# GuyTevet/motion-diffusion-model

Measured on NVIDIA H100. Metric: motions/sec, higher is better.
Workload: dtype fp16 operands / fp32 accumulate (in/out projections hi-lo split)

## Files before the change

include/b200mdm.h:

```cpp
#ifndef B200MDM_H_
#define B200MDM_H_

#include <stdint.h>

#ifdef __cplusplus
extern "C" {
#endif

#define B200MDM_OK 0
#define B200MDM_EINVAL (-1)
#define B200MDM_ECUDA (-2)
#define B200MDM_ESTATE (-3)
#define B200MDM_ENOTIMPL (-4)

#define B200MDM_ARCH_TRANS_ENC 0
#define B200MDM_ARCH_TRANS_DEC 1

#define B200MDM_COND_NONE 0
#define B200MDM_COND_TEXT 1
#define B200MDM_COND_ACTION 2

#define B200MDM_MODE_X0 0
#define B200MDM_MODE_DDPM 1
#define B200MDM_MODE_DDIM 2
#define B200MDM_MODE_DDIM_REVERSE 6

#define B200MDM_FLAG_CONST_NOISE 1
#define B200MDM_FLAG_CLIP_DENOISED 2
#define B200MDM_FLAG_PHILOX_NOISE 4

#define B200MDM_SCHED_STRIDE 8

typedef struct b200mdm_engine b200mdm_engine;

typedef struct b200mdm_config {
  int32_t arch;
  int32_t latent_dim;
  int32_t ff_size;
  int32_t num_layers;
  int32_t num_heads;
  int32_t njoints;
  int32_t nfeats;
  int32_t cond_mode;
  int32_t cond_dim;
  int32_t num_actions;
  int32_t mask_frames;
  int32_t pos_embed_max_len;
  int32_t temb_rows;
  int32_t context_len;
  int32_t target_encoder;
  int32_t target_enc_layers;
  int32_t target_joints;
  int32_t emb_trans_dec;
  int32_t dec_memory;
  int32_t reserved[1];
} b200mdm_config;

#define B200MDM_DEC_MEMORY_TOKENS 0
#define B200MDM_DEC_MEMORY_CLIP 1

#define B200MDM_TARGET_NONE 0
#define B200MDM_TARGET_SINGLE 1
#define B200MDM_TARGET_MULTI 2
#define B200MDM_TARGET_SPLIT 3

const char* b200mdm_last_error(void);
int b200mdm_version(void);

int b200mdm_create(const b200mdm_config* cfg, b200mdm_engine** out);
int b200mdm_destroy(b200mdm_engine* e);

int b200mdm_load_weight(b200mdm_engine* e, const char* name, const float* data, const int64_t* shape, int32_t ndim);

int b200mdm_finalize_weights(b200mdm_engine* e, void* stream);

int b200mdm_set_schedule(b200mdm_engine* e, int32_t n_steps, const float* rows_host, const int32_t* timestep_map_host);

#define B200MDM_SCHED_NEXT_STRIDE 2
int b200mdm_set_schedule_next(b200mdm_engine* e, int32_t n_steps, const float* rows_host);

#define B200MDM_SCHED_DPM_STRIDE 4
int b200mdm_set_schedule_dpm(b200mdm_engine* e, int32_t n_steps, const float* rows_host);

#define B200MDM_SCHED_VB_STRIDE 12
int b200mdm_set_schedule_vb(b200mdm_engine* e, int32_t n_steps, const float* rows_host);

int b200mdm_set_cond(b200mdm_engine* e, int32_t batch, int32_t nframes, const float* cond_embed_dev,
                     const int64_t* lengths_host, const float* scale_dev, int32_t force_uncond,
                     const int64_t* action_host, void* stream);

int b200mdm_set_cond_dec(b200mdm_engine* e, int32_t batch, int32_t nframes, const float* enc_text_dev,
                         const uint8_t* text_mask_host, int32_t n_tokens, const int64_t* lengths_host,
                         const float* scale_dev, int32_t force_uncond, void* stream);
int b200mdm_set_prefix(b200mdm_engine* e, const float* prefix_dev, void* stream);

int b200mdm_set_target(b200mdm_engine* e, const float* target_dev, const uint8_t* valid_host, void* stream);

int b200mdm_set_inpaint(b200mdm_engine* e, const uint8_t* mask_dev, const float* motion_dev);
int b200mdm_set_inpaint_weight(b200mdm_engine* e, const float* weight_dev, const float* motion_dev);

int b200mdm_set_handshake(b200mdm_engine* e, int32_t h, const int64_t* lengths_host, const uint8_t* motion_start_host,
                          void* stream);

int b200mdm_set_joint_guidance(b200mdm_engine* e, const float* mean_dev, const float* std_dev, const float* target_dev,
                               const float* weight_dev, float step, int32_t iters, void* stream);

int b200mdm_set_foot_guidance(b200mdm_engine* e, float contact_weight, float floor_weight, float floor_height,
                              const float* contact_dev, const int64_t* lengths_host, void* stream);

typedef struct b200mdm_grid {
  const float* values;
  int64_t batch_stride;
  int32_t gz, gx;
  float x0, z0, cell;
} b200mdm_grid;

int b200mdm_set_scene_guidance(b200mdm_engine* e, float obstacle_weight, float obstacle_margin, const b200mdm_grid* sdf,
                               const b200mdm_grid* terrain, void* stream);

#define B200MDM_MAX_INTERACTION_PAIRS 1024
int b200mdm_set_interaction_guidance(b200mdm_engine* e, int32_t characters, float weight, float margin,
                                     const float* placement_dev, const int32_t* pairs_host, int32_t n_pairs,
                                     const float* reach_host, const float* pair_weight_dev, int64_t pair_weight_stride,
                                     void* stream);

#define B200MDM_MAX_PROMPTS 8
int b200mdm_set_cond_multi(b200mdm_engine* e, int32_t batch, int32_t nframes, int32_t K, const float* prompt_embed_dev,
                           const int64_t* lengths_host, const int64_t* prompt_action_host, void* stream);
int b200mdm_set_cond_multi_dec(b200mdm_engine* e, int32_t batch, int32_t nframes, int32_t K, const float* prompt_clip_dev,
                               const int64_t* lengths_host, void* stream);
int b200mdm_set_cond_multi_tokens(b200mdm_engine* e, int32_t batch, int32_t nframes, int32_t K, const float* tokens_dev,
                                  const uint8_t* mask_host, int32_t n_tokens, const int64_t* lengths_host, void* stream);
int b200mdm_set_prompt_weight(b200mdm_engine* e, int32_t K, const float* weight_dev, int64_t stride_b, int64_t stride_k,
                              int64_t stride_f, int64_t stride_t, void* stream);

int b200mdm_denoise(b200mdm_engine* e, const float* x_dev, const int32_t* timesteps_host, float* out_dev, void* stream);

int b200mdm_sample_step(b200mdm_engine* e, int32_t mode, int32_t index, const float* x_t_dev, const float* noise_dev,
                        int32_t flags, float* x_out_dev, float* pred_xstart_dev, void* stream);

int b200mdm_sample_loop(b200mdm_engine* e, int32_t mode, int32_t skip_timesteps, const float* x_T_dev, float* x_0_dev,
                        const float* noise_tape_dev, int64_t noise_step_stride, int32_t flags, int32_t use_graph,
                        void* stream);

int b200mdm_sample_loop_range(b200mdm_engine* e, int32_t mode, int32_t first_index, int32_t n_run, const float* x_in_dev,
                              float* x_out_dev, const float* noise_tape_dev, int64_t noise_step_stride, int32_t flags,
                              int32_t use_graph, void* stream);

int b200mdm_sample_step_at(b200mdm_engine* e, int32_t mode, const int32_t* index_host, const float* x_t_dev,
                           const float* noise_dev, int32_t flags, float* x_out_dev, float* pred_xstart_dev, void* stream);

int b200mdm_slots_begin(b200mdm_engine* e, int32_t slots, int32_t nframes, int32_t guided, int32_t mode, int32_t flags,
                        void* stream);

int b200mdm_slot_admit(b200mdm_engine* e, int32_t slot, const float* cond_embed_dev, int64_t action, float scale,
                       int64_t length, uint64_t seed, int64_t sample_index, void* stream);

int b200mdm_slots_run(b200mdm_engine* e, int32_t n_steps, int32_t use_graph, void* stream);

int b200mdm_slot_read(b200mdm_engine* e, int32_t slot, float* out_dev, void* stream);

int b200mdm_chain_slots_begin(b200mdm_engine* e, int32_t slots, int32_t nframes, int32_t guided, int32_t mode,
                              int32_t flags, int32_t n_tokens, void* stream);

int b200mdm_chain_slot_admit(b200mdm_engine* e, int32_t slot, const float* tokens_dev, const uint8_t* mask_dev,
                             const float* prefix_dev, float scale, int64_t length, int32_t include_prefix, uint64_t seed,
                             int64_t sample_index, void* stream);

int b200mdm_chain_slot_handoff(b200mdm_engine* e, int32_t slot, float* out_dev, const float* tokens_dev,
                               const uint8_t* mask_dev, void* stream);

int b200mdm_ddim_reverse_loop_range(b200mdm_engine* e, int32_t first_index, int32_t n_run, const float* x_in_dev,
                                    float* x_out_dev, int32_t flags, int32_t use_graph, void* stream);

int b200mdm_plms_loop_range(b200mdm_engine* e, int32_t order, int32_t first_index, int32_t n_run, const float* x_in_dev,
                            float* x_out_dev, int32_t flags, int32_t use_graph, void* stream);

int b200mdm_plms_step(b200mdm_engine* e, int32_t index, int32_t order, const float* x_t_dev, const float* const* old_eps_dev,
                      int32_t n_old, int32_t flags, float* x_out_dev, float* pred_xstart_dev, float* eps_out_dev,
                      void* stream);

int b200mdm_dpm_loop_range(b200mdm_engine* e, int32_t order, int32_t first_index, int32_t n_run, const float* x_in_dev,
                           float* x_out_dev, int32_t flags, int32_t use_graph, void* stream);
int b200mdm_dpm_pred_xstart(b200mdm_engine* e, float* out_dev, void* stream);

int b200mdm_chain_setup(b200mdm_engine* e, int32_t n_chunks, int32_t pred_len, int32_t context_len, int32_t include_prefix,
                        int32_t crop, const float* enc_chunks_dev, const uint8_t* text_mask_chunks_host, void* stream);
int b200mdm_chain_loop_range(b200mdm_engine* e, int32_t mode, int32_t order, int32_t first_step, int32_t n_run,
                             const float* x_T_dev, int64_t x_T_chunk_stride, const float* noise_tape_dev,
                             int64_t noise_step_stride, float* out_dev, int32_t flags, int32_t use_graph, void* stream);
int b200mdm_chain_set_goal(b200mdm_engine* e, const float* mean_dev, const float* std_dev, const float* goal_dev,
                           int32_t n_goals, const uint8_t* valid_host, void* stream);
int b200mdm_chunk_frame(double* carry_dev, const float* frames_dev, int32_t batch, int32_t n_feats, int32_t n_frames,
                        const float* mean_dev, const float* std_dev, const float* goal_dev, int32_t n_ext, float* target_dev,
                        void* stream);

int b200mdm_vb_loop_range(b200mdm_engine* e, int32_t first_index, int32_t n_run, const float* x_start_dev,
                          const float* noise_tape_dev, int64_t noise_step_stride, int32_t flags, float* terms_dev,
                          float* bpd_dev, int32_t use_graph, void* stream);

int b200mdm_set_noise_stream(b200mdm_engine* e, uint64_t seed, int64_t sample_index_base);
int b200mdm_philox_normal(float* out_dev, int32_t batch, int64_t n_per_sample, uint64_t seed, int64_t sample_index_base,
                          int32_t step_id, void* stream);

int b200mdm_q_sample(b200mdm_engine* e, float sqrt_ac, float sqrt_1mac, const float* x_start_dev,
                     const float* noise_dev, float* out_dev, int64_t n, void* stream);

int64_t b200mdm_launch_count(b200mdm_engine* e, int32_t reset);

int b200mdm_recover_from_ric(const float* data_dev, int64_t stride_b, int64_t stride_f, int64_t stride_t,
                             const float* mean_dev, const float* std_dev, float* out_dev, int64_t ostride_b,
                             int64_t ostride_t, int64_t ostride_c, int32_t batch, int32_t nframes, int32_t njoints,
                             void* stream);

int b200mdm_test_gemm_f16(const void* a16_dev, const void* w16_dev, const float* bias_dev, void* out16_dev, int32_t M,
                          int32_t N, int32_t K, int32_t act, int32_t block_n, void* stream);
int b200mdm_test_gemm_epi(const void* a16_dev, const void* w16_dev, const float* bias_dev, void* out16_dev, int32_t M,
                          int32_t N, int32_t K, int32_t epi, void* stream);
int b200mdm_test_embed(const float* x_dev, const float* w_in_dev, const float* b_in_dev, const float* pe_dev, void* hres16_dev,
                       int32_t B, int32_t JF, int32_t T, int32_t d, int32_t s_off, int32_t halves, void* stream);
int b200mdm_test_out_step(const void* hres16_dev, const float* scale_dev, const float* w_out_dev, const float* b_out_dev,
                          const float* x_t_dev, const float* noise_dev, const float* sched_row_dev, int32_t mode, int32_t flags,
                          const uint8_t* inpaint_mask_dev, const float* inpaint_motion_dev, float* x_out_dev,
                          float* pred_xstart_dev, int32_t B, int32_t JF, int32_t T, int32_t d, int32_t s_off, int32_t halves,
                          void* stream);
int b200mdm_test_out_dpm(const void* hres16_dev, const float* scale_dev, const float* w_out_dev, const float* b_out_dev,
                         const float* x_t_dev, const float* dpm_row_dev, int32_t index, int32_t step, int32_t order,
                         int32_t flags, const uint8_t* inpaint_mask_dev, const float* inpaint_motion_dev,
                         float* x0_hist_dev, float* x_out_dev, int32_t B, int32_t JF, int32_t T, int32_t d, int32_t s_off,
                         int32_t halves, void* stream);
int b200mdm_test_out_vb(const void* hres16_dev, const float* scale_dev, const float* w_out_dev, const float* b_out_dev,
                        const float* x_t_dev, const float* x_start_dev, const float* noise_dev, const float* vb_row_dev,
                        int32_t index, int32_t n_steps, int32_t flags, const uint8_t* inpaint_mask_dev,
                        const float* inpaint_motion_dev, float* pred_xstart_dev, float* elem_dev, float* terms_dev, int32_t B,
                        int32_t JF, int32_t T, int32_t d, int32_t s_off, int32_t halves, void* stream);
int b200mdm_test_out_weight(const void* hres16_dev, const float* scale_dev, const float* w_out_dev, const float* b_out_dev,
                            const float* x_t_dev, int32_t mode, int32_t flags, const float* weight_dev,
                            const float* motion_dev, float* pred_xstart_dev, int32_t B, int32_t JF, int32_t T, int32_t d,
                            int32_t s_off, int32_t halves, void* stream);
int b200mdm_test_blend_handshake(const void* hres16_dev, const float* scale_dev, void* g16_dev, int32_t B, int32_t T,
                                 int32_t d, int32_t s_off, int32_t halves, int32_t h, const int64_t* lengths_host,
                                 const uint8_t* motion_start_host, void* stream);
int b200mdm_test_joint_guidance(const float* x0_dev, const float* mean_dev, const float* std_dev, const float* target_dev,
                                const float* weight_dev, int32_t B, int32_t T, int32_t D, float step, int32_t iters,
                                float* x0_out_dev, float* loss_out_dev, void* stream);
int b200mdm_test_foot_guidance(const float* x0_dev, const float* mean_dev, const float* std_dev, const float* target_dev,
                               const float* weight_dev, const float* contact_dev, const int64_t* lengths_host, int32_t B,
                               int32_t T, int32_t D, float step, int32_t iters, float contact_weight, float floor_weight,
                               float floor_height, float* x0_out_dev, float* loss_out_dev, void* stream);
int b200mdm_test_scene_guidance(const float* x0_dev, const float* mean_dev, const float* std_dev, const float* target_dev,
                                const float* weight_dev, const float* contact_dev, const int64_t* lengths_host, int32_t B,
                                int32_t T, int32_t D, float step, int32_t iters, float contact_weight, float floor_weight,
                                float floor_height, float obstacle_weight, float obstacle_margin, const b200mdm_grid* sdf,
                                const b200mdm_grid* terrain, float* x0_out_dev, float* loss_out_dev, void* stream);
int b200mdm_test_interaction_guidance(const float* x0_dev, const float* mean_dev, const float* std_dev, const float* target_dev,
                                      const float* weight_dev, const float* contact_dev, const int64_t* lengths_host,
                                      int32_t B, int32_t T, int32_t D, float step, int32_t iters, float contact_weight,
                                      float floor_weight, float floor_height, float obstacle_weight, float obstacle_margin,
                                      const b200mdm_grid* sdf, const b200mdm_grid* terrain, int32_t characters, float weight,
                                      float margin, const float* placement_dev, const int32_t* pairs_host, int32_t n_pairs,
                                      const float* reach_host, const float* pair_weight_dev, int64_t pair_weight_stride,
                                      float* x0_out_dev, float* loss_out_dev, void* stream);
int b200mdm_test_attention(const void* qkv16_dev, void* out16_dev, const int32_t* kvlen_dev, int32_t n_samples,
                           int32_t S, int32_t d, int32_t impl, void* stream);
int b200mdm_test_cross_attention(const void* q16_dev, const void* kv16_dev, const unsigned char* mask_dev, void* out16_dev,
                                 int32_t n_samples, int32_t S, int32_t n_tokens, int32_t ld_kv, void* stream);
int b200mdm_test_qkv_attention(const void* h16_dev, int32_t ld, const void* wqkv16_dev, const float* bqkv_dev,
                               void* out16_dev, const int32_t* kvlen_dev, int32_t n_samples, int32_t S, void* stream);
int b200mdm_test_gemm_resid_ln(const void* a16_dev, const void* w16_dev, const float* bias_dev, const float* gamma_dev,
                               const float* beta_dev, void* hres16_dev, int32_t M, int32_t K, void* stream);
int b200mdm_test_target(b200mdm_engine* e, const float* target_dev, const uint8_t* valid_host, int32_t batch,
                        float* out_dev, void* stream);
int b200mdm_test_cross_rows(b200mdm_engine* e, int32_t timestep, float* out_dev, void* stream);
int b200mdm_test_row_bias_ln(void* hres16_dev, const float* c_dev, const float* gamma_dev, const float* beta_dev,
                             int32_t M, int32_t S, void* stream);

#define B200MDM_TAP_EMBED 0
#define B200MDM_TAP_TOK0 1
#define B200MDM_TAP_CONDPROJ 2
#define B200MDM_TAP_TEMB 3
#define B200MDM_TAP_MEM16 4
#define B200MDM_TAP_CROSS_C 5
#define B200MDM_TAP_KVC16 6
#define B200MDM_TAP_L_IN 7
#define B200MDM_TAP_L_QKV 8
#define B200MDM_TAP_L_ATT 9
#define B200MDM_TAP_L_LN1 10
#define B200MDM_TAP_L_QC 11
#define B200MDM_TAP_L_XATT 12
#define B200MDM_TAP_L_LN2 13
#define B200MDM_TAP_L_FFN 14
#define B200MDM_TAP_L_LN3 15
#define B200MDM_TAP_BLEND 16
#define B200MDM_TAP_COUNT 17
int b200mdm_test_forward_taps(b200mdm_engine* e, const float* x_dev, const int32_t* timesteps_host, float* out_dev,
                              int32_t layer, void* const* tap_dev, int32_t n_taps, void* stream);

#ifdef __cplusplus
}
#endif
#endif
```

motion-diffusion-model_b200/_lib.py:

```python
import ctypes
import os

HERE = os.path.dirname(os.path.abspath(__file__))
LIB_PATH = os.environ.get("B200MDM_LIB") or os.path.join(HERE, "lib", "libb200mdm.so")

OK, EINVAL, ECUDA, ESTATE, ENOTIMPL = 0, -1, -2, -3, -4
ARCH = {"trans_enc": 0, "trans_dec": 1}
COND_NONE, COND_TEXT, COND_ACTION = 0, 1, 2
TARGET = {"single": 1, "multi": 2, "split": 3}
MODE_X0, MODE_DDPM, MODE_DDIM = 0, 1, 2
MODE_DDIM_REVERSE = 6
MODE_PLMS_AB, MODE_DPM, MODE_VB = 3, 7, 8
FLAG_CONST_NOISE, FLAG_CLIP_DENOISED, FLAG_PHILOX_NOISE = 1, 2, 4
SCHED_STRIDE = 8
SCHED_NEXT_STRIDE = 2
SCHED_DPM_STRIDE = 4
SCHED_VB_STRIDE = 12

SYMBOLS = [
    "b200mdm_last_error", "b200mdm_version", "b200mdm_create", "b200mdm_destroy", "b200mdm_load_weight",
    "b200mdm_finalize_weights", "b200mdm_set_schedule", "b200mdm_set_cond", "b200mdm_set_cond_dec", "b200mdm_set_prefix",
    "b200mdm_set_inpaint",
    "b200mdm_denoise", "b200mdm_sample_step", "b200mdm_sample_loop", "b200mdm_q_sample", "b200mdm_launch_count",
    "b200mdm_sample_loop_range", "b200mdm_set_noise_stream", "b200mdm_philox_normal",
    "b200mdm_recover_from_ric", "b200mdm_test_gemm_f16", "b200mdm_test_attention", "b200mdm_test_cross_attention", "b200mdm_test_qkv_attention",
    "b200mdm_test_gemm_resid_ln", "b200mdm_test_gemm_epi", "b200mdm_test_embed", "b200mdm_test_out_step",
    "b200mdm_set_target", "b200mdm_test_target", "b200mdm_plms_loop_range", "b200mdm_plms_step",
    "b200mdm_set_schedule_next", "b200mdm_ddim_reverse_loop_range", "b200mdm_test_cross_rows",
    "b200mdm_test_row_bias_ln", "b200mdm_test_forward_taps",
    "b200mdm_set_schedule_dpm", "b200mdm_dpm_loop_range", "b200mdm_dpm_pred_xstart", "b200mdm_test_out_dpm",
    "b200mdm_set_schedule_vb", "b200mdm_vb_loop_range", "b200mdm_test_out_vb",
    "b200mdm_set_handshake", "b200mdm_test_blend_handshake", "b200mdm_set_inpaint_weight", "b200mdm_test_out_weight",
    "b200mdm_chain_setup", "b200mdm_chain_loop_range", "b200mdm_set_joint_guidance", "b200mdm_test_joint_guidance",
    "b200mdm_set_cond_multi", "b200mdm_set_cond_multi_dec", "b200mdm_set_prompt_weight",
    "b200mdm_set_cond_multi_tokens", "b200mdm_set_foot_guidance", "b200mdm_test_foot_guidance",
    "b200mdm_set_scene_guidance", "b200mdm_test_scene_guidance", "b200mdm_chain_set_goal", "b200mdm_chunk_frame",
    "b200mdm_set_interaction_guidance", "b200mdm_test_interaction_guidance",
    "b200mdm_sample_step_at", "b200mdm_slots_begin", "b200mdm_slot_admit", "b200mdm_slots_run", "b200mdm_slot_read",
    "b200mdm_chain_slots_begin", "b200mdm_chain_slot_admit", "b200mdm_chain_slot_handoff",
]
MAX_PROMPTS = 8
MAX_CHARACTERS = 8
MAX_INTERACTION_PAIRS = 1024
MAX_MEMORY_TOKENS = 512
TAPS = ["EMBED", "TOK0", "CONDPROJ", "TEMB", "MEM16", "CROSS_C", "KVC16", "L_IN", "L_QKV", "L_ATT", "L_LN1", "L_QC",
        "L_XATT", "L_LN2", "L_FFN", "L_LN3", "BLEND"]
DEC_MEMORY_TOKENS, DEC_MEMORY_CLIP = 0, 1


class Config(ctypes.Structure):
    _fields_ = [(n, ctypes.c_int32) for n in (
        "arch", "latent_dim", "ff_size", "num_layers", "num_heads", "njoints", "nfeats", "cond_mode", "cond_dim",
        "num_actions", "mask_frames", "pos_embed_max_len", "temb_rows", "context_len", "target_encoder",
        "target_enc_layers", "target_joints", "emb_trans_dec", "dec_memory")] + [("reserved", ctypes.c_int32 * 1)]


class Grid(ctypes.Structure):
    _fields_ = [("values", ctypes.c_void_p), ("batch_stride", ctypes.c_int64), ("gz", ctypes.c_int32),
                ("gx", ctypes.c_int32), ("x0", ctypes.c_float), ("z0", ctypes.c_float), ("cell", ctypes.c_float)]


class B200MDMError(RuntimeError):
    def __init__(self, code, msg):
        super().__init__("libb200mdm error %d: %s" % (code, msg))
        self.code = code


_lib = None


def load():
    global _lib
    if _lib is not None:
        return _lib
    if not os.path.exists(LIB_PATH):
        raise ImportError(
            "libb200mdm.so is not built (%s). Run `python -c 'import __graft_entry__ as g; g.build()'`; "
            "there is no CPU / PyTorch fallback for the sampling path." % LIB_PATH)
    import torch
    lib = ctypes.CDLL(LIB_PATH, mode=ctypes.RTLD_GLOBAL)
    vp, i32, i64, f32 = ctypes.c_void_p, ctypes.c_int32, ctypes.c_int64, ctypes.c_float
    lib.b200mdm_last_error.restype = ctypes.c_char_p
    lib.b200mdm_last_error.argtypes = []
    lib.b200mdm_version.restype = i32
    lib.b200mdm_create.argtypes = [ctypes.POINTER(Config), ctypes.POINTER(vp)]
    lib.b200mdm_destroy.argtypes = [vp]
    lib.b200mdm_load_weight.argtypes = [vp, ctypes.c_char_p, vp, ctypes.POINTER(i64), i32]
    lib.b200mdm_finalize_weights.argtypes = [vp, vp]
    lib.b200mdm_set_schedule.argtypes = [vp, i32, vp, vp]
    lib.b200mdm_set_cond.argtypes = [vp, i32, i32, vp, vp, vp, i32, vp, vp]
    lib.b200mdm_set_cond_dec.argtypes = [vp, i32, i32, vp, vp, i32, vp, vp, i32, vp]
    lib.b200mdm_set_prefix.argtypes = [vp, vp, vp]
    lib.b200mdm_set_inpaint.argtypes = [vp, vp, vp]
    lib.b200mdm_recover_from_ric.argtypes = [vp, i64, i64, i64, vp, vp, vp, i64, i64, i64, i32, i32, i32, vp]
    lib.b200mdm_denoise.argtypes = [vp, vp, vp, vp, vp]
    lib.b200mdm_sample_step.argtypes = [vp, i32, i32, vp, vp, i32, vp, vp, vp]
    lib.b200mdm_sample_step_at.argtypes = [vp, i32, vp, vp, vp, i32, vp, vp, vp]
    lib.b200mdm_slots_begin.argtypes = [vp, i32, i32, i32, i32, i32, vp]
    lib.b200mdm_slot_admit.argtypes = [vp, i32, vp, i64, f32, i64, ctypes.c_uint64, i64, vp]
    lib.b200mdm_slots_run.argtypes = [vp, i32, i32, vp]
    lib.b200mdm_slot_read.argtypes = [vp, i32, vp, vp]
    lib.b200mdm_sample_loop.argtypes = [vp, i32, i32, vp, vp, vp, i64, i32, i32, vp]
    lib.b200mdm_sample_loop_range.argtypes = [vp, i32, i32, i32, vp, vp, vp, i64, i32, i32, vp]
    lib.b200mdm_set_noise_stream.argtypes = [vp, ctypes.c_uint64, i64]
    lib.b200mdm_philox_normal.argtypes = [vp, i32, i64, ctypes.c_uint64, i64, i32, vp]
    lib.b200mdm_q_sample.argtypes = [vp, f32, f32, vp, vp, vp, i64, vp]
    lib.b200mdm_launch_count.argtypes = [vp, i32]
    lib.b200mdm_launch_count.restype = i64
    lib.b200mdm_test_gemm_f16.argtypes = [vp, vp, vp, vp, i32, i32, i32, i32, i32, vp]
    lib.b200mdm_test_attention.argtypes = [vp, vp, vp, i32, i32, i32, i32, vp]
    if hasattr(lib, "b200mdm_test_cross_attention"):
        lib.b200mdm_test_cross_attention.argtypes = [vp, vp, vp, vp, i32, i32, i32, i32, vp]
    lib.b200mdm_test_qkv_attention.argtypes = [vp, i32, vp, vp, vp, vp, i32, i32, vp]
    lib.b200mdm_test_gemm_resid_ln.argtypes = [vp, vp, vp, vp, vp, vp, i32, i32, vp]
    for name, args in (("b200mdm_test_gemm_epi", [vp, vp, vp, vp, i32, i32, i32, i32, vp]),
                       ("b200mdm_test_embed", [vp, vp, vp, vp, vp, i32, i32, i32, i32, i32, i32, vp]),
                       ("b200mdm_test_out_step", [vp, vp, vp, vp, vp, vp, vp, i32, i32, vp, vp, vp, vp,
                                                  i32, i32, i32, i32, i32, i32, vp]),
                       ("b200mdm_set_target", [vp, vp, vp, vp]),
                       ("b200mdm_test_target", [vp, vp, vp, i32, vp, vp]),
                       ("b200mdm_plms_loop_range", [vp, i32, i32, i32, vp, vp, i32, i32, vp]),
                       ("b200mdm_plms_step", [vp, i32, i32, vp, ctypes.POINTER(vp), i32, i32, vp, vp, vp, vp]),
                       ("b200mdm_set_schedule_next", [vp, i32, vp]),
                       ("b200mdm_ddim_reverse_loop_range", [vp, i32, i32, vp, vp, i32, i32, vp]),
                       ("b200mdm_test_cross_rows", [vp, i32, vp, vp]),
                       ("b200mdm_test_row_bias_ln", [vp, vp, vp, vp, i32, i32, vp]),
                       ("b200mdm_test_forward_taps", [vp, vp, vp, vp, i32, ctypes.POINTER(vp), i32, vp]),
                       ("b200mdm_set_schedule_dpm", [vp, i32, vp]),
                       ("b200mdm_dpm_loop_range", [vp, i32, i32, i32, vp, vp, i32, i32, vp]),
                       ("b200mdm_dpm_pred_xstart", [vp, vp, vp]),
                       ("b200mdm_test_out_dpm", [vp, vp, vp, vp, vp, vp, i32, i32, i32, i32, vp, vp, vp, vp,
                                                 i32, i32, i32, i32, i32, i32, vp]),
                       ("b200mdm_set_schedule_vb", [vp, i32, vp]),
                       ("b200mdm_vb_loop_range", [vp, i32, i32, vp, vp, i64, i32, vp, vp, i32, vp]),
                       ("b200mdm_test_out_vb", [vp, vp, vp, vp, vp, vp, vp, vp, i32, i32, i32, vp, vp, vp, vp, vp,
                                                i32, i32, i32, i32, i32, i32, vp]),
                       ("b200mdm_set_handshake", [vp, i32, vp, vp, vp]),
                       ("b200mdm_test_blend_handshake", [vp, vp, vp, i32, i32, i32, i32, i32, i32, vp, vp, vp]),
                       ("b200mdm_set_inpaint_weight", [vp, vp, vp]),
                       ("b200mdm_test_out_weight", [vp, vp, vp, vp, vp, i32, i32, vp, vp, vp, i32, i32, i32, i32, i32, i32,
                                                    vp]),
                       ("b200mdm_chain_setup", [vp, i32, i32, i32, i32, i32, vp, vp, vp]),
                       ("b200mdm_chain_loop_range", [vp, i32, i32, i32, i32, vp, i64, vp, i64, vp, i32, i32, vp]),
                       ("b200mdm_set_joint_guidance", [vp, vp, vp, vp, vp, f32, i32, vp]),
                       ("b200mdm_test_joint_guidance", [vp, vp, vp, vp, vp, i32, i32, i32, f32, i32, vp, vp, vp]),
                       ("b200mdm_set_foot_guidance", [vp, f32, f32, f32, vp, vp, vp]),
                       ("b200mdm_test_foot_guidance", [vp, vp, vp, vp, vp, vp, vp, i32, i32, i32, f32, i32, f32, f32, f32,
                                                       vp, vp, vp]),
                       ("b200mdm_set_scene_guidance", [vp, f32, f32, ctypes.POINTER(Grid), ctypes.POINTER(Grid), vp]),
                       ("b200mdm_test_scene_guidance", [vp, vp, vp, vp, vp, vp, vp, i32, i32, i32, f32, i32, f32, f32, f32,
                                                        f32, f32, ctypes.POINTER(Grid), ctypes.POINTER(Grid), vp, vp, vp]),
                       ("b200mdm_set_interaction_guidance", [vp, i32, f32, f32, vp, vp, i32, vp, vp, ctypes.c_int64, vp]),
                       ("b200mdm_test_interaction_guidance", [vp, vp, vp, vp, vp, vp, vp, i32, i32, i32, f32, i32, f32, f32,
                                                              f32, f32, f32, ctypes.POINTER(Grid), ctypes.POINTER(Grid), i32,
                                                              f32, f32, vp, vp, i32, vp, vp, ctypes.c_int64, vp, vp, vp]),
                       ("b200mdm_set_cond_multi", [vp, i32, i32, i32, vp, vp, vp, vp]),
                       ("b200mdm_set_cond_multi_dec", [vp, i32, i32, i32, vp, vp, vp]),
                       ("b200mdm_set_cond_multi_tokens", [vp, i32, i32, i32, vp, vp, i32, vp, vp]),
                       ("b200mdm_set_prompt_weight", [vp, i32, vp, i64, i64, i64, i64, vp]),
                       ("b200mdm_chain_set_goal", [vp, vp, vp, vp, i32, vp, vp]),
                       ("b200mdm_chunk_frame", [vp, vp, i32, i32, i32, vp, vp, vp, i32, vp, vp]),
                       ("b200mdm_chain_slots_begin", [vp, i32, i32, i32, i32, i32, i32, vp]),
                       ("b200mdm_chain_slot_admit", [vp, i32, vp, vp, vp, f32, i64, i32, ctypes.c_uint64, i64, vp]),
                       ("b200mdm_chain_slot_handoff", [vp, i32, vp, vp, vp, vp])):
        if hasattr(lib, name):
            getattr(lib, name).argtypes = args
    for name in SYMBOLS:
        if not hasattr(lib, name) and os.environ.get("B200MDM_LIB"):
            continue
        fn = getattr(lib, name)
        if fn.restype is ctypes.c_int and name not in ("b200mdm_version",):
            fn.restype = i32
    _lib = lib
    return lib


def check(code):
    if code != OK:
        raise B200MDMError(code, load().b200mdm_last_error().decode("utf-8", "replace"))
```

motion-diffusion-model_b200/csrc/engine.cu:

```cuda
#include <cuda.h>
#include <cuda_fp16.h>
#include <cuda_runtime.h>

#include <algorithm>
#include <cmath>
#include <cstdarg>
#include <cstdio>
#include <cstring>
#include <initializer_list>
#include <map>
#include <string>
#include <vector>

#include "../../include/b200mdm.h"
#include "attention_tc.cuh"
#include "epilogues.cuh"
#include "gemm.cuh"
#include "gemm_ln.cuh"
#include "gemm_pingpong.cuh"
#include "chunk_frame.cuh"
#include "joint_guidance.cuh"
#include "compose.cuh"
#include "postprocess.cuh"
#include "kernels.cuh"

using namespace b200;

static thread_local char g_err[512] = "";
static int fail(int code, const char* fmt, ...) {
  va_list ap;
  va_start(ap, fmt);
  vsnprintf(g_err, sizeof(g_err), fmt, ap);
  va_end(ap);
  return code;
}
#define CUDA_TRY(expr)                                                                               \
  do {                                                                                               \
    cudaError_t _e = (expr);                                                                         \
    if (_e != cudaSuccess)                                                                           \
      return fail(B200MDM_ECUDA, "%s failed: %s (%s:%d)", #expr, cudaGetErrorString(_e), __FILE__, __LINE__); \
  } while (0)
#define TRY(expr)            \
  do {                       \
    int _r = (expr);         \
    if (_r != B200MDM_OK) return _r; \
  } while (0)

typedef CUresult (*EncodeTiledFn)(CUtensorMap*, CUtensorMapDataType, cuuint32_t, void*, const cuuint64_t*,
                                  const cuuint64_t*, const cuuint32_t*, const cuuint32_t*, CUtensorMapInterleave,
                                  CUtensorMapSwizzle, CUtensorMapL2promotion, CUtensorMapFloatOOBfill);
static EncodeTiledFn g_encode = nullptr;
static int resolve_driver() {
  if (g_encode) return B200MDM_OK;
  void* fn = nullptr;
  cudaDriverEntryPointQueryResult qres;
  CUDA_TRY(cudaGetDriverEntryPoint("cuTensorMapEncodeTiled", &fn, cudaEnableDefault, &qres));
  if (!fn || qres != cudaDriverEntryPointSuccess) return fail(B200MDM_ECUDA, "cuTensorMapEncodeTiled not available");
  g_encode = reinterpret_cast<EncodeTiledFn>(fn);
  return B200MDM_OK;
}
static int encode_map(CUtensorMap* m, CUtensorMapDataType dtype, uint32_t rank, const void* ptr, const cuuint64_t* gdim,
                      const cuuint64_t* gstride_bytes, const cuuint32_t* box, CUtensorMapSwizzle swizzle, const char* what) {
  TRY(resolve_driver());
  if ((reinterpret_cast<uintptr_t>(ptr) & 15) || gstride_bytes[0] % 16) return fail(B200MDM_EINVAL, "TMA operand misaligned");
  const cuuint32_t estr[3] = {1, 1, 1};
  CUresult r = g_encode(m, dtype, rank, const_cast<void*>(ptr), gdim, gstride_bytes, box, estr, CU_TENSOR_MAP_INTERLEAVE_NONE,
                        swizzle, CU_TENSOR_MAP_L2_PROMOTION_L2_256B, CU_TENSOR_MAP_FLOAT_OOB_FILL_NONE);
  if (r != CUDA_SUCCESS) return fail(B200MDM_ECUDA, "cuTensorMapEncodeTiled%s failed (%d)", what, static_cast<int>(r));
  return B200MDM_OK;
}
static int make_map_t(CUtensorMap* m, const void* ptr, int elem_bytes, uint64_t rows, uint64_t cols, uint64_t ld,
                      uint32_t box_rows) {
  const cuuint64_t gdim[2] = {cols, rows}, gstr[1] = {ld * elem_bytes};
  const cuuint32_t box[2] = {static_cast<cuuint32_t>(128 / elem_bytes), box_rows};
  return encode_map(m, elem_bytes == 2 ? CU_TENSOR_MAP_DATA_TYPE_FLOAT16 : CU_TENSOR_MAP_DATA_TYPE_FLOAT32, 2, ptr, gdim, gstr,
                    box, CU_TENSOR_MAP_SWIZZLE_128B, "");
}
static int make_map(CUtensorMap* m, const void* ptr, uint64_t rows, uint64_t cols, uint64_t ld, uint32_t box_rows) {
  return make_map_t(m, ptr, 2, rows, cols, ld, box_rows);
}
static int make_map_3d(CUtensorMap* m, const void* ptr, uint64_t n, uint64_t rows, uint64_t cols, uint64_t ld,
                       uint32_t box_rows) {
  const cuuint64_t gdim[3] = {cols, rows, n}, gstr[2] = {ld * 2, rows * ld * 2};
  const cuuint32_t box[3] = {64, box_rows, 1};
  return encode_map(m, CU_TENSOR_MAP_DATA_TYPE_FLOAT16, 3, ptr, gdim, gstr, box, CU_TENSOR_MAP_SWIZZLE_128B, "(3d)");
}

static int make_hres_map(CUtensorMap* m, const void* hres, uint64_t rows) {
  return make_map(m, hres, rows, 2 * GLN_D, 2 * GLN_D, GLN_RES_BOX_ROWS);
}

static int make_map_res(CUtensorMap* m, const void* ptr, uint64_t rows, uint64_t d) {
  const cuuint64_t gdim[2] = {2 * d, rows}, gstr[1] = {d * 4};
  const cuuint32_t box[2] = {32, 32};
  return encode_map(m, CU_TENSOR_MAP_DATA_TYPE_FLOAT16, 2, ptr, gdim, gstr, box, CU_TENSOR_MAP_SWIZZLE_64B, "(residual)");
}

enum SchedTable { TAB_STEP, TAB_NEXT, TAB_DPM, TAB_VB, N_TABLES };
static constexpr int TAB_STRIDE[N_TABLES] = {SCHED_STRIDE, SCHED_NEXT_STRIDE, SCHED_DPM_STRIDE, SCHED_VB_STRIDE};
static const char* const TAB_SETTER[N_TABLES] = {"b200mdm_set_schedule", "b200mdm_set_schedule_next",
                                                 "b200mdm_set_schedule_dpm", "b200mdm_set_schedule_vb"};
static_assert(SCHED_STRIDE == B200MDM_SCHED_STRIDE && SCHED_NEXT_STRIDE == B200MDM_SCHED_NEXT_STRIDE &&
                  SCHED_DPM_STRIDE == B200MDM_SCHED_DPM_STRIDE && SCHED_VB_STRIDE == B200MDM_SCHED_VB_STRIDE,
              "the tables' row layouts are part of the ABI");

struct Tensor32 {
  float* dev = nullptr;
  std::vector<int64_t> shape;
  size_t numel = 0;
};

struct LayerW {
  __half *wqkv = nullptr, *wo = nullptr, *w1 = nullptr, *w2 = nullptr;
  const float *bqkv, *bo, *b1, *b2, *g1, *be1, *g2, *be2;
  CUtensorMap m_wqkv, m_w1;
  CUtensorMap m_wo_256, m_w2_256;
  __half *wq_c = nullptr, *wo_c = nullptr;
  const float *bq_c = nullptr, *bo_c = nullptr, *g3 = nullptr, *be3 = nullptr;
  CUtensorMap m_wq_c, m_wo_c_256;
  const float *wv_c32 = nullptr, *bv_c32 = nullptr, *wo_c32 = nullptr;
};

struct GraphKey {
  int mode = -1, B = 0, T = 0, flags = 0;
  int order = 0;
  const void *pred = nullptr, *imask = nullptr, *iweight = nullptr, *imotion = nullptr;
  const void* target_g = nullptr;
  const void* hs = nullptr;
  int guide = -1;
  int chars = 0;
  int groups = 0;
  bool slots = false;
  bool operator==(const GraphKey& o) const {
    return mode == o.mode && B == o.B && T == o.T && flags == o.flags && order == o.order && pred == o.pred &&
           imask == o.imask && iweight == o.iweight && imotion == o.imotion && target_g == o.target_g && hs == o.hs &&
           guide == o.guide && chars == o.chars && groups == o.groups && slots == o.slots;
  }
};

struct Workspace {
  int B = 0, T = 0, S = 0, halves = 1, Bp = 0, M = 0, MB = 0;
  int groups = 0;
  float* mp_x0 = nullptr;
  __half *xin16 = nullptr, *hres = nullptr, *qkv16 = nullptr, *att16 = nullptr, *ffn16 = nullptr, *g16 = nullptr;
  float *tok0 = nullptr, *condproj = nullptr, *proj = nullptr, *scale = nullptr, *x_work = nullptr, *eps_buf = nullptr;
  int *kvlen = nullptr, *tvec = nullptr, *action = nullptr;
  CUtensorMap m_xin, m_h16, m_att, m_ffn, m_g16;
  CUtensorMap m_qkv_st, m_ffn_st;
  CUtensorMap m_qkv_kv;
  CUtensorMap m_res_c, m_res_u;
  CUtensorMap m_hres;
  float* pe_bias = nullptr;
  bool cond_set = false;
  int Mt = 0;
  float *encperm = nullptr, *memtok = nullptr, *memproj = nullptr;
  __half *mem16 = nullptr, *qc16 = nullptr, *kvc16 = nullptr;
  unsigned char* memmask = nullptr;
  CUtensorMap m_mem, m_qc_st, m_kvc_st;
  bool prefix_set = false;
  float *cross_mb = nullptr, *cross_u = nullptr, *cross_b = nullptr, *cross_c = nullptr;
  float *tgt_valid = nullptr, *tgt_g = nullptr;
  bool target_set = false;
  int* hs_desc = nullptr;
  bool hs_set = false;
  float* jg_x0 = nullptr;
  float *plms_ring = nullptr, *plms_mid = nullptr, *plms_pred = nullptr;
  int plms_done = -1, plms_order = 0;
  float* dpm_hist = nullptr;
  int dpm_done = -1, dpm_order = 0;
  float *vb_xs = nullptr, *vb_part = nullptr, *vb_terms = nullptr;
  int vb_cap = 0;
  bool vb_live = false;
  SlotState* slots = nullptr;
  cudaGraphExec_t graph_exec = nullptr;
  GraphKey graph_key;
  int graph_kernels = 0;
  unsigned long long last_use = 0;
};

struct b200mdm_engine : Workspace {
  b200mdm_config cfg;
  int d, ff, L, H, JF, Kp_in, N_out_pad;
  int num_sms = 132;
  std::map<std::string, Tensor32> store;
  bool finalized = false;
  __half *w_in3 = nullptr, *w_out3 = nullptr;
  CUtensorMap m_win, m_wout;
  std::vector<LayerW> layers;
  const float *b_in = nullptr, *b_out = nullptr, *pe = nullptr, *w_txt = nullptr, *b_txt = nullptr, *act_emb = nullptr;
  float *temb_hidden = nullptr, *temb_table = nullptr;
  __half* wkv_all = nullptr;
  float* bkv_all = nullptr;
  CUtensorMap m_wkv_all;
  float *tw0 = nullptr, *tb0 = nullptr, *twk = nullptr, *tbk = nullptr, *twsum = nullptr;
  int tG = 0, tdj = 0, tin = 0, tlayers = 0;
  std::vector<float> h_valid;
  float* tab[N_TABLES] = {};
  bool tab_fresh[N_TABLES] = {};
  int* tmap = nullptr;
  int n_steps = 0, sched_cap = 0;
  std::vector<Workspace> pool;
  unsigned long long use_clock = 0;
  std::vector<int> h_kv, h_action;
  std::vector<unsigned char> h_mask;
  std::vector<int> h_hs;
  bool dec = false;
  bool dec_clip = false;
  float* cross_t = nullptr;
  int ctx = 0, s_off = 1;
  int kw = 1;
  const unsigned char* inpaint_mask = nullptr;
  const float* inpaint_weight = nullptr;
  const float* inpaint_motion = nullptr;
  GuideDesc* jg_desc = nullptr;
  GuideDesc h_guide{};
  unsigned guide_terms = 0;
  int* fg_len = nullptr;
  int fg_len_cap = 0;
  std::vector<int> h_fg_len;
  InterPair* ig_pairs = nullptr;
  int ig_pairs_cap = 0;
  std::vector<InterPair> h_ig_pairs;
  PromptWeight* pw_desc = nullptr;
  PromptWeight h_pw{};
  bool pw_set = false;
  unsigned long long noise_seed = 0;
  long long noise_sample_base = 0;
  StepState* state = nullptr;
  cudaStream_t work = nullptr;
  cudaEvent_t ev_in = nullptr, ev_out = nullptr;
  long long launches = 0;
  bool mem_uncond = false;
  float *chain_mem = nullptr, *chain_prefix = nullptr;
  unsigned char* chain_mask = nullptr;
  size_t chain_mem_cap = 0, chain_mask_cap = 0, chain_prefix_cap = 0;
  std::vector<unsigned char> h_chain_mask;
  int chain_n = 0, chain_off = 0, chain_crop = 0, chain_next = -1;
  bool chain_mems = false;
  const float* prefix_src = nullptr;
  bool slot_mode = false;
  int slot_sampler = 0, slot_flags = 0;
  std::vector<unsigned char> slot_busy;
  std::vector<int> slot_left;
  std::vector<int> h_slot_idx;
  struct ChainSlot {
    unsigned long long seed = 0;
    long long g = 0;
    float scale = 0.f;
    int kv = 0, length = 0, off = 0, chunk = 0, n_chunks = 0;
  };
  std::vector<ChainSlot> chain_slot;
  const float *goal_mean = nullptr, *goal_std = nullptr, *goal_src = nullptr;
  double* goal_carry = nullptr;
  float* goal_tgt = nullptr;
  size_t goal_carry_cap = 0, goal_tgt_cap = 0;
  int goal_n = 0;
  bool goal_set = false;
};

template <class T>
static int dalloc(T** p, size_t n, bool zero = false) {
  const cudaError_t err = cudaMalloc(reinterpret_cast<void**>(p), n * sizeof(T));
  if (err != cudaSuccess) {
    cudaGetLastError();
    return fail(B200MDM_ECUDA, "cudaMalloc of %zu bytes failed: %s", n * sizeof(T), cudaGetErrorString(err));
  }
  if (zero) CUDA_TRY(cudaMemset(*p, 0, n * sizeof(T)));
  return B200MDM_OK;
}
template <class T>
static void dfree(T*& p) {
  if (p) cudaFree(p);
  p = nullptr;
}

template <int BN, class Epi>
static int set_gemm_attr() {
  CUDA_TRY(cudaFuncSetAttribute(gemm_f16_wgmma<BN, Epi>, cudaFuncAttributeMaxDynamicSharedMemorySize, GemmSmem<BN, Epi>::TOTAL));
  return B200MDM_OK;
}
template <class Epi>
static int set_pingpong_attr() {
  CUDA_TRY(cudaFuncSetAttribute(gemm_f16_pingpong<Epi>, cudaFuncAttributeMaxDynamicSharedMemorySize, PP_SMEM_BYTES));
  return B200MDM_OK;
}
template <int KEYS>
static int set_attention_attr() {
  CUDA_TRY(cudaFuncSetAttribute(attention_tc_kernel<KEYS, false>, cudaFuncAttributeMaxDynamicSharedMemorySize,
                                AttnTcSmem::total(KEYS)));
  CUDA_TRY(cudaFuncSetAttribute(attention_tc_kernel<KEYS, true>, cudaFuncAttributeMaxDynamicSharedMemorySize,
                                AttnTcSmem::total(KEYS)));
  return B200MDM_OK;
}

enum GuideTerm : unsigned { GT_JOINT = 1, GT_FOOT = 2, GT_SCENE = 4, GT_INTER = 8 };
struct GuideVariant {
  void (*step)(const GuideDesc*, const float*, EpiOutParams);
  void (*test)(GuideDesc, const float*, float*, float*, int, int, int);
  size_t (*smem)(int, int);
  bool clusters;
};
static const GuideVariant GUIDE_VARIANTS[] = {
    {joint_guidance_step_kernel<false, false>, joint_guidance_test_kernel<false, false>, jg_smem_bytes, false},
    {joint_guidance_step_kernel<true, false>, joint_guidance_test_kernel<true, false>, fg_smem_bytes, false},
    {joint_guidance_step_kernel<true, true>, joint_guidance_test_kernel<true, true>, fg_smem_bytes, false},
    {joint_guidance_step_kernel<true, true, true>, joint_guidance_test_kernel<true, true, true>, ig_smem_bytes, true},
};
static int guide_variant(unsigned terms) { return terms ? 31 - __builtin_clz(terms) : -1; }
struct RicDims {
  int J, R;
};
static RicDims ric_dims(int D) {
  const int J = D == 263 ? 22 : 21;
  return {J, 4 + 3 * (J - 1)};
}

static int init_kernel_attrs() {
  static unsigned long long done_mask = 0;
  int dev = 0;
  CUDA_TRY(cudaGetDevice(&dev));
  if (dev < 64 && ((done_mask >> dev) & 1ull)) return B200MDM_OK;
  TRY((set_pingpong_attr<EpiBiasF16<false>>()));
  TRY((set_pingpong_attr<EpiBiasF16<true>>()));
  TRY((set_pingpong_attr<EpiBiasF16Wide<true>>()));
  TRY((set_pingpong_attr<EpiBiasF16Global>()));
  CUDA_TRY(cudaFuncSetAttribute(gemm_resid_ln_cluster, cudaFuncAttributeMaxDynamicSharedMemorySize, GemmLnSmem::TOTAL));
  TRY((set_gemm_attr<128, EpiEmbed>()));
  TRY((set_gemm_attr<96, EpiOut<OutStep>>()));
  TRY((set_gemm_attr<96, EpiOut<OutStepSlots>>()));
  TRY((set_gemm_attr<96, EpiOut<OutPlms>>()));
  TRY((set_gemm_attr<96, EpiOut<OutReverse>>()));
  TRY((set_gemm_attr<96, EpiOut<OutDpm>>()));
  TRY((set_gemm_attr<96, EpiOut<OutVb>>()));
  TRY((set_attention_attr<64>()));
  TRY((set_attention_attr<208>()));
  TRY((set_attention_attr<256>()));
  CUDA_TRY(cudaFuncSetAttribute(cross_attention_long_kernel, cudaFuncAttributeMaxDynamicSharedMemorySize, XAL_SMEM));
  for (const GuideVariant& v : GUIDE_VARIANTS) {
    const int smem = static_cast<int>(v.smem(JG_MAX_FRAMES, JG_MAX_FEATS));
    CUDA_TRY(cudaFuncSetAttribute(v.step, cudaFuncAttributeMaxDynamicSharedMemorySize, smem));
    CUDA_TRY(cudaFuncSetAttribute(v.test, cudaFuncAttributeMaxDynamicSharedMemorySize, smem));
  }
  if (dev < 64) done_mask |= 1ull << dev;
  return B200MDM_OK;
}

static bool g_pdl_now = false;
static bool pdl_enabled() {
  static int v = -1;
  if (v < 0) {
    const char* e = getenv("B200MDM_PDL");
    v = (e && e[0] == '0') ? 0 : 1;
  }
  return v == 1;
}
struct PdlScope {
  PdlScope() { g_pdl_now = pdl_enabled(); }
  ~PdlScope() { g_pdl_now = false; }
};
template <class... KArgs, class... Args>
static cudaError_t launch_kc(void (*kern)(KArgs...), dim3 grid, dim3 block, size_t smem, cudaStream_t s, int cluster,
                             Args&&... args) {
  cudaLaunchConfig_t cfg;
  memset(&cfg, 0, sizeof(cfg));
  cfg.gridDim = grid;
  cfg.blockDim = block;
  cfg.dynamicSmemBytes = smem;
  cfg.stream = s;
  cudaLaunchAttribute at[2];
  int n = 0;
  if (cluster > 0) {
    at[n].id = cudaLaunchAttributeClusterDimension;
    at[n].val.clusterDim.x = static_cast<unsigned>(cluster);
    at[n].val.clusterDim.y = 1;
    at[n].val.clusterDim.z = 1;
    ++n;
  }
  if (g_pdl_now) {
    at[n].id = cudaLaunchAttributeProgrammaticStreamSerialization;
    at[n].val.programmaticStreamSerializationAllowed = 1;
    ++n;
  }
  cfg.attrs = at;
  cfg.numAttrs = n;
  return cudaLaunchKernelEx(&cfg, kern, static_cast<KArgs>(std::forward<Args>(args))...);
}
template <class... KArgs, class... Args>
static cudaError_t launch_k(void (*kern)(KArgs...), dim3 grid, dim3 block, size_t smem, cudaStream_t s, Args&&... args) {
  return launch_kc(kern, grid, block, smem, s, 0, std::forward<Args>(args)...);
}

template <class Epi, class = void> struct epi_unstaged : std::false_type {};
template <class Epi> struct epi_unstaged<Epi, std::enable_if_t<Epi::UNSTAGED>> : std::true_type {};

static_assert(GemmSmem<128, EpiEmbed>::STAGES == 2, "shared-memory budget: 2 operand stages for the embedding GEMM");
static_assert(GemmSmem<96, EpiOut<OutStep>>::STAGES == 5, "shared-memory budget: 5 operand stages for the output GEMM");
template <int BN, class Epi>
static int launch_gemm(const CUtensorMap& a, const CUtensorMap& b, int M, int N, int K, const typename Epi::Params& p,
                       cudaStream_t s, int num_sms) {
  const int tiles = ((M + GEMM_BLOCK_M - 1) / GEMM_BLOCK_M) * ((N + BN - 1) / BN);
  const int grid = tiles < num_sms ? tiles : num_sms;
  CUDA_TRY(launch_k(gemm_f16_wgmma<BN, Epi>, dim3(grid), dim3(GEMM_THREADS), GemmSmem<BN, Epi>::TOTAL, s, a, b, M, N, K, p));
  return B200MDM_OK;
}
template <class Epi>
static int launch_gemm_pp(const CUtensorMap& a, const CUtensorMap& b, const CUtensorMap& c, int M, int N, int K,
                          const typename Epi::Params& p, cudaStream_t s, int num_sms) {
  if (!epi_unstaged<Epi>::value && N * 4 > GEMM_BIAS_BYTES)
    return fail(B200MDM_ENOTIMPL, "GEMM epilogue vectors are staged for N <= %d", GEMM_BIAS_BYTES / 4);
  const int tiles = ((M + GEMM_BLOCK_M - 1) / GEMM_BLOCK_M) * ((N + PP_BLOCK_N - 1) / PP_BLOCK_N);
  const int grid = tiles < num_sms ? tiles : num_sms;
  CUDA_TRY(launch_k(gemm_f16_pingpong<Epi>, dim3(grid), dim3(GEMM_THREADS), PP_SMEM_BYTES, s, a, b, c, M, N, K, p));
  return B200MDM_OK;
}
template <bool GELU>
static int launch_gemm_bias(const CUtensorMap& a, const CUtensorMap& b, const CUtensorMap& c, int M, int N, int K,
                            const float* bias, cudaStream_t s, int num_sms) {
  typename EpiBiasF16<GELU>::Params p{bias};
  return launch_gemm_pp<EpiBiasF16<GELU>>(a, b, c, M, N, K, p, s, num_sms);
}

static int launch_gemm_resid_ln(const CUtensorMap& a, const CUtensorMap& w256, const CUtensorMap& hres, int M, int K,
                                const float* bias, const float* gamma, const float* beta, cudaStream_t s, int num_sms) {
  const int tiles = (M + GEMM_BLOCK_M - 1) / GEMM_BLOCK_M;
  const int max_clusters = num_sms / 2;
  const int clusters = tiles < max_clusters ? tiles : max_clusters;
  GemmLnParams lp{bias, gamma, beta, 1e-5f};
  CUDA_TRY(launch_k(gemm_resid_ln_cluster, dim3(2 * clusters), dim3(GLN_THREADS), GemmLnSmem::TOTAL, s, a, w256, hres, M, K, lp));
  return B200MDM_OK;
}

static int make_attention_kv_map(CUtensorMap* m, const void* qkv, int n_samples, int S, int ld) {
  return make_map_3d(m, qkv, n_samples, S, ld, ld, atc_keys(S));
}
template <int KEYS>
static cudaError_t launch_attention_keys(const CUtensorMap& map_kv, const __half* qkv, __half* out, const int* kvlen,
                                         dim3 grid, int S, int d, float scale_log2, cudaStream_t s, bool wide) {
  return launch_k(wide ? attention_tc_kernel<KEYS, true> : attention_tc_kernel<KEYS, false>, grid, dim3(ATC_THREADS),
                  AttnTcSmem::total(KEYS), s, map_kv, qkv, out, kvlen, S, d, scale_log2);
}
static int launch_attention_tc(const CUtensorMap& map_kv, const __half* qkv, __half* out, const int* kvlen, int n_samples,
                               int S, int d, int H, cudaStream_t s, bool wide = false) {
  if (d != H * ATC_DH) return fail(B200MDM_ENOTIMPL, "attention: head_dim must be 128");
  if (S > ATC_MAX_KEYS) return fail(B200MDM_ENOTIMPL, "attention: at most %d tokens per sample", ATC_MAX_KEYS);
  const float scale_log2 = 1.4426950408889634f / sqrtf(static_cast<float>(ATC_DH));
  const int tiles = (S + ATC_QROWS - 1) / ATC_QROWS;
  const dim3 grid(H, n_samples, (tiles + ATC_TILES_PER_CTA - 1) / ATC_TILES_PER_CTA);
  const int keys = atc_keys(S);
  if (keys == 64) CUDA_TRY(launch_attention_keys<64>(map_kv, qkv, out, kvlen, grid, S, d, scale_log2, s, wide));
  else if (keys == 208) CUDA_TRY(launch_attention_keys<208>(map_kv, qkv, out, kvlen, grid, S, d, scale_log2, s, wide));
  else CUDA_TRY(launch_attention_keys<256>(map_kv, qkv, out, kvlen, grid, S, d, scale_log2, s, wide));
  return B200MDM_OK;
}
static int launch_cross_attention(const __half* q16, const __half* kv, const unsigned char* mask, __half* out, int n_samples,
                                  int S, int Mt, int d, int H, int ld_kv, cudaStream_t s) {
  const float sl2 = 1.4426950408889634f / sqrtf(128.0f);
  const dim3 cg(H, n_samples), cb(128);
  if (Mt <= 16)
    CUDA_TRY(launch_k(cross_attention_kernel<2>, cg, cb, 0, s, q16, kv, mask, out, S, Mt, d, ld_kv, sl2));
  else if (Mt <= 32)
    CUDA_TRY(launch_k(cross_attention_kernel<4>, cg, cb, 0, s, q16, kv, mask, out, S, Mt, d, ld_kv, sl2));
  else if (Mt <= 64)
    CUDA_TRY(launch_k(cross_attention_kernel<8>, cg, cb, 0, s, q16, kv, mask, out, S, Mt, d, ld_kv, sl2));
  else
    CUDA_TRY(launch_k(cross_attention_long_kernel, dim3(H, n_samples, (S + XAL_ROWS - 1) / XAL_ROWS), cb, XAL_SMEM, s, q16, kv,
                      mask, out, S, Mt, d, ld_kv, sl2));
  return B200MDM_OK;
}
static int launch_row_bias_ln(__half* hres, const float* c, const float* gamma, const float* beta, int M, int S, cudaStream_t s) {
  CUDA_TRY(launch_k(row_bias_ln_kernel, dim3((M + RBLN_ROWS_PER_CTA - 1) / RBLN_ROWS_PER_CTA), dim3(32 * RBLN_ROWS_PER_CTA), 0, s,
                    hres, c, gamma, beta, M, S, 1e-5f));
  return B200MDM_OK;
}
static int philox_blocks(int B, long long n) {
  const long long quads = (n + 3) / 4 * B;
  return static_cast<int>(quads / 256 + 1 < 1184 ? quads / 256 + 1 : 1184);
}
static int launch_philox(float* out, int B, long long n, unsigned long long seed, long long sample_base, uint32_t step_id,
                         const StepState* state, cudaStream_t s) {
  CUDA_TRY(launch_k(philox_normal_kernel, dim3(philox_blocks(B, n)), dim3(256), 0, s, out, B, n, seed, sample_base, step_id,
                    state));
  return B200MDM_OK;
}
static int launch_pack_input(const float* x, __half* xin16, int B, int JF, int cols, int S, int Kp, int row_off, cudaStream_t s) {
  CUDA_TRY(launch_k(pack_input_kernel, dim3((cols + 31) / 32, (JF + 31) / 32, B), dim3(32, 8), 0, s, x, xin16, B, JF, cols, S,
                    Kp, 3 * Kp, row_off));
  return B200MDM_OK;
}
static int launch_embed_gemm(const CUtensorMap& m_xin, const CUtensorMap& m_win, const CUtensorMap& m_res_c,
                             const CUtensorMap& m_res_u, const float* pe_bias, int MB, int S, int d, int Kp, int halves,
                             cudaStream_t s, int num_sms) {
  EpiEmbed::Params p;
  p.res_c = m_res_c; p.res_u = m_res_u;
  p.pe_bias = pe_bias;
  p.S = S; p.d = d; p.halves = halves;
  return launch_gemm<128, EpiEmbed>(m_xin, m_win, MB, d, 3 * Kp, p, s, num_sms);
}
static int launch_vb_xt(float* x_t, const float* x_start, const float* noise, const float* sched_vb, const StepState* state,
                        size_t n, cudaStream_t s) {
  const int blocks = static_cast<int>(n / 256 + 1 < 1184 ? n / 256 + 1 : 1184);
  CUDA_TRY(launch_k(vb_xt_kernel, dim3(blocks), dim3(256), 0, s, x_t, x_start, noise, sched_vb, state, n));
  return B200MDM_OK;
}
static int launch_vb_reduce(float* terms, int ld_terms, const float* part, int B, int T, int JF, const StepState* state,
                            cudaStream_t s) {
  CUDA_TRY(launch_k(vb_reduce_kernel, dim3(B, VB_TERMS), dim3(VB_REDUCE_THREADS), 0, s, terms, ld_terms, part, B,
                    T * ((JF + 31) / 32), static_cast<float>(JF) * static_cast<float>(T), state));
  return B200MDM_OK;
}
static int launch_blend_split(const __half* hres, __half* g16, const float* scale, int B, int S, int T, int s_off, int d,
                              int halves, const int* hs, cudaStream_t s) {
  CUDA_TRY(launch_k(blend_split_kernel, dim3((B * T + 7) / 8), dim3(256), 0, s, hres, g16, scale, B, S, T, s_off, d, halves, hs));
  return B200MDM_OK;
}

static int handshake_desc(int h, int B, int T, const int64_t* lengths, const uint8_t* motion_start, std::vector<int>* desc) {
  desc->clear();
  if (h < 0) return fail(B200MDM_EINVAL, "handshake size %d < 0", h);
  if (B <= 0 || T <= 0) return fail(B200MDM_EINVAL, "bad batch / nframes");
  if (motion_start && !motion_start[0]) return fail(B200MDM_EINVAL, "window 0 must begin a motion (motion_start[0])");
  if (h == 0) return B200MDM_OK;
  std::vector<int> d(1 + 2 * static_cast<size_t>(B), 0);
  d[HS_H] = h;
  bool any = false;
  for (int b = 0; b < B; ++b) {
    const long long n = lengths ? lengths[b] : T;
    if (n < 0 || n > T) return fail(B200MDM_EINVAL, "window %d: length %lld outside [0, %d]", b, n, T);
    d[HS_LEN(b)] = static_cast<int>(n);
    d[HS_CHAIN(b)] = (b > 0 && !(motion_start && motion_start[b])) ? 1 : 0;
    any = any || d[HS_CHAIN(b)];
  }
  for (int b = 0; b < B; ++b) {
    const bool prev = d[HS_CHAIN(b)] != 0, next = b + 1 < B && d[HS_CHAIN(b + 1)] != 0;
    const int n = d[HS_LEN(b)];
    if ((prev || next) && n < h) return fail(B200MDM_EINVAL, "chained window %d has %d frames < handshake size %d", b, n, h);
    if (prev && next && n < 2 * h)
      return fail(B200MDM_EINVAL, "window %d has %d frames < 2 x handshake size %d: its two handshakes would overlap", b, n, h);
  }
  if (any) desc->swap(d);
  return B200MDM_OK;
}
#ifdef B200_TRACE
static int debug_skip_mask() {
  static int v = -1;
  if (v < 0) {
    const char* e = getenv("B200MDM_DEBUG_SKIP");
    v = e ? atoi(e) : 0;
  }
  return v;
}
#define B200_SKIP(bit) (debug_skip_mask() & (bit))
#else
#define B200_SKIP(bit) (0)
#endif
extern "C" const char* b200mdm_last_error(void) { return g_err; }
extern "C" int b200mdm_version(void) { return 1; }

extern "C" int b200mdm_create(const b200mdm_config* cfg, b200mdm_engine** out) {
  if (!cfg || !out) return fail(B200MDM_EINVAL, "null argument");
  if (cfg->arch != B200MDM_ARCH_TRANS_ENC && cfg->arch != B200MDM_ARCH_TRANS_DEC)
    return fail(B200MDM_ENOTIMPL, "arch %d: trans_enc and trans_dec are implemented", cfg->arch);
  if (cfg->arch == B200MDM_ARCH_TRANS_DEC && (cfg->cond_mode != B200MDM_COND_TEXT || cfg->context_len < 0))
    return fail(B200MDM_ENOTIMPL, "trans_dec needs text-token conditioning (BERT) and context_len >= 0");
  if (cfg->emb_trans_dec < 0 || cfg->emb_trans_dec > 1 || cfg->dec_memory < B200MDM_DEC_MEMORY_TOKENS ||
      cfg->dec_memory > B200MDM_DEC_MEMORY_CLIP)
    return fail(B200MDM_EINVAL, "emb_trans_dec must be 0 or 1 and dec_memory 0 (tokens) or 1 (CLIP) (got %d / %d)",
                cfg->emb_trans_dec, cfg->dec_memory);
  if (cfg->arch == B200MDM_ARCH_TRANS_ENC && (cfg->emb_trans_dec || cfg->dec_memory))
    return fail(B200MDM_EINVAL, "emb_trans_dec and dec_memory are trans_dec fields");
  if (cfg->arch == B200MDM_ARCH_TRANS_DEC && (cfg->dec_memory == B200MDM_DEC_MEMORY_CLIP) != (cfg->emb_trans_dec == 1))
    return fail(B200MDM_ENOTIMPL, "trans_dec implements the BERT token memory without the timestep token (DiP) and the CLIP "
                "memory with it (emb_trans_dec); got dec_memory %d, emb_trans_dec %d", cfg->dec_memory, cfg->emb_trans_dec);
  if (cfg->dec_memory == B200MDM_DEC_MEMORY_CLIP && cfg->context_len != 0)
    return fail(B200MDM_ENOTIMPL, "trans_dec with a CLIP memory has no prefix completion (context_len %d)", cfg->context_len);
  if (cfg->latent_dim != 512 || cfg->num_heads != 4 || cfg->ff_size % 64 || cfg->ff_size <= 0)
    return fail(B200MDM_ENOTIMPL, "kernels are specialised for latent_dim 512 / 4 heads (got %d / %d)", cfg->latent_dim,
                cfg->num_heads);
  if (cfg->num_layers <= 0 || cfg->njoints <= 0 || cfg->nfeats <= 0 || cfg->pos_embed_max_len <= 0 || cfg->temb_rows <= 0)
    return fail(B200MDM_EINVAL, "bad config");
  if (cfg->target_encoder < B200MDM_TARGET_NONE || cfg->target_encoder > B200MDM_TARGET_SPLIT)
    return fail(B200MDM_EINVAL, "target_encoder %d: 0 none, 1 single, 2 multi, 3 split", cfg->target_encoder);
  if (cfg->target_encoder != B200MDM_TARGET_NONE) {
    if (cfg->target_joints <= 0 || cfg->target_joints > 64 || cfg->target_enc_layers < 0 || cfg->target_enc_layers > 16)
      return fail(B200MDM_EINVAL, "target encoder: 1..64 joints and 0..16 layers (got %d / %d)", cfg->target_joints,
                  cfg->target_enc_layers);
    if (cfg->target_encoder == B200MDM_TARGET_SPLIT && cfg->latent_dim % cfg->target_joints)
      return fail(B200MDM_EINVAL, "split target encoder: latent_dim %% target_joints != 0 (model/mdm.py:427)");
  }
  int dev = 0;
  CUDA_TRY(cudaGetDevice(&dev));
  cudaDeviceProp prop;
  CUDA_TRY(cudaGetDeviceProperties(&prop, dev));
  if (prop.major != 9 || prop.minor != 0) return fail(B200MDM_ECUDA, "sm_90a device required (found sm_%d%d)", prop.major, prop.minor);
  TRY(init_kernel_attrs());
  TRY(resolve_driver());
  b200mdm_engine* e = new b200mdm_engine();
  e->cfg = *cfg;
  e->d = cfg->latent_dim;
  e->ff = cfg->ff_size;
  e->L = cfg->num_layers;
  e->H = cfg->num_heads;
  e->JF = cfg->njoints * cfg->nfeats;
  e->Kp_in = (e->JF + 7) & ~7;
  e->N_out_pad = ((e->JF + 95) / 96) * 96;
  e->num_sms = prop.multiProcessorCount;
  e->layers.resize(e->L);
  e->dec = cfg->arch == B200MDM_ARCH_TRANS_DEC;
  e->dec_clip = e->dec && cfg->dec_memory == B200MDM_DEC_MEMORY_CLIP;
  e->ctx = e->dec ? cfg->context_len : 0;
  e->s_off = (e->dec && !e->dec_clip) ? e->ctx : 1;
  e->kw = (e->dec && !e->dec_clip) ? 2 : 1;
  CUDA_TRY(cudaStreamCreateWithFlags(&e->work, cudaStreamNonBlocking));
  CUDA_TRY(cudaEventCreateWithFlags(&e->ev_in, cudaEventDisableTiming));
  CUDA_TRY(cudaEventCreateWithFlags(&e->ev_out, cudaEventDisableTiming));
  TRY(dalloc(&e->state, 1, true));
  *out = e;
  return B200MDM_OK;
}

static void drop_graph(Workspace* w) {
  if (w->graph_exec) cudaGraphExecDestroy(w->graph_exec);
  w->graph_exec = nullptr;
  w->graph_key = GraphKey();
}
static void free_workspace(Workspace* w) {
  drop_graph(w);
  dfree(w->xin16); dfree(w->hres); dfree(w->qkv16); dfree(w->att16); dfree(w->ffn16); dfree(w->g16);
  dfree(w->tok0); dfree(w->condproj); dfree(w->proj); dfree(w->scale); dfree(w->x_work); dfree(w->pe_bias); dfree(w->eps_buf);
  dfree(w->kvlen); dfree(w->tvec); dfree(w->action); dfree(w->slots);
  dfree(w->encperm); dfree(w->memtok); dfree(w->memproj); dfree(w->mem16); dfree(w->qc16); dfree(w->kvc16); dfree(w->memmask);
  dfree(w->cross_mb); dfree(w->cross_u); dfree(w->cross_b); dfree(w->cross_c);
  dfree(w->tgt_valid); dfree(w->tgt_g); dfree(w->hs_desc); dfree(w->jg_x0); dfree(w->mp_x0);
  dfree(w->plms_ring); dfree(w->plms_mid); dfree(w->plms_pred);
  dfree(w->dpm_hist);
  dfree(w->vb_xs); dfree(w->vb_part); dfree(w->vb_terms);
  *w = Workspace();
}
static void free_all_workspaces(b200mdm_engine* e) {
  free_workspace(static_cast<Workspace*>(e));
  for (auto& w : e->pool) free_workspace(&w);
  e->pool.clear();
}
static void drop_all_graphs(b200mdm_engine* e) {
  drop_graph(static_cast<Workspace*>(e));
  for (auto& w : e->pool) drop_graph(&w);
}

static void free_repacks(b200mdm_engine* e) {
  for (auto& l : e->layers) { dfree(l.wqkv); dfree(l.wo); dfree(l.w1); dfree(l.w2); dfree(l.wq_c); dfree(l.wo_c); }
  dfree(e->w_in3); dfree(e->w_out3); dfree(e->temb_hidden); dfree(e->temb_table); dfree(e->wkv_all); dfree(e->bkv_all);
  dfree(e->cross_t);
}

extern "C" int b200mdm_destroy(b200mdm_engine* e) {
  if (!e) return B200MDM_OK;
  cudaDeviceSynchronize();
  free_all_workspaces(e);
  for (auto& kv : e->store) cudaFree(kv.second.dev);
  free_repacks(e);
  for (float*& t : e->tab) dfree(t);
  dfree(e->tmap);
  dfree(e->chain_mem); dfree(e->chain_mask); dfree(e->chain_prefix);
  dfree(e->goal_carry); dfree(e->goal_tgt);
  dfree(e->tw0); dfree(e->tb0); dfree(e->twk); dfree(e->tbk); dfree(e->twsum);
  dfree(e->state);
  dfree(e->jg_desc);
  dfree(e->ig_pairs);
  dfree(e->fg_len);
  dfree(e->pw_desc);
  if (e->work) cudaStreamDestroy(e->work);
  if (e->ev_in) cudaEventDestroy(e->ev_in);
  if (e->ev_out) cudaEventDestroy(e->ev_out);
  delete e;
  return B200MDM_OK;
}

static bool known_weight_name(const b200mdm_engine* e, const std::string& n) {
  static const char* fixed[] = {"input_process.poseEmbedding.weight", "input_process.poseEmbedding.bias",
                                "embed_timestep.time_embed.0.weight", "embed_timestep.time_embed.0.bias",
                                "embed_timestep.time_embed.2.weight", "embed_timestep.time_embed.2.bias",
                                "embed_text.weight", "embed_text.bias", "embed_action.action_embedding",
                                "output_process.poseFinal.weight", "output_process.poseFinal.bias",
                                "sequence_pos_encoder.pe", "embed_timestep.sequence_pos_encoder.pe"};
  for (const char* f : fixed)
    if (n == f) return true;
  static const char* per_layer[] = {"self_attn.in_proj_weight", "self_attn.in_proj_bias", "self_attn.out_proj.weight",
                                    "self_attn.out_proj.bias", "linear1.weight", "linear1.bias", "linear2.weight",
                                    "linear2.bias", "norm1.weight", "norm1.bias", "norm2.weight", "norm2.bias",
                                    "multihead_attn.in_proj_weight", "multihead_attn.in_proj_bias",
                                    "multihead_attn.out_proj.weight", "multihead_attn.out_proj.bias", "norm3.weight", "norm3.bias"};
  const std::string pre = e->dec ? "seqTransDecoder.layers." : "seqTransEncoder.layers.";
  if (n.compare(0, pre.size(), pre) == 0) {
    size_t dot = n.find('.', pre.size());
    if (dot == std::string::npos) return false;
    int l = atoi(n.substr(pre.size(), dot - pre.size()).c_str());
    if (l < 0 || l >= e->L) return false;
    std::string rest = n.substr(dot + 1);
    for (const char* f : per_layer)
      if (rest == f) return true;
  }
  if (e->cfg.target_encoder != B200MDM_TARGET_NONE) {
    const int tl = e->cfg.target_enc_layers, nj = e->cfg.target_joints;
    auto lin = [](const std::string& r, int max_layer) {
      for (int k = 0; k <= max_layer; ++k)
        if (r == std::to_string(2 * k) + ".weight" || r == std::to_string(2 * k) + ".bias") return true;
      return false;
    };
    auto joint = [nj](const std::string& r, std::string* tail) {
      size_t dot = r.find('.');
      if (dot == std::string::npos || dot == 0 || r.find_first_not_of("0123456789") != dot) return false;
      if (atoi(r.substr(0, dot).c_str()) >= nj) return false;
      *tail = r.substr(dot + 1);
      return true;
    };
    const std::string pre = "embed_target_cond.";
    if (n.compare(0, pre.size(), pre) != 0) return false;
    const std::string r = n.substr(pre.size());
    std::string tail;
    switch (e->cfg.target_encoder) {
      case B200MDM_TARGET_SINGLE:
        return r.compare(0, 4, "mlp.") == 0 && lin(r.substr(4), tl);
      case B200MDM_TARGET_SPLIT:
        return r.compare(0, 10, "mini_mlps.") == 0 && joint(r.substr(10), &tail) && lin(tail, tl);
      case B200MDM_TARGET_MULTI:
        if (r == "target_all_loc_emb.weights") return true;
        return r.compare(0, 15, "target_loc_emb.") == 0 && joint(r.substr(15), &tail) && lin(tail, 1);
    }
  }
  return false;
}

// ... 836 lines not shown
  CUDA_TRY(cudaOccupancyMaxActiveClusters(&n, kern, &cfg));
  if (n < 1) return fail(B200MDM_ENOTIMPL, "a cluster of %d guidance CTAs (%zu B of shared memory each) cannot be resident",
                         characters, smem);
  return B200MDM_OK;
}

static int upload_guide(b200mdm_engine* e, unsigned term, void* stream) {
  CUDA_TRY(cudaMemcpyAsync(e->jg_desc, &e->h_guide, sizeof(GuideDesc), cudaMemcpyHostToDevice,
                           static_cast<cudaStream_t>(stream)));
  e->guide_terms |= term;
  return B200MDM_OK;
}

extern "C" int b200mdm_set_joint_guidance(b200mdm_engine* e, const float* mean_dev, const float* std_dev,
                                          const float* target_dev, const float* weight_dev, float step, int32_t iters,
                                          void* stream) {
  if (!e) return fail(B200MDM_EINVAL, "null argument");
  JointGuide j;
  TRY(fill_joint(mean_dev, std_dev, target_dev, weight_dev, step, iters, &j));
  if (e->cfg.nfeats != 1 || (e->JF != 263 && e->JF != 251))
    return fail(B200MDM_EINVAL, "joint-position control needs the ric features of HumanML3D (263) or KIT (251) with nfeats 1 "
                "(got %d x %d)", e->cfg.njoints, e->cfg.nfeats);
  TRY(refuse(e, FAM_JOINT, F_PREFIX));
  if (!e->cond_set) return fail(B200MDM_ESTATE, "call b200mdm_set_cond / b200mdm_set_cond_dec first (they size the workspace)");
  TRY(refuse(e, FAM_JOINT));
  if (e->T > JG_MAX_FRAMES) return fail(B200MDM_ENOTIMPL, "joint-position control: at most %d frames", JG_MAX_FRAMES);
  if (!e->jg_desc) TRY(dalloc(&e->jg_desc, 1));
  if (!e->jg_x0) TRY(dalloc(&e->jg_x0, static_cast<size_t>(e->B) * e->JF * e->T));
  e->guide_terms = 0;
  e->h_guide = GuideDesc{};
  e->h_guide.j = j;
  return upload_guide(e, GT_JOINT, stream);
}

extern "C" int b200mdm_set_foot_guidance(b200mdm_engine* e, float contact_weight, float floor_weight, float floor_height,
                                         const float* contact_dev, const int64_t* lengths_host, void* stream) {
  if (!e) return fail(B200MDM_EINVAL, "null engine");
  FootGuide f;
  std::vector<int> len;
  TRY(fill_foot(contact_weight, floor_weight, floor_height, contact_dev, lengths_host, e->B, e->T, &f, &len));
  if (!(e->guide_terms & GT_JOINT)) return fail(B200MDM_ESTATE, "call b200mdm_set_joint_guidance first (foot guidance extends it)");
  e->guide_terms &= GT_FOOT - 1;
  if (lengths_host) {
    if (e->fg_len_cap < e->B) {
      dfree(e->fg_len);
      e->fg_len_cap = 0;
      TRY(dalloc(&e->fg_len, static_cast<size_t>(e->B)));
      e->fg_len_cap = e->B;
    }
    e->h_fg_len = std::move(len);
    CUDA_TRY(cudaMemcpyAsync(e->fg_len, e->h_fg_len.data(), e->B * sizeof(int), cudaMemcpyHostToDevice,
                             static_cast<cudaStream_t>(stream)));
    f.lengths = e->fg_len;
  }
  e->h_guide.f = f;
  e->h_guide.s = SceneGuide{};
  e->h_guide.i = InterGuide{};
  return upload_guide(e, contact_weight == 0.f && floor_weight == 0.f ? 0u : GT_FOOT, stream);
}

extern "C" int b200mdm_set_scene_guidance(b200mdm_engine* e, float obstacle_weight, float obstacle_margin,
                                          const b200mdm_grid* sdf, const b200mdm_grid* terrain, void* stream) {
  if (!e) return fail(B200MDM_EINVAL, "null engine");
  const bool joint = e->guide_terms & GT_JOINT;
  SceneGuide sg{};
  TRY(fill_scene(obstacle_weight, obstacle_margin, sdf, terrain, e->B, joint ? &e->h_guide.f : nullptr,
                 " (b200mdm_set_foot_guidance)", &sg));
  if (!joint) return fail(B200MDM_ESTATE, "call b200mdm_set_joint_guidance first (scene guidance extends it)");
  e->guide_terms &= GT_SCENE - 1;
  e->h_guide.s = sg;
  e->h_guide.i = InterGuide{};
  return upload_guide(e, obstacle_weight == 0.f && !terrain ? 0u : GT_SCENE, stream);
}

extern "C" int b200mdm_set_interaction_guidance(b200mdm_engine* e, int32_t characters, float weight, float margin,
                                                const float* placement_dev, const int32_t* pairs_host, int32_t n_pairs,
                                                const float* reach_host, const float* pair_weight_dev,
                                                int64_t pair_weight_stride, void* stream) {
  if (!e) return fail(B200MDM_EINVAL, "null engine");
  if (!(e->guide_terms & GT_JOINT))
    return fail(B200MDM_ESTATE, "call b200mdm_set_joint_guidance first (interaction guidance extends it)");
  InterGuide ig;
  std::vector<InterPair> rows;
  TRY(fill_inter(characters, weight, margin, placement_dev, pairs_host, n_pairs, reach_host, pair_weight_dev,
                 pair_weight_stride, e->B, e->T, e->JF, &ig, &rows));
  TRY(init_kernel_attrs());
  TRY(check_inter_cluster(GUIDE_VARIANTS[guide_variant(GT_INTER)].step, characters, e->B, e->T, e->JF));
  e->guide_terms &= GT_INTER - 1;
  if (n_pairs > 0) {
    if (e->ig_pairs_cap < n_pairs) {
      dfree(e->ig_pairs);
      e->ig_pairs_cap = 0;
      TRY(dalloc(&e->ig_pairs, static_cast<size_t>(n_pairs)));
      e->ig_pairs_cap = n_pairs;
    }
    e->h_ig_pairs = std::move(rows);
    CUDA_TRY(cudaMemcpyAsync(e->ig_pairs, e->h_ig_pairs.data(), n_pairs * sizeof(InterPair), cudaMemcpyHostToDevice,
                             static_cast<cudaStream_t>(stream)));
  }
  ig.pairs = e->ig_pairs;
  e->h_guide.i = ig;
  return upload_guide(e, GT_INTER, stream);
}

extern "C" int b200mdm_set_prompt_weight(b200mdm_engine* e, int32_t K, const float* weight_dev, int64_t stride_b,
                                         int64_t stride_k, int64_t stride_f, int64_t stride_t, void* stream) {
  if (!e || !weight_dev) return fail(B200MDM_EINVAL, "null argument");
  if (stride_b < 0 || stride_k < 0 || stride_f < 0 || stride_t < 0) return fail(B200MDM_EINVAL, "negative weight stride");
  if (!e->cond_set || e->groups == 0)
    return fail(B200MDM_ESTATE, "call b200mdm_set_cond_multi / b200mdm_set_cond_multi_dec first (they clear the weights)");
  if (K != e->groups - 1) return fail(B200MDM_EINVAL, "%d prompt weights for %d prompts", K, e->groups - 1);
  if (!e->pw_desc) TRY(dalloc(&e->pw_desc, 1));
  e->h_pw = PromptWeight{weight_dev, stride_b, stride_k, stride_f, stride_t, K};
  CUDA_TRY(cudaMemcpyAsync(e->pw_desc, &e->h_pw, sizeof(PromptWeight), cudaMemcpyHostToDevice, static_cast<cudaStream_t>(stream)));
  e->pw_set = true;
  return B200MDM_OK;
}

struct StepArgs {
  int mode = B200MDM_MODE_X0;
  const float* x_in = nullptr;
  const float* noise = nullptr;
  int const_noise = 0;
  int clip = 0;
  float* x_out = nullptr;
  float* pred = nullptr;
  bool explicit_t = false;
  bool philox = false;
  int back = 0;
  const float* x_step = nullptr;
  int order = 0;
  bool model_only = false;
  bool slots = false;
};

static void set_step_params(EpiOutParams* pp, const StepArgs& a, int B, int T, int JF) {
  EpiOutParams& p = *pp;
  p.x_t = a.x_in;
  p.noise = a.noise;
  p.x_out = a.x_out;
  p.pred_xstart = a.pred;
  p.x_step = a.x_step;
  p.noise_batch_stride = a.const_noise ? 0 : static_cast<long long>(JF) * T;
  p.B = B; p.T = T; p.J = JF; p.mode = a.mode;
  p.vb_chunks = (JF + 31) / 32;
  p.clip_denoised = a.clip;
  p.order = a.order;
  p.back = a.back;
}
static int launch_out_gemm(const CUtensorMap& m_g16, const CUtensorMap& m_wout, int B, int T, int JF, int d,
                           const StepArgs& a, EpiOutParams p, cudaStream_t s, int sms) {
  set_step_params(&p, a, B, T, JF);
  const int M = B * T, N = ((JF + 95) / 96) * 96, K = 3 * d;
  if (a.slots) return launch_gemm<96, EpiOut<OutStepSlots>>(m_g16, m_wout, M, N, K, p, s, sms);
  if (a.mode <= MODE_DDIM) return launch_gemm<96, EpiOut<OutStep>>(m_g16, m_wout, M, N, K, p, s, sms);
  if (a.mode == MODE_DDIM_REVERSE) return launch_gemm<96, EpiOut<OutReverse>>(m_g16, m_wout, M, N, K, p, s, sms);
  if (a.mode == MODE_DPM) return launch_gemm<96, EpiOut<OutDpm>>(m_g16, m_wout, M, N, K, p, s, sms);
  if (a.mode == MODE_VB) return launch_gemm<96, EpiOut<OutVb>>(m_g16, m_wout, M, N, K, p, s, sms);
  return launch_gemm<96, EpiOut<OutPlms>>(m_g16, m_wout, M, N, K, p, s, sms);
}

struct ForwardTaps {
  int layer = 0;
  void* const* dst = nullptr;
  int n = 0;
  const int32_t* t_host = nullptr;
};

static void tap_source(const b200mdm_engine* e, int id, const void** src, size_t* bytes) {
  const size_t M = e->M, d = e->d, h = sizeof(__half), f = sizeof(float), kw = e->kw, mem = static_cast<size_t>(e->Bp) * e->Mt;
  const bool dip = e->dec && !e->dec_clip;
  *src = nullptr;
  *bytes = 0;
  switch (id) {
    case B200MDM_TAP_EMBED: case B200MDM_TAP_TOK0: case B200MDM_TAP_L_IN: case B200MDM_TAP_L_LN1: case B200MDM_TAP_L_LN3:
      *src = e->hres; *bytes = M * 2 * d * h; break;
    case B200MDM_TAP_L_LN2:
      if (e->dec) { *src = e->hres; *bytes = M * 2 * d * h; }
      break;
    case B200MDM_TAP_CONDPROJ:
      if (!dip) { *src = e->condproj; *bytes = static_cast<size_t>(e->Bp) * d * f; }
      break;
    case B200MDM_TAP_TEMB: *src = e->temb_table; *bytes = static_cast<size_t>(e->B) * d * f; break;
    case B200MDM_TAP_MEM16: if (dip) { *src = e->mem16; *bytes = mem * 2 * d * h; } break;
    case B200MDM_TAP_KVC16: if (dip) { *src = e->kvc16; *bytes = mem * 2 * d * e->L * h; } break;
    case B200MDM_TAP_CROSS_C:
      if (e->dec_clip) { *src = e->cross_c; *bytes = static_cast<size_t>(e->L) * e->Bp * d * f; }
      break;
    case B200MDM_TAP_L_QKV: *src = e->qkv16; *bytes = M * 3 * d * h; break;
    case B200MDM_TAP_L_ATT: *src = e->att16; *bytes = M * kw * d * h; break;
    case B200MDM_TAP_L_QC: if (dip) { *src = e->qc16; *bytes = M * d * h; } break;
    case B200MDM_TAP_L_XATT: if (dip) { *src = e->att16; *bytes = M * kw * d * h; } break;
    case B200MDM_TAP_L_FFN: *src = e->ffn16; *bytes = M * kw * e->ff * h; break;
    case B200MDM_TAP_BLEND:
      *src = e->g16; *bytes = static_cast<size_t>(e->groups ? e->Bp : e->B) * e->T * 3 * d * h; break;
  }
}

static int take_taps(const b200mdm_engine* e, const ForwardTaps& tp, int first, int last, int l, cudaStream_t s) {
  if (l >= 0 && l != tp.layer) return B200MDM_OK;
  for (int id = first; id <= last && id < tp.n; ++id) {
    if (!tp.dst[id]) continue;
    const void* src;
    size_t bytes;
    tap_source(e, id, &src, &bytes);
    if (bytes == 0) continue;
    if (id == B200MDM_TAP_TEMB) {
      const size_t row = static_cast<size_t>(e->d) * sizeof(float);
      for (int b = 0; b < e->B; ++b)
        CUDA_TRY(cudaMemcpyAsync(static_cast<char*>(tp.dst[id]) + b * row, e->temb_table + static_cast<size_t>(tp.t_host[b]) * e->d,
                                 row, cudaMemcpyDeviceToDevice, s));
      continue;
    }
    CUDA_TRY(cudaMemcpyAsync(tp.dst[id], src, bytes, cudaMemcpyDeviceToDevice, s));
  }
  return B200MDM_OK;
}

static int launch_cross_rows(const b200mdm_engine* e, float* out, const int* tvec, int back, cudaStream_t s) {
  CUDA_TRY(launch_k(cross_rows_kernel, dim3(e->Bp, e->L), dim3(128), 0, s, out, e->cross_b, e->cross_t, tvec, e->tmap, e->state,
                    e->B, e->Bp, e->d, e->cfg.temb_rows, back));
  return B200MDM_OK;
}

static int enqueue_forward(b200mdm_engine* e, const StepArgs& a, cudaStream_t s, int* n_kernels,
                           const ForwardTaps* taps = nullptr) {
  const int d = e->d, ff = e->ff, B = e->B, T = e->T, S = e->S, JF = e->JF, Kp = e->Kp_in;
  int nk = 0;
  PdlScope pdl_scope;
  if (a.philox && a.slots) {
    const long long n = static_cast<long long>(JF) * T;
    CUDA_TRY(launch_k(philox_slots_kernel, dim3(philox_blocks(B, n)), dim3(256), 0, s, e->eps_buf, B, n,
                      static_cast<const SlotState*>(e->slots)));
    ++nk;
  } else if (a.philox) {
    TRY(launch_philox(e->eps_buf, B, static_cast<long long>(JF) * T, 0ull, 0ll, 0u, e->state, s));
    ++nk;
  }
  if (a.mode == MODE_VB) {
    TRY(launch_vb_xt(e->x_work, e->vb_xs, a.noise, e->tab[TAB_VB], e->state, static_cast<size_t>(B) * JF * T, s));
    ++nk;
  }
  TRY(launch_pack_input(a.x_in, e->xin16, B, JF, T, S, Kp, e->s_off, s));
  TRY(launch_embed_gemm(e->m_xin, e->m_win, e->m_res_c, e->m_res_u, e->pe_bias, e->MB, S, d, Kp, e->halves > 1 || e->groups > 1 ? 2 : 1,
                        s, e->num_sms));
  nk += 2;
  for (int g = 1; g < e->groups - 1; g += 2) {
    const int pair = g + 1 < e->groups - 1 ? 2 : 1;
    CUtensorMap m_a, m_b;
    TRY(make_map_res(&m_a, e->hres + static_cast<size_t>(g) * e->MB * d * 2, e->MB, d));
    TRY(make_map_res(&m_b, e->hres + static_cast<size_t>(g + pair - 1) * e->MB * d * 2, e->MB, d));
    TRY(launch_embed_gemm(e->m_xin, e->m_win, m_a, m_b, e->pe_bias, e->MB, S, d, Kp, pair, s, e->num_sms));
    ++nk;
  }
  if (taps) TRY(take_taps(e, *taps, B200MDM_TAP_EMBED, B200MDM_TAP_EMBED, -1, s));
  const float* target_g = e->target_set ? e->tgt_g : nullptr;
  if (!e->dec || e->dec_clip) {
    CUDA_TRY(launch_k(tok0_rows_kernel, dim3(e->Bp), dim3(128), 0, s, e->hres, e->dec_clip ? nullptr : e->condproj,
                      e->temb_table, e->pe, a.explicit_t ? e->tvec : nullptr, e->tmap, e->state, target_g, B, S, d,
                      e->cfg.temb_rows, a.back));
    if (e->dec_clip) {
      TRY(launch_cross_rows(e, e->cross_c, a.explicit_t ? e->tvec : nullptr, a.back, s));
      ++nk;
    }
  } else {
    CUDA_TRY(launch_k(mem_build_kernel, dim3(e->Mt, e->Bp), dim3(128), 0, s, e->mem16, e->memproj, e->temb_table,
                      a.explicit_t ? e->tvec : nullptr, e->tmap, e->state, target_g, B, e->Mt, d, e->cfg.temb_rows, a.back));
    EpiBiasF16Global::Params p{e->bkv_all};
    TRY((launch_gemm_pp<EpiBiasF16Global>(e->m_mem, e->m_wkv_all, e->m_kvc_st, e->Bp * e->Mt, e->L * 2 * d, d, p, s, e->num_sms)));
    ++nk;
  }
  ++nk;
  if (taps) TRY(take_taps(e, *taps, B200MDM_TAP_TOK0, B200MDM_TAP_KVC16, -1, s));
  const int kw = e->kw;
  const bool wide = kw == 2;
  for (int l = 0; l < e->L; ++l) {
    const LayerW& w = e->layers[l];
    if (taps) TRY(take_taps(e, *taps, B200MDM_TAP_L_IN, B200MDM_TAP_L_IN, l, s));
    if (B200_SKIP(1)) {
      ++nk;
    } else {
      {
        TRY((launch_gemm_bias<false>(e->m_h16, w.m_wqkv, e->m_qkv_st, e->M, 3 * d, d, w.bqkv, s, e->num_sms)));
      }
      if (taps) TRY(take_taps(e, *taps, B200MDM_TAP_L_QKV, B200MDM_TAP_L_QKV, l, s));
      TRY(launch_attention_tc(e->m_qkv_kv, e->qkv16, e->att16, e->kvlen, e->Bp, S, d, e->H, s, wide));
      if (taps) TRY(take_taps(e, *taps, B200MDM_TAP_L_ATT, B200MDM_TAP_L_ATT, l, s));
    }
    if (!B200_SKIP(2)) TRY(launch_gemm_resid_ln(e->m_att, w.m_wo_256, e->m_hres, e->M, kw * d, w.bo, w.g1, w.be1, s, e->num_sms));
    if (taps) TRY(take_taps(e, *taps, B200MDM_TAP_L_LN1, B200MDM_TAP_L_LN1, l, s));
    if (e->dec_clip) {
      TRY(launch_row_bias_ln(e->hres, e->cross_c + static_cast<size_t>(l) * e->Bp * d, w.g2, w.be2, e->M, S, s));
      ++nk;
    } else if (e->dec) {
      TRY((launch_gemm_bias<false>(e->m_h16, w.m_wq_c, e->m_qc_st, e->M, d, d, w.bq_c, s, e->num_sms)));
      if (taps) TRY(take_taps(e, *taps, B200MDM_TAP_L_QC, B200MDM_TAP_L_QC, l, s));
      TRY(launch_cross_attention(e->qc16, e->kvc16 + static_cast<size_t>(l) * 2 * d, e->memmask, e->att16, e->Bp, S, e->Mt, d,
                                 e->H, e->L * 2 * d, s));
      if (taps) TRY(take_taps(e, *taps, B200MDM_TAP_L_XATT, B200MDM_TAP_L_XATT, l, s));
      TRY(launch_gemm_resid_ln(e->m_att, w.m_wo_c_256, e->m_hres, e->M, d, w.bo_c, w.g2, w.be2, s, e->num_sms));
      nk += 3;
    }
    if (taps) TRY(take_taps(e, *taps, B200MDM_TAP_L_LN2, B200MDM_TAP_L_LN2, l, s));
    if (wide) {
      EpiBiasF16Wide<true>::Params p{w.b1, ff};
      TRY((launch_gemm_pp<EpiBiasF16Wide<true>>(e->m_h16, w.m_w1, e->m_ffn_st, e->M, ff, kw * d, p, s, e->num_sms)));
    } else if (!B200_SKIP(4)) {
      TRY((launch_gemm_bias<true>(e->m_h16, w.m_w1, e->m_ffn_st, e->M, ff, d, w.b1, s, e->num_sms)));
    }
    if (taps) TRY(take_taps(e, *taps, B200MDM_TAP_L_FFN, B200MDM_TAP_L_FFN, l, s));
    if (!B200_SKIP(8)) TRY(launch_gemm_resid_ln(e->m_ffn, w.m_w2_256, e->m_hres, e->M, kw * ff, w.b2, e->dec ? w.g3 : w.g2,
                             e->dec ? w.be3 : w.be2, s, e->num_sms));
    if (taps) TRY(take_taps(e, *taps, B200MDM_TAP_L_LN3, B200MDM_TAP_L_LN3, l, s));
    nk += 5;
  }
  const int G = e->groups, GB = G ? G * B : B;
  TRY(launch_blend_split(e->hres, e->g16, e->scale, GB, S, T, e->s_off, d, G ? 1 : e->halves, e->hs_set ? e->hs_desc : nullptr, s));
  ++nk;
  if (taps) TRY(take_taps(e, *taps, B200MDM_TAP_BLEND, B200MDM_TAP_BLEND, -1, s));
  {
    EpiOutParams p{};
    p.bias = e->b_out;
    p.inpaint_mask = a.model_only ? nullptr : e->inpaint_mask;
    p.inpaint_weight = a.model_only ? nullptr : e->inpaint_weight;
    p.inpaint_motion = a.model_only ? nullptr : e->inpaint_motion;
    set_tables(&p, e->tab);
    p.eps_ring = e->plms_ring;
    p.x0_hist = e->dpm_hist;
    p.x_start = e->vb_xs;
    p.vb_part = e->vb_part;
    p.state = e->state;
    p.slots = e->slots;
    if (G) {
      StepArgs ax = a;
      ax.mode = MODE_X0;
      ax.x_out = e->mp_x0;
      ax.pred = nullptr;
      ax.clip = 0;
      EpiOutParams px = p;
      px.inpaint_mask = nullptr;
      px.inpaint_weight = nullptr;
      px.inpaint_motion = nullptr;
      TRY(launch_out_gemm(e->m_g16, e->m_wout, GB, T, JF, d, ax, px, s, e->num_sms));
      set_step_params(&p, a, B, T, JF);
      const dim3 grid(static_cast<unsigned>((static_cast<size_t>(JF) * T + MP_THREADS - 1) / MP_THREADS), B);
      const PromptWeight* pw = e->pw_desc;
      const float* x0g = e->mp_x0;
      if (a.mode <= MODE_DDIM) CUDA_TRY(launch_k(compose_step_kernel<OutStep>, grid, dim3(MP_THREADS), 0, s, pw, x0g, p));
      else if (a.mode == MODE_DDIM_REVERSE) CUDA_TRY(launch_k(compose_step_kernel<OutReverse>, grid, dim3(MP_THREADS), 0, s, pw, x0g, p));
      else if (a.mode == MODE_DPM) CUDA_TRY(launch_k(compose_step_kernel<OutDpm>, grid, dim3(MP_THREADS), 0, s, pw, x0g, p));
      else
        CUDA_TRY(launch_k(compose_step_kernel<OutPlms>, grid, dim3(MP_THREADS), 0, s, pw, x0g, p));
      nk += 2;
    } else if (e->guide_terms && !a.model_only) {
      StepArgs ax = a;
      ax.mode = MODE_X0;
      ax.x_out = e->jg_x0;
      ax.pred = nullptr;
      ax.clip = 0;
      EpiOutParams px = p;
      px.inpaint_mask = nullptr;
      px.inpaint_weight = nullptr;
      px.inpaint_motion = nullptr;
      TRY(launch_out_gemm(e->m_g16, e->m_wout, B, T, JF, d, ax, px, s, e->num_sms));
      set_step_params(&p, a, B, T, JF);
      const GuideVariant& v = GUIDE_VARIANTS[guide_variant(e->guide_terms)];
      CUDA_TRY(launch_kc(v.step, dim3(B), dim3(JG_THREADS), v.smem(T, ric_dims(JF).R), s, v.clusters ? e->h_guide.i.chars : 0,
                         static_cast<const GuideDesc*>(e->jg_desc), static_cast<const float*>(e->jg_x0), p));
      nk += 2;
    } else {
      TRY(launch_out_gemm(e->m_g16, e->m_wout, B, T, JF, d, a, p, s, e->num_sms));
      ++nk;
    }
  }
  if (a.mode == MODE_VB) {
    TRY(launch_vb_reduce(e->vb_terms, e->vb_cap, e->vb_part, B, T, JF, e->state, s));
    ++nk;
  }
  *n_kernels = nk;
  return B200MDM_OK;
}

static int check_ready(b200mdm_engine* e, bool need_sched) {
  if (!e) return fail(B200MDM_EINVAL, "null engine");
  if (!e->finalized) return fail(B200MDM_ESTATE, "weights not finalised");
  if (!e->cond_set) return fail(B200MDM_ESTATE, "b200mdm_set_cond has not been called");
  if (e->dec && e->ctx > 0 && !e->prefix_set) return fail(B200MDM_ESTATE, "b200mdm_set_prefix has not been called (y['prefix'])");
  if (need_sched && e->n_steps <= 0) return fail(B200MDM_ESTATE, "b200mdm_set_schedule has not been called");
  if (e->groups && !e->pw_set) return fail(B200MDM_ESTATE, "b200mdm_set_prompt_weight has not been called");
  return B200MDM_OK;
}

static int check_flags(const char* family, int32_t flags, int32_t allowed) {
  if (!(flags & ~allowed)) return B200MDM_OK;
  return fail(B200MDM_EINVAL, "%s takes no flag but B200MDM_FLAG_CLIP_DENOISED%s", family,
              (allowed & B200MDM_FLAG_PHILOX_NOISE) ? " and B200MDM_FLAG_PHILOX_NOISE" : "");
}

static int check_timesteps(const b200mdm_engine* e, const int32_t* timesteps_host) {
  for (int b = 0; b < e->B; ++b)
    if (timesteps_host[b] < 0 || timesteps_host[b] >= e->cfg.temb_rows)
      return fail(B200MDM_EINVAL, "timestep %d outside the pre-embedded range [0, %d)", timesteps_host[b], e->cfg.temb_rows);
  return B200MDM_OK;
}

static int denoise_forward(b200mdm_engine* e, const float* x_dev, const int32_t* timesteps_host, float* out_dev,
                           cudaStream_t s, const ForwardTaps* taps, int* n_kernels) {
  CUDA_TRY(cudaMemcpyAsync(e->tvec, timesteps_host, e->B * sizeof(int), cudaMemcpyHostToDevice, s));
  CUDA_TRY(cudaStreamSynchronize(s));
  StepArgs a;
  a.mode = B200MDM_MODE_X0;
  a.x_in = x_dev;
  a.x_out = out_dev;
  a.explicit_t = true;
  a.model_only = true;
  return enqueue_forward(e, a, s, n_kernels, taps);
}

extern "C" int b200mdm_denoise(b200mdm_engine* e, const float* x_dev, const int32_t* timesteps_host, float* out_dev,
                               void* stream) {
  TRY(check_ready(e, false));
  if (!x_dev || !timesteps_host || !out_dev) return fail(B200MDM_EINVAL, "null tensor");
  TRY(check_timesteps(e, timesteps_host));
  int nk = 0;
  TRY(denoise_forward(e, x_dev, timesteps_host, out_dev, static_cast<cudaStream_t>(stream), nullptr, &nk));
  e->launches += nk;
  return B200MDM_OK;
}

extern "C" int b200mdm_test_forward_taps(b200mdm_engine* e, const float* x_dev, const int32_t* timesteps_host, float* out_dev,
                                         int32_t layer, void* const* tap_dev, int32_t n_taps, void* stream) {
  if (!e || !x_dev || !timesteps_host || !out_dev) return fail(B200MDM_EINVAL, "null argument");
  if (n_taps < 0 || n_taps > B200MDM_TAP_COUNT || (n_taps > 0 && !tap_dev))
    return fail(B200MDM_EINVAL, "n_taps %d: 0..%d tap buffers (tap_dev may be NULL only with n_taps 0)", n_taps, B200MDM_TAP_COUNT);
  TRY(check_ready(e, false));
  if (layer < 0 || layer >= e->L) return fail(B200MDM_EINVAL, "layer %d outside [0, %d)", layer, e->L);
  TRY(check_timesteps(e, timesteps_host));
  for (int id = 0; id < n_taps; ++id) {
    const void* src;
    size_t bytes;
    tap_source(e, id, &src, &bytes);
    if (tap_dev[id] && bytes == 0) return fail(B200MDM_EINVAL, "tap point %d does not exist in this model", id);
  }
  ForwardTaps tp;
  tp.layer = layer;
  tp.dst = tap_dev;
  tp.n = n_taps;
  tp.t_host = timesteps_host;
  int nk = 0;
  return denoise_forward(e, x_dev, timesteps_host, out_dev, static_cast<cudaStream_t>(stream), &tp, &nk);
}

extern "C" int b200mdm_sample_step(b200mdm_engine* e, int32_t mode, int32_t index, const float* x_t_dev,
                                   const float* noise_dev, int32_t flags, float* x_out_dev,
                                   float* pred_xstart_dev, void* stream) {
  TRY(check_ready(e, true));
  const bool reverse = mode == B200MDM_MODE_DDIM_REVERSE;
  if (mode != B200MDM_MODE_DDPM && mode != B200MDM_MODE_DDIM && !reverse) return fail(B200MDM_EINVAL, "bad mode");
  if (index < 0 || index >= e->n_steps) return fail(B200MDM_EINVAL, "schedule index out of range");
  if (!x_t_dev || (!noise_dev && !reverse) || !x_out_dev) return fail(B200MDM_EINVAL, "null tensor");
  if (reverse) {
    TRY(check_flags("DDIM inversion", flags, B200MDM_FLAG_CLIP_DENOISED));
    TRY(need_table(e, TAB_NEXT));
    TRY(refuse(e, FAM_REVERSE));
  }
  cudaStream_t s = static_cast<cudaStream_t>(stream);
  step_set_kernel<<<1, 1, 0, s>>>(e->state, 0, index, nullptr, 0, e->noise_seed, e->noise_sample_base, e->n_steps);
  CUDA_TRY(cudaGetLastError());
  StepArgs a;
  a.mode = mode;
  a.x_in = x_t_dev;
  a.noise = noise_dev;
  a.const_noise = flags & B200MDM_FLAG_CONST_NOISE;
  a.clip = (flags & B200MDM_FLAG_CLIP_DENOISED) ? 1 : 0;
  a.x_out = x_out_dev;
  a.pred = pred_xstart_dev;
  int nk = 0;
  TRY(enqueue_forward(e, a, s, &nk));
  e->launches += nk + 1;
  return B200MDM_OK;
}

static cudaError_t launch_advance(b200mdm_engine* e, const StepArgs& a, cudaStream_t s) {
  PdlScope pdl_scope;
  if (a.slots)
    return launch_k(slot_advance_kernel, dim3((e->B + 127) / 128), dim3(128), 0, s, e->slots, e->tvec,
                    static_cast<const int*>(e->tmap), e->B);
  return launch_k(step_advance_kernel, dim3(1), dim3(1), 0, s, e->state, a.mode == MODE_DDIM_REVERSE ? 1 : -1);
}

static int ensure_step_graph(b200mdm_engine* e, const GraphKey& key, const StepArgs& a) {
  if (e->graph_exec && key == e->graph_key) return B200MDM_OK;
  drop_graph(e);
  cudaGraph_t graph = nullptr;
  CUDA_TRY(cudaStreamBeginCapture(e->work, cudaStreamCaptureModeThreadLocal));
  int nk = 0;
  int r = enqueue_forward(e, a, e->work, &nk);
  if (r == B200MDM_OK && launch_advance(e, a, e->work) != cudaSuccess)
    r = fail(B200MDM_ECUDA, "step_advance launch failed during capture");
  cudaError_t ce = cudaStreamEndCapture(e->work, &graph);
  if (r != B200MDM_OK) {
    if (graph) cudaGraphDestroy(graph);
    return r;
  }
  if (ce != cudaSuccess) return fail(B200MDM_ECUDA, "graph capture failed: %s", cudaGetErrorString(ce));
  ce = cudaGraphInstantiate(&e->graph_exec, graph, 0);
  cudaGraphDestroy(graph);
  if (ce != cudaSuccess) {
    e->graph_exec = nullptr;
    return fail(B200MDM_ECUDA, "graph instantiate failed: %s", cudaGetErrorString(ce));
  }
  e->graph_key = key;
  e->graph_kernels = nk + 1;
  return B200MDM_OK;
}

static int enqueue_step(b200mdm_engine* e, const StepArgs& a, cudaStream_t s, bool use_graph) {
  if (use_graph) {
    CUDA_TRY(cudaGraphLaunch(e->graph_exec, s));
    e->launches += e->graph_kernels;
    return B200MDM_OK;
  }
  int nk = 0;
  TRY(enqueue_forward(e, a, s, &nk));
  CUDA_TRY(launch_advance(e, a, s));
  e->launches += nk + 1;
  return B200MDM_OK;
}

static int enqueue_plms_euler(b200mdm_engine* e, const StepArgs& base, const float* x_t, float* x_out, cudaStream_t s) {
  StepArgs a = base;
  a.mode = MODE_PLMS_EULER1;
  a.x_in = x_t;
  a.x_out = e->plms_mid;
  a.pred = e->plms_pred;
  int nk1 = 0, nk2 = 0;
  TRY(enqueue_forward(e, a, s, &nk1));
  a.mode = MODE_PLMS_EULER2;
  a.x_in = e->plms_mid;
  a.x_step = x_t;
  a.x_out = x_out;
  a.back = 1;
  TRY(enqueue_forward(e, a, s, &nk2));
  CUDA_TRY(launch_advance(e, a, s));
  e->launches += nk1 + nk2 + 1;
  return B200MDM_OK;
}

static int loop_enter(b200mdm_engine* e, const StepArgs& a, int32_t flags, int32_t use_graph, cudaStream_t user,
                      cudaStream_t* s) {
  *s = use_graph ? e->work : user;
  if (!use_graph) attach_l2_window(e, user);
  if (use_graph) {
    GraphKey key;
    key.mode = a.mode; key.B = e->B; key.T = e->T; key.flags = flags; key.order = a.order;
    key.imask = e->inpaint_mask; key.iweight = e->inpaint_weight; key.imotion = e->inpaint_motion;
    key.target_g = e->target_set ? e->tgt_g : nullptr;
    key.hs = e->hs_set ? e->hs_desc : nullptr;
    key.guide = guide_variant(e->guide_terms);
    key.chars = key.guide >= 0 && GUIDE_VARIANTS[key.guide].clusters ? e->h_guide.i.chars : 0;
    key.groups = e->groups;
    key.slots = a.slots;
    TRY(ensure_step_graph(e, key, a));
    CUDA_TRY(cudaEventRecord(e->ev_in, user));
    CUDA_TRY(cudaStreamWaitEvent(e->work, e->ev_in, 0));
  }
  e->plms_done = -1;
  e->dpm_done = -1;
  e->chain_next = -1;
  return B200MDM_OK;
}

static int loop_leave(b200mdm_engine* e, int32_t use_graph, cudaStream_t user) {
  if (use_graph) {
    CUDA_TRY(cudaEventRecord(e->ev_out, e->work));
    CUDA_TRY(cudaStreamWaitEvent(user, e->ev_out, 0));
  }
  return B200MDM_OK;
}

static int run_loop(b200mdm_engine* e, const StepArgs& a, int32_t flags, int32_t first_index, int32_t n_run,
                    const float* x_in_dev, float* x_out_dev, const float* noise_tape_dev, int64_t noise_step_stride,
                    int32_t use_graph, void* stream, int done = 0, bool plms_euler = false) {
  cudaStream_t user = static_cast<cudaStream_t>(stream);
  const size_t x_bytes = static_cast<size_t>(e->B) * e->JF * e->T * sizeof(float);
  cudaStream_t s;
  TRY(loop_enter(e, a, flags, use_graph, user, &s));
  if (x_in_dev) CUDA_TRY(cudaMemcpyAsync(e->x_work, x_in_dev, x_bytes, cudaMemcpyDeviceToDevice, s));
  step_set_kernel<<<1, 1, 0, s>>>(e->state, done, first_index, noise_tape_dev, noise_step_stride, e->noise_seed,
                                  e->noise_sample_base, e->n_steps);
  CUDA_TRY(cudaGetLastError());
  e->launches += 1;
  int k = 0;
  if (plms_euler) {
    TRY(enqueue_plms_euler(e, a, e->x_work, e->x_work, s));
    k = 1;
  }
  for (; k < n_run; ++k) TRY(enqueue_step(e, a, s, use_graph));
  if (a.mode == MODE_PLMS_AB) {
    e->plms_done = done + n_run;
    e->plms_order = a.order;
  } else if (a.mode == MODE_DPM) {
    e->dpm_done = done + n_run;
    e->dpm_order = a.order;
  }
  if (x_out_dev) CUDA_TRY(cudaMemcpyAsync(x_out_dev, e->x_work, x_bytes, cudaMemcpyDeviceToDevice, s));
  return loop_leave(e, use_graph, user);
}

static int check_range_down(const b200mdm_engine* e, int32_t first_index, int32_t n_run) {
  if (n_run <= 0 || first_index >= e->n_steps || first_index - n_run + 1 < 0) return fail(B200MDM_EINVAL, "bad step range");
  return B200MDM_OK;
}

static StepArgs loop_args(b200mdm_engine* e, int mode, int order, int32_t flags, bool philox) {
  StepArgs a;
  a.mode = mode;
// ... 736 lines not shown
struct StreamScratch {
  cudaStream_t s;
  std::vector<void*> ptrs;
  explicit StreamScratch(cudaStream_t st) : s(st) {}
  ~StreamScratch() {
    for (void* p : ptrs) cudaFreeAsync(p, s);
  }
  template <class T>
  int alloc(T** p, size_t n, bool zero = false) {
    CUDA_TRY(cudaMallocAsync(reinterpret_cast<void**>(p), n * sizeof(T), s));
    ptrs.push_back(*p);
    if (zero) CUDA_TRY(cudaMemsetAsync(*p, 0, n * sizeof(T), s));
    return B200MDM_OK;
  }
};

extern "C" int b200mdm_test_gemm_epi(const void* a16_dev, const void* w16_dev, const float* bias_dev, void* out16_dev,
                                     int32_t M, int32_t N, int32_t K, int32_t epi, void* stream) {
  if (!a16_dev || !w16_dev || !bias_dev || !out16_dev || M <= 0 || N <= 0 || K <= 0 || K % 8)
    return fail(B200MDM_EINVAL, "bad argument (K %% 8 == 0 required)");
  int sms = 132;
  TRY(test_prologue(&sms));
  cudaStream_t s = static_cast<cudaStream_t>(stream);
  CUtensorMap ma, mb, mc;
  TRY(make_map(&ma, a16_dev, M, K, K, GEMM_BLOCK_M));
  TRY(make_map(&mb, w16_dev, N, K, K, 128));
  if (epi == 0) {
    if (N % 64) return fail(B200MDM_EINVAL, "EpiBiasF16Wide needs N %% 64 == 0");
    TRY(make_map_t(&mc, out16_dev, 2, M, 2 * static_cast<uint64_t>(N), 2 * static_cast<uint64_t>(N), 32));
    EpiBiasF16Wide<true>::Params p{bias_dev, N};
    return launch_gemm_pp<EpiBiasF16Wide<true>>(ma, mb, mc, M, N, K, p, s, sms);
  }
  if (epi == 1) {
    if (N % 32) return fail(B200MDM_EINVAL, "EpiBiasF16Global needs N %% 32 == 0");
    TRY(make_map_t(&mc, out16_dev, 2, M, N, N, 32));
    EpiBiasF16Global::Params p{bias_dev};
    return launch_gemm_pp<EpiBiasF16Global>(ma, mb, mc, M, N, K, p, s, sms);
  }
  return fail(B200MDM_EINVAL, "epi must be 0 (EpiBiasF16Wide<GELU>) or 1 (EpiBiasF16Global)");
}

extern "C" int b200mdm_test_embed(const float* x_dev, const float* w_in_dev, const float* b_in_dev, const float* pe_dev,
                                  void* hres16_dev, int32_t B, int32_t JF, int32_t T, int32_t d, int32_t s_off,
                                  int32_t halves, void* stream) {
  if (!x_dev || !w_in_dev || !b_in_dev || !pe_dev || !hres16_dev || B <= 0 || JF <= 0 || T <= 0 || s_off < 0 ||
      d <= 0 || d % 64 || d * 4 > GEMM_BIAS_BYTES || (halves != 1 && halves != 2))
    return fail(B200MDM_EINVAL, "bad argument (d %% 64 == 0, d <= %d, halves 1 or 2)", GEMM_BIAS_BYTES / 4);
  int sms = 132;
  TRY(test_prologue(&sms));
  cudaStream_t s = static_cast<cudaStream_t>(stream);
  const int S = T + s_off, Kp = (JF + 7) & ~7, MB = B * S;
  StreamScratch scr(s);
  __half *xin16 = nullptr, *w_in3 = nullptr;
  float* pe_bias = nullptr;
  TRY(scr.alloc(&xin16, static_cast<size_t>(MB) * 3 * Kp, true));
  TRY(scr.alloc(&w_in3, static_cast<size_t>(d) * 3 * Kp, true));
  TRY(scr.alloc(&pe_bias, static_cast<size_t>(S) * d));
  TRY(launch_pack_input(x_dev, xin16, B, JF, T, S, Kp, s_off, s));
  split_weight_kernel<<<d, 128, 0, s>>>(w_in_dev, w_in3, d, JF, Kp);
  CUDA_TRY(cudaGetLastError());
  pe_bias_kernel<<<S, 128, 0, s>>>(pe_bias, pe_dev, b_in_dev, S, d);
  CUDA_TRY(cudaGetLastError());
  CUtensorMap m_xin, m_win, m_res_c, m_res_u;
  TRY(make_map(&m_xin, xin16, MB, 3 * Kp, 3 * Kp, GEMM_BLOCK_M));
  TRY(make_map(&m_win, w_in3, d, 3 * Kp, 3 * Kp, 128));
  TRY(make_map_res(&m_res_c, hres16_dev, MB, d));
  TRY(make_map_res(&m_res_u, static_cast<__half*>(hres16_dev) + (halves == 2 ? static_cast<size_t>(MB) * d * 2 : 0), MB, d));
  return launch_embed_gemm(m_xin, m_win, m_res_c, m_res_u, pe_bias, MB, S, d, Kp, halves, s, sms);
}

struct OutHook {
  const void* hres16;
  const float *scale, *w_out, *b_out;
  int B, JF, T, d, s_off, halves;
  const uint8_t* inpaint_mask;
  const float *inpaint_weight, *inpaint_motion;
  StepArgs a;
  SchedTable table = TAB_STEP;
  const float* row = nullptr;
  int index = 0, done = 0, n_steps = 0;
  float *x0_hist = nullptr, *vb_elem = nullptr, *terms = nullptr;
  const float* x_start = nullptr;
};
static int run_out_hook(OutHook h, cudaStream_t s) {
  const int B = h.B, JF = h.JF, T = h.T, d = h.d;
  if (!h.hres16 || !h.w_out || !h.b_out || !h.a.x_in || B <= 0 || JF <= 0 || T <= 0 || h.s_off < 0 || d <= 0 || d % 64 ||
      (h.halves != 1 && h.halves != 2) || (h.halves == 2 && !h.scale) ||
      (h.inpaint_mask == nullptr && h.inpaint_weight == nullptr) != (h.inpaint_motion == nullptr))
    return fail(B200MDM_EINVAL, "bad argument");
  int sms = 132;
  TRY(test_prologue(&sms));
  StreamScratch scr(s);
  const int N_out_pad = ((JF + 95) / 96) * 96;
  const size_t n = static_cast<size_t>(B) * JF * T;
  __half *g16 = nullptr, *w_out3 = nullptr;
  TRY(scr.alloc(&g16, static_cast<size_t>(B) * T * 3 * d));
  TRY(scr.alloc(&w_out3, static_cast<size_t>(N_out_pad) * 3 * d, true));
  split_weight_kernel<<<JF, 128, 0, s>>>(h.w_out, w_out3, JF, d, d);
  CUDA_TRY(cudaGetLastError());
  TRY(launch_blend_split(static_cast<const __half*>(h.hres16), g16, h.scale, B, T + h.s_off, T, h.s_off, d, h.halves, nullptr, s));
  CUtensorMap m_g16, m_wout;
  TRY(make_map(&m_g16, g16, static_cast<uint64_t>(B) * T, 3 * d, 3 * d, GEMM_BLOCK_M));
  TRY(make_map(&m_wout, w_out3, N_out_pad, 3 * d, 3 * d, 96));
  EpiOutParams p{};
  p.bias = h.b_out;
  p.inpaint_mask = h.inpaint_mask;
  p.inpaint_weight = h.inpaint_weight;
  p.inpaint_motion = h.inpaint_motion;
  float* tab[N_TABLES];
  for (int t = 0; t < N_TABLES; ++t) TRY(scr.alloc(&tab[t], static_cast<size_t>(h.index + 1) * TAB_STRIDE[t], true));
  if (h.row)
    CUDA_TRY(cudaMemcpyAsync(tab[h.table] + static_cast<size_t>(h.index) * TAB_STRIDE[h.table], h.row,
                             TAB_STRIDE[h.table] * sizeof(float), cudaMemcpyDeviceToDevice, s));
  set_tables(&p, tab);
  StepState* st = nullptr;
  TRY(scr.alloc(&st, 1));
  step_set_kernel<<<1, 1, 0, s>>>(st, h.done, h.index, nullptr, 0, 0, 0, h.n_steps);
  CUDA_TRY(cudaGetLastError());
  p.state = st;
  float* zeros = nullptr;
  TRY(scr.alloc(&zeros, n, true));
  TRY(scr.alloc(&p.eps_ring, PLMS_RING * n, true));
  p.x0_hist = h.x0_hist;
  if (!p.x0_hist) TRY(scr.alloc(&p.x0_hist, DPM_SLOTS * n, true));
  TRY(scr.alloc(&p.vb_part, static_cast<size_t>(VB_TERMS) * B * T * ((JF + 31) / 32), true));
  p.vb_elem = h.vb_elem;
  p.x_start = h.x_start ? h.x_start : zeros;
  if (!h.a.noise) h.a.noise = zeros;
  if (!h.a.x_out) TRY(scr.alloc(&h.a.x_out, n));
  TRY(launch_out_gemm(m_g16, m_wout, B, T, JF, d, h.a, p, s, sms));
  return h.terms ? launch_vb_reduce(h.terms, h.n_steps, p.vb_part, B, T, JF, st, s) : B200MDM_OK;
}

extern "C" int b200mdm_test_out_step(const void* hres16_dev, const float* scale_dev, const float* w_out_dev,
                                     const float* b_out_dev, const float* x_t_dev, const float* noise_dev,
                                     const float* sched_row_dev, int32_t mode, int32_t flags, const uint8_t* inpaint_mask_dev,
                                     const float* inpaint_motion_dev, float* x_out_dev, float* pred_xstart_dev, int32_t B,
                                     int32_t JF, int32_t T, int32_t d, int32_t s_off, int32_t halves, void* stream) {
  if (!x_out_dev || !pred_xstart_dev || mode < B200MDM_MODE_X0 || mode > B200MDM_MODE_DDIM ||
      (mode != B200MDM_MODE_X0 && (!noise_dev || !sched_row_dev)))
    return fail(B200MDM_EINVAL, "bad argument");
  OutHook h{hres16_dev, scale_dev, w_out_dev, b_out_dev, B, JF, T, d, s_off, halves, inpaint_mask_dev, nullptr, inpaint_motion_dev};
  h.a.mode = mode;
  h.a.x_in = x_t_dev;
  h.a.noise = noise_dev;
  h.a.const_noise = flags & B200MDM_FLAG_CONST_NOISE;
  h.a.clip = (flags & B200MDM_FLAG_CLIP_DENOISED) ? 1 : 0;
  h.a.x_out = x_out_dev;
  h.a.pred = pred_xstart_dev;
  h.row = sched_row_dev;
  return run_out_hook(h, static_cast<cudaStream_t>(stream));
}

extern "C" int b200mdm_test_out_dpm(const void* hres16_dev, const float* scale_dev, const float* w_out_dev,
                                    const float* b_out_dev, const float* x_t_dev, const float* dpm_row_dev, int32_t index,
                                    int32_t step, int32_t order, int32_t flags, const uint8_t* inpaint_mask_dev,
                                    const float* inpaint_motion_dev, float* x0_hist_dev, float* x_out_dev, int32_t B,
                                    int32_t JF, int32_t T, int32_t d, int32_t s_off, int32_t halves, void* stream) {
  if (!dpm_row_dev || !x0_hist_dev || !x_out_dev || index < 0 || step < 0 || (order != 1 && order != 2) ||
      (flags & ~B200MDM_FLAG_CLIP_DENOISED))
    return fail(B200MDM_EINVAL, "bad argument");
  OutHook h{hres16_dev, scale_dev, w_out_dev, b_out_dev, B, JF, T, d, s_off, halves, inpaint_mask_dev, nullptr, inpaint_motion_dev};
  h.a.mode = MODE_DPM;
  h.a.order = order;
  h.a.x_in = x_t_dev;
  h.a.clip = (flags & B200MDM_FLAG_CLIP_DENOISED) ? 1 : 0;
  h.a.x_out = x_out_dev;
  h.table = TAB_DPM;
  h.row = dpm_row_dev;
  h.index = index;
  h.done = step;
  h.n_steps = index + 1;
  h.x0_hist = x0_hist_dev;
  return run_out_hook(h, static_cast<cudaStream_t>(stream));
}

extern "C" int b200mdm_test_out_vb(const void* hres16_dev, const float* scale_dev, const float* w_out_dev,
                                   const float* b_out_dev, const float* x_t_dev, const float* x_start_dev, const float* noise_dev,
                                   const float* vb_row_dev, int32_t index, int32_t n_steps, int32_t flags,
                                   const uint8_t* inpaint_mask_dev, const float* inpaint_motion_dev, float* pred_xstart_dev,
                                   float* elem_dev, float* terms_dev, int32_t B, int32_t JF, int32_t T, int32_t d, int32_t s_off,
                                   int32_t halves, void* stream) {
  if (!x_start_dev || !noise_dev || !vb_row_dev || !terms_dev || index < 0 || index >= n_steps ||
      (flags & ~B200MDM_FLAG_CLIP_DENOISED))
    return fail(B200MDM_EINVAL, "bad argument");
  OutHook h{hres16_dev, scale_dev, w_out_dev, b_out_dev, B, JF, T, d, s_off, halves, inpaint_mask_dev, nullptr, inpaint_motion_dev};
  h.a.mode = MODE_VB;
  h.a.x_in = x_t_dev;
  h.a.noise = noise_dev;
  h.a.clip = (flags & B200MDM_FLAG_CLIP_DENOISED) ? 1 : 0;
  h.a.pred = pred_xstart_dev;
  h.table = TAB_VB;
  h.row = vb_row_dev;
  h.index = index;
  h.n_steps = n_steps;
  h.x_start = x_start_dev;
  h.vb_elem = elem_dev;
  h.terms = terms_dev;
  return run_out_hook(h, static_cast<cudaStream_t>(stream));
}

extern "C" int b200mdm_test_out_weight(const void* hres16_dev, const float* scale_dev, const float* w_out_dev,
                                       const float* b_out_dev, const float* x_t_dev, int32_t mode, int32_t flags,
                                       const float* weight_dev, const float* motion_dev, float* pred_xstart_dev, int32_t B,
                                       int32_t JF, int32_t T, int32_t d, int32_t s_off, int32_t halves, void* stream) {
  const bool family = mode == MODE_X0 || mode == MODE_DDPM || mode == MODE_DDIM || mode == MODE_PLMS_AB ||
                      mode == MODE_DDIM_REVERSE || mode == MODE_DPM || mode == MODE_VB;
  if (!pred_xstart_dev || !family || (flags & ~B200MDM_FLAG_CLIP_DENOISED)) return fail(B200MDM_EINVAL, "bad argument");
  OutHook h{hres16_dev, scale_dev, w_out_dev, b_out_dev, B, JF, T, d, s_off, halves, nullptr, weight_dev, motion_dev};
  h.a.mode = mode;
  h.a.order = 1;
  h.a.x_in = x_t_dev;
  h.a.clip = (flags & B200MDM_FLAG_CLIP_DENOISED) ? 1 : 0;
  h.a.pred = pred_xstart_dev;
  h.n_steps = 1;
  return run_out_hook(h, static_cast<cudaStream_t>(stream));
}

extern "C" int b200mdm_test_blend_handshake(const void* hres16_dev, const float* scale_dev, void* g16_dev, int32_t B,
                                            int32_t T, int32_t d, int32_t s_off, int32_t halves, int32_t h,
                                            const int64_t* lengths_host, const uint8_t* motion_start_host, void* stream) {
  if (!hres16_dev || !g16_dev || B <= 0 || T <= 0 || s_off < 0 || d <= 0 || d % 64 || (halves != 1 && halves != 2) ||
      (halves == 2 && !scale_dev))
    return fail(B200MDM_EINVAL, "bad argument");
  std::vector<int> desc;
  TRY(handshake_desc(h, B, T, lengths_host, motion_start_host, &desc));
  cudaStream_t s = static_cast<cudaStream_t>(stream);
  StreamScratch scr(s);
  int* hs = nullptr;
  if (!desc.empty()) {
    TRY(scr.alloc(&hs, desc.size()));
    CUDA_TRY(cudaMemcpyAsync(hs, desc.data(), desc.size() * sizeof(int), cudaMemcpyHostToDevice, s));
  }
  TRY(launch_blend_split(static_cast<const __half*>(hres16_dev), static_cast<__half*>(g16_dev), scale_dev, B, T + s_off, T,
                         s_off, d, halves, hs, s));
  CUDA_TRY(cudaStreamSynchronize(s));
  return B200MDM_OK;
}

extern "C" int b200mdm_test_attention(const void* qkv16_dev, void* out16_dev, const int32_t* kvlen_dev,
                                      int32_t n_samples, int32_t S, int32_t d, int32_t impl, void* stream) {
  if (!qkv16_dev || !out16_dev || !kvlen_dev || n_samples <= 0 || S <= 0) return fail(B200MDM_EINVAL, "bad argument");
  TRY(init_kernel_attrs());
  cudaStream_t s = static_cast<cudaStream_t>(stream);
  if (impl != 0 && impl != 1) return fail(B200MDM_EINVAL, "impl must be 0 (fp16 output) or 1 ([hi | lo] output)");
  if (S > ATC_MAX_KEYS) return fail(B200MDM_EINVAL, "attention handles at most %d tokens", ATC_MAX_KEYS);
  CUtensorMap mkv;
  TRY(make_attention_kv_map(&mkv, qkv16_dev, n_samples, S, 3 * d));
  return launch_attention_tc(mkv, static_cast<const __half*>(qkv16_dev), static_cast<__half*>(out16_dev), kvlen_dev, n_samples,
                             S, d, d / ATC_DH, s, impl == 1);
}

extern "C" int b200mdm_test_cross_attention(const void* q16_dev, const void* kv16_dev, const unsigned char* mask_dev,
                                            void* out16_dev, int32_t n_samples, int32_t S, int32_t n_tokens, int32_t ld_kv,
                                            void* stream) {
  const int d = 512;
  if (!q16_dev || !kv16_dev || !mask_dev || !out16_dev || n_samples <= 0 || S <= 0 || n_tokens <= 0 || n_tokens > XAL_MAX_MT ||
      ld_kv < 2 * d || ld_kv % 8)
    return fail(B200MDM_EINVAL, "bad argument");
  TRY(init_kernel_attrs());
  return launch_cross_attention(static_cast<const __half*>(q16_dev), static_cast<const __half*>(kv16_dev), mask_dev,
                                static_cast<__half*>(out16_dev), n_samples, S, n_tokens, d, d / 128, ld_kv,
                                static_cast<cudaStream_t>(stream));
}

extern "C" int b200mdm_test_qkv_attention(const void* h16_dev, int32_t ld, const void* wqkv16_dev, const float* bqkv_dev,
                                          void* out16_dev, const int32_t* kvlen_dev, int32_t n_samples, int32_t S,
                                          void* stream) {
  if (!h16_dev || !wqkv16_dev || !bqkv_dev || !out16_dev || !kvlen_dev || n_samples <= 0 || S <= 0 || S > ATC_MAX_KEYS ||
      ld < 512 || ld % 8)
    return fail(B200MDM_EINVAL, "bad argument");
  int sms = 132;
  TRY(test_prologue(&sms));
  cudaStream_t s = static_cast<cudaStream_t>(stream);
  const int M = n_samples * S;
  __half* qkv = nullptr;
  CUDA_TRY(cudaMallocAsync(reinterpret_cast<void**>(&qkv), static_cast<size_t>(M) * 1536 * sizeof(__half), s));
  CUtensorMap ma, mb, mc, mkv;
  int r = make_map(&ma, h16_dev, M, 512, ld, GEMM_BLOCK_M);
  if (r == B200MDM_OK) r = make_map(&mb, wqkv16_dev, 1536, 512, 512, 128);
  if (r == B200MDM_OK) r = make_map_t(&mc, qkv, 2, M, 1536, 1536, 32);
  if (r == B200MDM_OK) r = launch_gemm_bias<false>(ma, mb, mc, M, 1536, 512, bqkv_dev, s, sms);
  if (r == B200MDM_OK) r = make_attention_kv_map(&mkv, qkv, n_samples, S, 1536);
  if (r == B200MDM_OK)
    r = launch_attention_tc(mkv, qkv, static_cast<__half*>(out16_dev), kvlen_dev, n_samples, S, 512, 4, s);
  CUDA_TRY(cudaFreeAsync(qkv, s));
  return r;
}

extern "C" int b200mdm_test_gemm_resid_ln(const void* a16_dev, const void* w16_dev, const float* bias_dev,
                                          const float* gamma_dev, const float* beta_dev, void* hres16_dev, int32_t M,
                                          int32_t K, void* stream) {
  if (!a16_dev || !w16_dev || !bias_dev || !gamma_dev || !beta_dev || !hres16_dev || M <= 0 || K <= 0 || K % 8)
    return fail(B200MDM_EINVAL, "bad argument");
  int sms = 132;
  TRY(test_prologue(&sms));
  CUtensorMap ma, mb, mh;
  TRY(make_map(&ma, a16_dev, M, K, K, GEMM_BLOCK_M));
  TRY(make_map(&mb, w16_dev, GLN_D, K, K, 256));
  TRY(make_hres_map(&mh, hres16_dev, M));
  return launch_gemm_resid_ln(ma, mb, mh, M, K, bias_dev, gamma_dev, beta_dev, static_cast<cudaStream_t>(stream), sms);
}

extern "C" int b200mdm_test_cross_rows(b200mdm_engine* e, int32_t timestep, float* out_dev, void* stream) {
  if (!e || !out_dev) return fail(B200MDM_EINVAL, "bad argument");
  if (!e->dec_clip) return fail(B200MDM_EINVAL, "cross-attention rows belong to trans_dec engines with a CLIP memory");
  if (!e->finalized || !e->cond_set) return fail(B200MDM_ESTATE, "weights and b200mdm_set_cond_dec first");
  if (timestep < 0 || timestep >= e->cfg.temb_rows) return fail(B200MDM_EINVAL, "timestep outside [0, %d)", e->cfg.temb_rows);
  cudaStream_t s = static_cast<cudaStream_t>(stream);
  std::vector<int> t(e->B, timestep);
  CUDA_TRY(cudaMemcpyAsync(e->tvec, t.data(), e->B * sizeof(int), cudaMemcpyHostToDevice, s));
  TRY(launch_cross_rows(e, out_dev, e->tvec, 0, s));
  CUDA_TRY(cudaStreamSynchronize(s));
  return B200MDM_OK;
}

extern "C" int b200mdm_test_row_bias_ln(void* hres16_dev, const float* c_dev, const float* gamma_dev, const float* beta_dev,
                                        int32_t M, int32_t S, void* stream) {
  if (!hres16_dev || !c_dev || !gamma_dev || !beta_dev || M <= 0 || S <= 0) return fail(B200MDM_EINVAL, "bad argument");
  if ((reinterpret_cast<uintptr_t>(hres16_dev) | reinterpret_cast<uintptr_t>(c_dev) | reinterpret_cast<uintptr_t>(gamma_dev) |
       reinterpret_cast<uintptr_t>(beta_dev)) & 15)
    return fail(B200MDM_EINVAL, "operands must be 16-byte aligned");
  return launch_row_bias_ln(static_cast<__half*>(hres16_dev), c_dev, gamma_dev, beta_dev, M, S, static_cast<cudaStream_t>(stream));
}

#ifdef B200_TRACE
extern "C" int b200mdm_debug_ln_trace(uint64_t* host_out, int32_t* dims) {
  if (!dims) return fail(B200MDM_EINVAL, "bad argument");
  dims[0] = GLN_TRACE_CTAS; dims[1] = GLN_TRACE_ITERS; dims[2] = GLN_TRACE_ROLES; dims[3] = GLN_TRACE_EVENTS;
  if (host_out) {
    CUDA_TRY(cudaDeviceSynchronize());
    CUDA_TRY(cudaMemcpyFromSymbol(host_out, g_gln_trace, sizeof(g_gln_trace)));
    void* dev = nullptr;
    CUDA_TRY(cudaGetSymbolAddress(&dev, g_gln_trace));
    CUDA_TRY(cudaMemset(dev, 0, sizeof(g_gln_trace)));
    CUDA_TRY(cudaDeviceSynchronize());
  }
  return B200MDM_OK;
}
#endif

static int fill_test_joint(const float* x0_dev, const float* x0_out_dev, const float* mean_dev, const float* std_dev,
                           const float* target_dev, const float* weight_dev, int32_t B, int32_t T, int32_t D, float step,
                           int32_t iters, JointGuide* out) {
  if (!x0_dev || !x0_out_dev) return fail(B200MDM_EINVAL, "null argument");
  TRY(fill_joint(mean_dev, std_dev, target_dev, weight_dev, step, iters, out));
  if (D != 263 && D != 251) return fail(B200MDM_EINVAL, "D %d: 263 (HumanML3D) or 251 (KIT)", D);
  if (B < 1 || T < 1 || T > JG_MAX_FRAMES) return fail(B200MDM_EINVAL, "B %d, T %d: B >= 1, 1 <= T <= %d", B, T, JG_MAX_FRAMES);
  return B200MDM_OK;
}

static int test_guidance(GuideDesc d, unsigned top, const std::vector<int>& len, const std::vector<InterPair>& rows,
                         const float* x0_dev, float* x0_out_dev, float* loss_out_dev, int B, int T, int D, void* stream) {
  const GuideVariant& v = GUIDE_VARIANTS[guide_variant(top)];
  TRY(init_kernel_attrs());
  if (v.clusters) TRY(check_inter_cluster(v.test, d.i.chars, B, T, D));
  cudaStream_t s = static_cast<cudaStream_t>(stream);
  int* dlen = nullptr;
  InterPair* dpairs = nullptr;
  if (!len.empty()) {
    CUDA_TRY(cudaMallocAsync(reinterpret_cast<void**>(&dlen), len.size() * sizeof(int), s));
    CUDA_TRY(cudaMemcpyAsync(dlen, len.data(), len.size() * sizeof(int), cudaMemcpyHostToDevice, s));
    d.f.lengths = dlen;
  }
  if (!rows.empty()) {
    CUDA_TRY(cudaMallocAsync(reinterpret_cast<void**>(&dpairs), rows.size() * sizeof(InterPair), s));
    CUDA_TRY(cudaMemcpyAsync(dpairs, rows.data(), rows.size() * sizeof(InterPair), cudaMemcpyHostToDevice, s));
    d.i.pairs = dpairs;
  }
  cudaError_t err = launch_kc(v.test, dim3(B), dim3(JG_THREADS), v.smem(T, ric_dims(D).R), s, v.clusters ? d.i.chars : 0,
                              d, x0_dev, x0_out_dev, loss_out_dev, B, T, D);
  if (err == cudaSuccess) err = cudaGetLastError();
  if (dlen) cudaFreeAsync(dlen, s);
  if (dpairs) cudaFreeAsync(dpairs, s);
  if (err != cudaSuccess) return fail(B200MDM_ECUDA, "%s", cudaGetErrorString(err));
  if (dlen || dpairs) CUDA_TRY(cudaStreamSynchronize(s));
  return B200MDM_OK;
}

extern "C" int b200mdm_test_joint_guidance(const float* x0_dev, const float* mean_dev, const float* std_dev,
                                           const float* target_dev, const float* weight_dev, int32_t B, int32_t T, int32_t D,
                                           float step, int32_t iters, float* x0_out_dev, float* loss_out_dev, void* stream) {
  GuideDesc d{};
  TRY(fill_test_joint(x0_dev, x0_out_dev, mean_dev, std_dev, target_dev, weight_dev, B, T, D, step, iters, &d.j));
  return test_guidance(d, GT_JOINT, {}, {}, x0_dev, x0_out_dev, loss_out_dev, B, T, D, stream);
}

extern "C" int b200mdm_test_foot_guidance(const float* x0_dev, const float* mean_dev, const float* std_dev,
                                          const float* target_dev, const float* weight_dev, const float* contact_dev,
                                          const int64_t* lengths_host, int32_t B, int32_t T, int32_t D, float step,
                                          int32_t iters, float contact_weight, float floor_weight, float floor_height,
                                          float* x0_out_dev, float* loss_out_dev, void* stream) {
  GuideDesc d{};
  std::vector<int> len;
  TRY(fill_test_joint(x0_dev, x0_out_dev, mean_dev, std_dev, target_dev, weight_dev, B, T, D, step, iters, &d.j));
  TRY(fill_foot(contact_weight, floor_weight, floor_height, contact_dev, lengths_host, B, T, &d.f, &len));
  return test_guidance(d, GT_FOOT, len, {}, x0_dev, x0_out_dev, loss_out_dev, B, T, D, stream);
}

extern "C" int b200mdm_test_scene_guidance(const float* x0_dev, const float* mean_dev, const float* std_dev,
                                           const float* target_dev, const float* weight_dev, const float* contact_dev,
                                           const int64_t* lengths_host, int32_t B, int32_t T, int32_t D, float step,
                                           int32_t iters, float contact_weight, float floor_weight, float floor_height,
                                           float obstacle_weight, float obstacle_margin, const b200mdm_grid* sdf,
                                           const b200mdm_grid* terrain, float* x0_out_dev, float* loss_out_dev,
                                           void* stream) {
  GuideDesc d{};
  std::vector<int> len;
  TRY(fill_test_joint(x0_dev, x0_out_dev, mean_dev, std_dev, target_dev, weight_dev, B, T, D, step, iters, &d.j));
  TRY(fill_foot(contact_weight, floor_weight, floor_height, contact_dev, lengths_host, B, T, &d.f, &len));
  TRY(fill_scene(obstacle_weight, obstacle_margin, sdf, terrain, B, &d.f, "", &d.s));
  return test_guidance(d, GT_SCENE, len, {}, x0_dev, x0_out_dev, loss_out_dev, B, T, D, stream);
}

extern "C" int b200mdm_test_interaction_guidance(
    const float* x0_dev, const float* mean_dev, const float* std_dev, const float* target_dev, const float* weight_dev,
    const float* contact_dev, const int64_t* lengths_host, int32_t B, int32_t T, int32_t D, float step, int32_t iters,
    float contact_weight, float floor_weight, float floor_height, float obstacle_weight, float obstacle_margin,
    const b200mdm_grid* sdf, const b200mdm_grid* terrain, int32_t characters, float weight, float margin,
    const float* placement_dev, const int32_t* pairs_host, int32_t n_pairs, const float* reach_host,
    const float* pair_weight_dev, int64_t pair_weight_stride, float* x0_out_dev, float* loss_out_dev, void* stream) {
  GuideDesc d{};
  std::vector<int> len;
  std::vector<InterPair> rows;
  TRY(fill_test_joint(x0_dev, x0_out_dev, mean_dev, std_dev, target_dev, weight_dev, B, T, D, step, iters, &d.j));
  TRY(fill_foot(contact_weight, floor_weight, floor_height, contact_dev, lengths_host, B, T, &d.f, &len));
  TRY(fill_scene(obstacle_weight, obstacle_margin, sdf, terrain, B, &d.f, "", &d.s));
  TRY(fill_inter(characters, weight, margin, placement_dev, pairs_host, n_pairs, reach_host, pair_weight_dev,
                 pair_weight_stride, B, T, D, &d.i, &rows));
  return test_guidance(d, GT_INTER, len, rows, x0_dev, x0_out_dev, loss_out_dev, B, T, D, stream);
}

extern "C" int b200mdm_recover_from_ric(const float* data_dev, int64_t stride_b, int64_t stride_f, int64_t stride_t,
                                        const float* mean_dev, const float* std_dev, float* out_dev, int64_t ostride_b,
                                        int64_t ostride_t, int64_t ostride_c, int32_t batch, int32_t nframes,
                                        int32_t njoints, void* stream) {
  if (!data_dev || !out_dev || batch <= 0 || nframes <= 0 || njoints < 2) return fail(B200MDM_EINVAL, "bad argument");
  if ((mean_dev == nullptr) != (std_dev == nullptr)) return fail(B200MDM_EINVAL, "mean and std come together");
  const size_t smem = static_cast<size_t>(nframes) * 7 * sizeof(float);
  if (smem > 48 * 1024) return fail(B200MDM_ENOTIMPL, "recover_from_ric: %d frames exceed the single-CTA scan", nframes);
  RicArgs a;
  a.x = data_dev; a.xb = stride_b; a.xf = stride_f; a.xt = stride_t;
  a.mean = mean_dev; a.std = std_dev;
  a.out = out_dev; a.ob = ostride_b; a.ot = ostride_t; a.oc = ostride_c;
  a.T = nframes; a.joints = njoints;
  recover_from_ric_kernel<<<batch, 256, smem, static_cast<cudaStream_t>(stream)>>>(a);
  CUDA_TRY(cudaGetLastError());
  return B200MDM_OK;
}

extern "C" int b200mdm_test_target(b200mdm_engine* e, const float* target_dev, const uint8_t* valid_host, int32_t batch,
                                   float* out_dev, void* stream) {
  if (!e || !target_dev || !valid_host || !out_dev || batch <= 0) return fail(B200MDM_EINVAL, "bad argument");
  if (e->cfg.target_encoder == B200MDM_TARGET_NONE) return fail(B200MDM_EINVAL, "this engine has no target encoder");
  if (!e->finalized) return fail(B200MDM_ESTATE, "weights not finalised");
  cudaStream_t s = static_cast<cudaStream_t>(stream);
  float* valid = nullptr;
  CUDA_TRY(cudaMallocAsync(reinterpret_cast<void**>(&valid), static_cast<size_t>(batch) * e->cfg.target_joints * sizeof(float), s));
  std::vector<float> staging;
  const int r = encode_target(e, target_dev, valid_host, batch, valid, out_dev, staging, s);
  cudaFreeAsync(valid, s);
  CUDA_TRY(cudaStreamSynchronize(s));
  return r;
}
```

motion-diffusion-model_b200/csrc/gemm_ln.cuh:

```cuda
#pragma once
#include "epilogues.cuh"
#include "gemm.cuh"

namespace b200 {

constexpr int GLN_THREADS = 384;
constexpr int GLN_D = 512;
constexpr int GLN_BN = 256;
constexpr int GLN_STAGE_BYTES = (128 + GLN_BN) * GEMM_BLOCK_K * 2;
constexpr int GLN_STAGES = 4;
constexpr int GLN_GROUPS = GLN_BN / 64;
constexpr int GLN_RES_BOX_ROWS = 64;
constexpr int GLN_RES_BOX_BYTES = GLN_RES_BOX_ROWS * 128;
constexpr int GLN_RES_HALF = GEMM_BLOCK_M * 128;
static_assert(2 * GLN_RES_HALF <= GLN_STAGE_BYTES, "a residual group fits in one ring stage");
static_assert(GLN_GROUPS <= GLN_STAGES, "a tile's residual groups occupy distinct ring stages");
constexpr int GLN_REGS_PRODUCER = 40, GLN_REGS_CONSUMER = 232;
constexpr int GLN_AUX_BYTES = 3 * GLN_BN * 4  + 2 * 128 * 8  + 1024 ;

struct GemmLnSmem {
  static constexpr int TOTAL = 1024 + GLN_STAGES * GLN_STAGE_BYTES + GLN_AUX_BYTES;
  static_assert(TOTAL <= 227 * 1024, "shared memory budget");
};

#ifdef B200_TRACE
constexpr int GLN_TRACE_CTAS = 264, GLN_TRACE_ITERS = 16, GLN_TRACE_ROLES = 3, GLN_TRACE_EVENTS = 8;
__device__ uint64_t g_gln_trace[GLN_TRACE_CTAS * GLN_TRACE_ITERS * GLN_TRACE_ROLES * GLN_TRACE_EVENTS];
__device__ __forceinline__ void gln_stamp(int it, int role, int ev) {
  if (blockIdx.x < GLN_TRACE_CTAS && it < GLN_TRACE_ITERS)
    g_gln_trace[((blockIdx.x * GLN_TRACE_ITERS + it) * GLN_TRACE_ROLES + role) * GLN_TRACE_EVENTS + ev] = globaltimer_ns();
}
#define GLN_STAMP(cond, it, role, ev) if (cond) gln_stamp(it, role, ev)
#else
#define GLN_STAMP(cond, it, role, ev)
#endif

struct GemmLnParams {
  const float* bias;
  const float* gamma;
  const float* beta;
  float eps;
};

__global__ void __cluster_dims__(2, 1, 1) __launch_bounds__(GLN_THREADS, 1)
gemm_resid_ln_cluster(const __grid_constant__ CUtensorMap map_a, const __grid_constant__ CUtensorMap map_b,
                      const __grid_constant__ CUtensorMap map_h, int M, int K, const GemmLnParams lp) {
  extern __shared__ uint8_t smem_raw[];
  uint8_t* tiles = smem_raw + smem_pad1024(smem_raw);
  float* prm = reinterpret_cast<float*>(tiles + GLN_STAGES * GLN_STAGE_BYTES);
  float2* st_remote = reinterpret_cast<float2*>(prm + 3 * GLN_BN);
  uint64_t* bars = reinterpret_cast<uint64_t*>(st_remote + 256);
  uint64_t* full_bar = bars;
  uint64_t* empty_bar = bars + GLN_STAGES;
  uint64_t* xbar = bars + 2 * GLN_STAGES;

  const int warp = threadIdx.x >> 5;
  const int lane = threadIdx.x & 31;
  const uint32_t rank = cluster_ctarank();
  const int cluster_id = blockIdx.x >> 1;
  const int num_clusters = gridDim.x >> 1;
  const int num_tiles = (M + GEMM_BLOCK_M - 1) / GEMM_BLOCK_M;
  const int num_kb = (K + GEMM_BLOCK_K - 1) / GEMM_BLOCK_K;
  const int col_cta = static_cast<int>(rank) * GLN_BN;

  pdl_launch_dependents();
  for (int i = threadIdx.x; i < GLN_BN; i += blockDim.x) {
    prm[i] = lp.bias[col_cta + i];
    prm[GLN_BN + i] = lp.gamma[col_cta + i];
    prm[2 * GLN_BN + i] = lp.beta[col_cta + i];
  }
  if (threadIdx.x == 0) {
    tma_prefetch_desc(&map_a);
    tma_prefetch_desc(&map_b);
    tma_prefetch_desc(&map_h);
    for (int s = 0; s < GLN_STAGES; ++s) {
      mbar_init(&full_bar[s], 1);
      mbar_init(&empty_bar[s], 8);
    }
    for (int s = 0; s < 16; ++s) mbar_init(&xbar[s], 1);
    fence_barrier_init();
  }
  __syncthreads();
  cluster_sync_all();
  pdl_wait();

  if (warp < 4) {
    asm volatile("setmaxnreg.dec.sync.aligned.u32 %0;" ::"n"(GLN_REGS_PRODUCER));
    if (warp == 0 && elect_one()) {
      Ring<GLN_STAGES> ring;
      for (int tile = cluster_id; tile < num_tiles; tile += num_clusters) {
        GLN_STAMP(true, (tile - cluster_id) / num_clusters, 0, 0);
        produce_kblocks(ring, tiles, GLN_STAGE_BYTES, full_bar, empty_bar, &map_a, tile * GEMM_BLOCK_M, &map_b, 16384,
                        col_cta, num_kb, [&] { GLN_STAMP(true, (tile - cluster_id) / num_clusters, 0, 1); });
        const int r0 = tile * GEMM_BLOCK_M;
        const bool two = r0 + GLN_RES_BOX_ROWS < M;
        for (int grp = 0; grp < GLN_GROUPS; ++grp) {
          mbar_wait(&empty_bar[ring.stage], ring.phase ^ 1);
          uint64_t* fb = &full_bar[ring.stage];
          uint8_t* sr = tiles + ring.stage * GLN_STAGE_BYTES;
          const int c = col_cta + 64 * grp;
          mbar_expect_tx(fb, (two ? 4 : 2) * GLN_RES_BOX_BYTES);
          tma_load_2d(sr, &map_h, fb, c, r0);
          tma_load_2d(sr + GLN_RES_HALF, &map_h, fb, GLN_D + c, r0);
          if (two) {
            tma_load_2d(sr + GLN_RES_BOX_BYTES, &map_h, fb, c, r0 + GLN_RES_BOX_ROWS);
            tma_load_2d(sr + GLN_RES_HALF + GLN_RES_BOX_BYTES, &map_h, fb, GLN_D + c, r0 + GLN_RES_BOX_ROWS);
          }
          ring.advance();
        }
        GLN_STAMP(true, (tile - cluster_id) / num_clusters, 0, 2);
      }
    }
  } else {
    asm volatile("setmaxnreg.inc.sync.aligned.u32 %0;" ::"n"(GLN_REGS_CONSUMER));
    const int wg = (warp >> 2) - 1;
    const int wq = warp & 3;
    const int cw = warp - 4;
    const int g = lane >> 2, t = lane & 3;
    const int lrow = 64 * wg + 16 * wq + g;
    const bool store_thread = wq == 0 && lane == 0;
    const int toff = lrow * 128 + 4 * t;
    const float* bias_s = prm;
    const float* gamma_s = prm + GLN_BN;
    const float* beta_s = prm + 2 * GLN_BN;
    Ring<GLN_STAGES> ring;
    float acc[128];
    int it = 0;
    auto mma = [&](uint32_t s, int kb) {
      GLN_STAMP(kb == 0 && store_thread, it, 1 + wg, 1);
      const uint64_t da = wgmma_desc_k_sw128(s + wg * 64 * 128);
      const uint64_t db = wgmma_desc_k_sw128(s + 16384);
      wgmma_fence_acc(acc);
      wgmma_fence();
#pragma unroll
      for (int k = 0; k < GEMM_BLOCK_K / 16; ++k) Wgmma<256>::mma(acc, da + 2 * k, db + 2 * k, (kb | k) != 0);
      wgmma_commit();
      wgmma_fence_acc(acc);
    };
    for (int tile = cluster_id; tile < num_tiles; tile += num_clusters, ++it) {
      const int as = it & 1;
      const uint32_t aphase = (it >> 1) & 1;
      if (lane == 0) mbar_expect_tx(&xbar[as * 8 + cw], 16 * 8);
      GLN_STAMP(store_thread, it, 1 + wg, 0);
      const int last_stage = consume_kblocks(ring, tiles, GLN_STAGE_BYTES, full_bar, empty_bar, num_kb, lane, mma);
      wgmma_wait<0>();
      wgmma_fence_acc(acc);
      GLN_STAMP(store_thread, it, 1 + wg, 2);
      if (lane == 0) mbar_arrive(&empty_bar[last_stage]);

      float sa = 0.f, qa = 0.f, sb = 0.f, qb = 0.f;
#pragma unroll
      for (int j = 0; j < GLN_BN / 8; ++j) {
        const int grp = j >> 3, jj = j & 7;
        const Ring<GLN_STAGES> rg = ring.ahead(grp);
        if (jj == 0) mbar_wait(&full_bar[rg.stage], rg.phase);
        GLN_STAMP(jj == 0 && (grp == 0 || grp == GLN_GROUPS - 1) && store_thread, it, 1 + wg, grp == 0 ? 3 : 4);
        const uint8_t* slab = tiles + rg.stage * GLN_STAGE_BYTES + toff + ((jj ^ g) << 4);
        const int c = 8 * j + 2 * t;
        const float2 bb = *reinterpret_cast<const float2*>(bias_s + c);
        float2 ra, rb;
        {
          const float2 h = __half22float2(*reinterpret_cast<const __half2*>(slab));
          const float2 l = __half22float2(*reinterpret_cast<const __half2*>(slab + GLN_RES_HALF));
          ra = make_float2(h.x + l.x, h.y + l.y);
        }
        {
          const float2 h = __half22float2(*reinterpret_cast<const __half2*>(slab + 1024));
          const float2 l = __half22float2(*reinterpret_cast<const __half2*>(slab + GLN_RES_HALF + 1024));
          rb = make_float2(h.x + l.x, h.y + l.y);
        }
        acc[4 * j] = ra.x + (acc[4 * j] + bb.x);
        acc[4 * j + 1] = ra.y + (acc[4 * j + 1] + bb.y);
        acc[4 * j + 2] = rb.x + (acc[4 * j + 2] + bb.x);
        acc[4 * j + 3] = rb.y + (acc[4 * j + 3] + bb.y);
        sa += acc[4 * j] + acc[4 * j + 1];
        qa = fmaf(acc[4 * j], acc[4 * j], fmaf(acc[4 * j + 1], acc[4 * j + 1], qa));
        sb += acc[4 * j + 2] + acc[4 * j + 3];
        qb = fmaf(acc[4 * j + 2], acc[4 * j + 2], fmaf(acc[4 * j + 3], acc[4 * j + 3], qb));
      }
#pragma unroll
      for (int o = 1; o < 4; o <<= 1) {
        sa += __shfl_xor_sync(0xffffffffu, sa, o);
        qa += __shfl_xor_sync(0xffffffffu, qa, o);
        sb += __shfl_xor_sync(0xffffffffu, sb, o);
        qb += __shfl_xor_sync(0xffffffffu, qb, o);
      }
      float2* rem = st_remote + as * 128;
      if (t == 0) {
        const uint32_t peer = rank ^ 1;
        const uint32_t pbar = mapa_shared(smem_u32(&xbar[as * 8 + cw]), peer);
        st_async_f32x2(mapa_shared(smem_u32(&rem[lrow]), peer), sa, qa, pbar);
        st_async_f32x2(mapa_shared(smem_u32(&rem[lrow + 8]), peer), sb, qb, pbar);
      }
      mbar_wait_cluster(&xbar[as * 8 + cw], aphase);
      GLN_STAMP(store_thread, it, 1 + wg, 5);
      const float2 pa = rem[lrow], pb = rem[lrow + 8];
      const float mean_a = (sa + pa.x) * (1.f / GLN_D), mean_b = (sb + pb.x) * (1.f / GLN_D);
      const float rstd_a = rsqrtf(fmaxf((qa + pa.y) * (1.f / GLN_D) - mean_a * mean_a, 0.f) + lp.eps);
      const float rstd_b = rsqrtf(fmaxf((qb + pb.y) * (1.f / GLN_D) - mean_b * mean_b, 0.f) + lp.eps);
      const int row_wg = tile * GEMM_BLOCK_M + 64 * wg;
#pragma unroll
      for (int j = 0; j < GLN_BN / 8; ++j) {
        const int grp = j >> 3, jj = j & 7;
        const int rs = ring.ahead(grp).stage;
        uint8_t* slab = tiles + rs * GLN_STAGE_BYTES + toff + ((jj ^ g) << 4);
        const int c = 8 * j + 2 * t;
        const float2 gg = *reinterpret_cast<const float2*>(gamma_s + c);
        const float2 ee = *reinterpret_cast<const float2*>(beta_s + c);
        {
          const float y0 = (acc[4 * j] - mean_a) * rstd_a * gg.x + ee.x, y1 = (acc[4 * j + 1] - mean_a) * rstd_a * gg.y + ee.y;
          const __half2 h = __floats2half2_rn(y0, y1);
          const float2 f = __half22float2(h);
          *reinterpret_cast<__half2*>(slab) = h;
          *reinterpret_cast<__half2*>(slab + GLN_RES_HALF) = __floats2half2_rn(y0 - f.x, y1 - f.y);
        }
        {
          const float y0 = (acc[4 * j + 2] - mean_b) * rstd_b * gg.x + ee.x, y1 = (acc[4 * j + 3] - mean_b) * rstd_b * gg.y + ee.y;
          const __half2 h = __floats2half2_rn(y0, y1);
          const float2 f = __half22float2(h);
          *reinterpret_cast<__half2*>(slab + 1024) = h;
          *reinterpret_cast<__half2*>(slab + GLN_RES_HALF + 1024) = __floats2half2_rn(y0 - f.x, y1 - f.y);
        }
        if (jj == 7) {
          GLN_STAMP(grp == GLN_GROUPS - 1 && store_thread, it, 1 + wg, 6);
          fence_proxy_async_smem();
          named_bar_sync(1 + wg, 128);
          if (store_thread) {
            uint8_t* sg = tiles + rs * GLN_STAGE_BYTES + wg * GLN_RES_BOX_BYTES;
            if (row_wg < M) {
              const int cg = col_cta + 64 * grp;
              tma_store_2d(&map_h, sg, cg, row_wg);
              tma_store_2d(&map_h, sg + GLN_RES_HALF, GLN_D + cg, row_wg);
              bulk_commit_group();
            }
            bulk_wait_group_read<0>();
            GLN_STAMP(grp == GLN_GROUPS - 1, it, 1 + wg, 7);
            mbar_arrive_cnt(&empty_bar[rs], 4);
          }
        }
      }
      ring = ring.ahead(GLN_GROUPS);
    }
    if (store_thread) bulk_wait_group<0>();
  }

  __syncwarp();
  cluster_sync_all();
}

}
```

motion-diffusion-model_b200/csrc/ptx.cuh:

```cuda
#pragma once
#include <cuda.h>
#include <cuda_fp16.h>
#include <cuda_runtime.h>
#include <stdint.h>

namespace b200 {

__device__ __forceinline__ uint32_t smem_u32(const void* p) {
  return static_cast<uint32_t>(__cvta_generic_to_shared(p));
}

__device__ __forceinline__ bool elect_one() {
  uint32_t pred = 0;
  asm volatile(
      "{\n\t.reg .pred P;\n\t"
      "elect.sync _|P, 0xffffffff;\n\t"
      "selp.u32 %0, 1, 0, P;\n\t}\n"
      : "=r"(pred));
  return pred != 0;
}

__device__ __forceinline__ void mbar_init(uint64_t* bar, uint32_t count) {
  asm volatile("mbarrier.init.shared::cta.b64 [%0], %1;" ::"r"(smem_u32(bar)), "r"(count) : "memory");
}
__device__ __forceinline__ void fence_barrier_init() {
  asm volatile("fence.mbarrier_init.release.cluster;" ::: "memory");
}
__device__ __forceinline__ void mbar_expect_tx(uint64_t* bar, uint32_t bytes) {
  asm volatile("mbarrier.arrive.expect_tx.shared::cta.b64 _, [%0], %1;" ::"r"(smem_u32(bar)), "r"(bytes)
               : "memory");
}
__device__ __forceinline__ void mbar_arrive(uint64_t* bar) {
  asm volatile("mbarrier.arrive.shared::cta.b64 _, [%0];" ::"r"(smem_u32(bar)) : "memory");
}
__device__ __forceinline__ void mbar_arrive_cnt(uint64_t* bar, uint32_t count) {
  asm volatile("mbarrier.arrive.shared::cta.b64 _, [%0], %1;" ::"r"(smem_u32(bar)), "r"(count) : "memory");
}
__device__ __forceinline__ bool mbar_try_wait(uint64_t* bar, uint32_t parity) {
  uint32_t ok;
  asm volatile(
      "{\n\t.reg .pred P;\n\t"
      "mbarrier.try_wait.parity.shared::cta.b64 P, [%1], %2;\n\t"
      "selp.u32 %0, 1, 0, P;\n\t}\n"
      : "=r"(ok)
      : "r"(smem_u32(bar)), "r"(parity)
      : "memory");
  return ok != 0;
}
#ifndef B200_WATCHDOG_CYCLES
#define B200_WATCHDOG_CYCLES (4000000000ll)
#endif
__device__ __forceinline__ void mbar_wait(uint64_t* bar, uint32_t parity) {
  if (mbar_try_wait(bar, parity)) return;
  long long t0 = clock64();
  while (!mbar_try_wait(bar, parity)) {
    if (clock64() - t0 > B200_WATCHDOG_CYCLES) __trap();
  }
}

__device__ __forceinline__ void fence_proxy_async_smem() {
  asm volatile("fence.proxy.async.shared::cta;" ::: "memory");
}

__device__ __forceinline__ void tma_prefetch_desc(const CUtensorMap* m) {
  asm volatile("prefetch.tensormap [%0];" ::"l"(reinterpret_cast<uint64_t>(m)) : "memory");
}
__device__ __forceinline__ void tma_load_2d(void* smem_dst, const CUtensorMap* map, uint64_t* bar, int c0, int c1) {
  asm volatile(
      "cp.async.bulk.tensor.2d.shared::cluster.global.mbarrier::complete_tx::bytes [%0], [%1, {%3, %4}], [%2];"
      ::"r"(smem_u32(smem_dst)), "l"(reinterpret_cast<uint64_t>(map)), "r"(smem_u32(bar)), "r"(c0), "r"(c1)
      : "memory");
}
__device__ __forceinline__ void tma_load_3d(void* smem_dst, const CUtensorMap* map, uint64_t* bar, int c0, int c1, int c2) {
  asm volatile(
      "cp.async.bulk.tensor.3d.shared::cluster.global.mbarrier::complete_tx::bytes [%0], [%1, {%3, %4, %5}], [%2];"
      ::"r"(smem_u32(smem_dst)), "l"(reinterpret_cast<uint64_t>(map)), "r"(smem_u32(bar)), "r"(c0), "r"(c1), "r"(c2)
      : "memory");
}
__device__ __forceinline__ void tma_store_2d(const CUtensorMap* map, const void* smem_src, int c0, int c1) {
  asm volatile("cp.async.bulk.tensor.2d.global.shared::cta.bulk_group [%0, {%2, %3}], [%1];"
               ::"l"(reinterpret_cast<uint64_t>(map)), "r"(smem_u32(smem_src)), "r"(c0), "r"(c1)
               : "memory");
}
__device__ __forceinline__ void bulk_commit_group() { asm volatile("cp.async.bulk.commit_group;" ::: "memory"); }
template <int N>
__device__ __forceinline__ void bulk_wait_group_read() {
  asm volatile("cp.async.bulk.wait_group.read %0;" ::"n"(N) : "memory");
}
template <int N>
__device__ __forceinline__ void bulk_wait_group() {
  asm volatile("cp.async.bulk.wait_group %0;" ::"n"(N) : "memory");
}

__device__ __forceinline__ uint64_t globaltimer_ns() {
  uint64_t t;
  asm volatile("mov.u64 %0, %%globaltimer;" : "=l"(t));
  return t;
}
__device__ __forceinline__ void named_bar_sync(int id, int nthreads) {
  asm volatile("bar.sync %0, %1;" ::"r"(id), "r"(nthreads) : "memory");
}
__device__ __forceinline__ void named_bar_arrive(int id, int nthreads) {
  asm volatile("bar.arrive %0, %1;" ::"r"(id), "r"(nthreads) : "memory");
}

__device__ __forceinline__ void pdl_wait() { asm volatile("griddepcontrol.wait;" ::: "memory"); }
__device__ __forceinline__ void pdl_launch_dependents() { asm volatile("griddepcontrol.launch_dependents;" ::: "memory"); }

__device__ __forceinline__ uint32_t cluster_ctarank() {
  uint32_t r;
  asm volatile("mov.u32 %0, %%cluster_ctarank;" : "=r"(r));
  return r;
}
__device__ __forceinline__ uint32_t mapa_shared(uint32_t local_smem_addr, uint32_t cta_rank) {
  uint32_t r;
  asm volatile("mapa.shared::cluster.u32 %0, %1, %2;" : "=r"(r) : "r"(local_smem_addr), "r"(cta_rank));
  return r;
}
__device__ __forceinline__ bool mbar_try_wait_cluster(uint64_t* bar, uint32_t parity) {
  uint32_t ok;
  asm volatile(
      "{\n\t.reg .pred P;\n\t"
      "mbarrier.try_wait.parity.acquire.cluster.shared::cta.b64 P, [%1], %2;\n\t"
      "selp.u32 %0, 1, 0, P;\n\t}\n"
      : "=r"(ok)
      : "r"(smem_u32(bar)), "r"(parity)
      : "memory");
  return ok != 0;
}
__device__ __forceinline__ void mbar_wait_cluster(uint64_t* bar, uint32_t parity) {
  if (mbar_try_wait_cluster(bar, parity)) return;
  long long t0 = clock64();
  while (!mbar_try_wait_cluster(bar, parity)) {
    if (clock64() - t0 > B200_WATCHDOG_CYCLES) __trap();
  }
}
__device__ __forceinline__ void cluster_sync_all() {
  asm volatile("barrier.cluster.arrive.release.aligned;\n\tbarrier.cluster.wait.acquire.aligned;" ::: "memory");
}
__device__ __forceinline__ void cluster_arrive_release() { asm volatile("barrier.cluster.arrive.release;" ::: "memory"); }
__device__ __forceinline__ void cluster_wait_acquire() { asm volatile("barrier.cluster.wait.acquire;" ::: "memory"); }
__device__ __forceinline__ float ld_shared_cluster_f32(uint32_t addr) {
  float v;
  asm volatile("ld.shared::cluster.f32 %0, [%1];" : "=f"(v) : "r"(addr) : "memory");
  return v;
}
__device__ __forceinline__ void st_async_f32x2(uint32_t remote_addr, float a, float b, uint32_t remote_bar) {
  asm volatile("st.async.shared::cluster.mbarrier::complete_tx::bytes.v2.f32 [%0], {%1, %2}, [%3];"
               ::"r"(remote_addr), "f"(a), "f"(b), "r"(remote_bar)
               : "memory");
}

__device__ __forceinline__ uint64_t wgmma_desc_k_sw128(uint32_t smem_addr) {
  uint64_t d = 0;
  d |= static_cast<uint64_t>((smem_addr & 0x3FFFF) >> 4);
  d |= static_cast<uint64_t>(1) << 16;
  d |= static_cast<uint64_t>(1024 >> 4) << 32;
  d |= static_cast<uint64_t>(1) << 62;
  return d;
}
__device__ __forceinline__ uint64_t wgmma_desc_mn_sw128(uint32_t smem_addr, uint32_t mn_atom_bytes) {
  uint64_t d = 0;
  d |= static_cast<uint64_t>((smem_addr & 0x3FFFF) >> 4);
  d |= static_cast<uint64_t>((mn_atom_bytes >> 4) & 0x3FFF) << 16;
  d |= static_cast<uint64_t>(1024 >> 4) << 32;
  d |= static_cast<uint64_t>(1) << 62;
  return d;
}
__device__ __forceinline__ void wgmma_fence() { asm volatile("wgmma.fence.sync.aligned;" ::: "memory"); }
__device__ __forceinline__ void wgmma_commit() { asm volatile("wgmma.commit_group.sync.aligned;" ::: "memory"); }
template <int N>
__device__ __forceinline__ void wgmma_wait() {
  asm volatile("wgmma.wait_group.sync.aligned %0;" ::"n"(N) : "memory");
}
template <int NR>
__device__ __forceinline__ void wgmma_fence_acc(float (&d)[NR]) {
#pragma unroll
  for (int i = 0; i < NR; ++i) asm volatile("" : "+f"(d[i])::"memory");
}

template <int N> struct Wgmma;
template <int N, int TRANS_B> struct WgmmaRA;
#include "wgmma_ops.inc"

__device__ __forceinline__ void mma_16816(float (&c)[4], const uint32_t (&a)[4], uint32_t b0, uint32_t b1) {
  asm volatile("mma.sync.aligned.m16n8k16.row.col.f32.f16.f16.f32 {%0,%1,%2,%3}, {%4,%5,%6,%7}, {%8,%9}, {%0,%1,%2,%3};\n"
               : "+f"(c[0]), "+f"(c[1]), "+f"(c[2]), "+f"(c[3])
               : "r"(a[0]), "r"(a[1]), "r"(a[2]), "r"(a[3]), "r"(b0), "r"(b1));
}
__device__ __forceinline__ void ldmatrix_x4(uint32_t (&r)[4], uint32_t smem_addr) {
  asm volatile("ldmatrix.sync.aligned.m8n8.x4.shared.b16 {%0,%1,%2,%3}, [%4];"
               : "=r"(r[0]), "=r"(r[1]), "=r"(r[2]), "=r"(r[3]) : "r"(smem_addr));
}
__device__ __forceinline__ void ldmatrix_x4_trans(uint32_t (&r)[4], uint32_t smem_addr) {
  asm volatile("ldmatrix.sync.aligned.m8n8.x4.trans.shared.b16 {%0,%1,%2,%3}, [%4];"
               : "=r"(r[0]), "=r"(r[1]), "=r"(r[2]), "=r"(r[3]) : "r"(smem_addr));
}

}
```

Measured before the change: 430.6.

## Fuse FFN up-projection, GELU and down-projection with residual LayerNorm into one cluster kernel

Adds a 2-CTA cluster kernel that computes the FFN hidden activations in 128-column chunks held in shared memory, exchanges them with the peer CTA via bulk cluster copies, and feeds them straight into the down-projection with the residual-add LayerNorm epilogue. This removes the write and re-read of the full FFN intermediate through global memory, and one kernel launch per layer. The residual epilogue and producer code are factored into shared helpers, and the watchdog trap is moved into a noinline function, probably to reduce register and code pressure. The cost is tighter register and shared-memory budgets and cross-CTA handshakes that can serialise the up and down phases.

After: 426.0, median of 6. -1.1%, worse.

```diff
diff --git a/include/b200mdm.h b/include/b200mdm.h
--- a/include/b200mdm.h
+++ b/include/b200mdm.h
@@ -269,6 +269,9 @@
                                void* out16_dev, const int32_t* kvlen_dev, int32_t n_samples, int32_t S, void* stream);
 int b200mdm_test_gemm_resid_ln(const void* a16_dev, const void* w16_dev, const float* bias_dev, const float* gamma_dev,
                                const float* beta_dev, void* hres16_dev, int32_t M, int32_t K, void* stream);
+int b200mdm_test_ffn_block(void* hres16_dev, const void* w1_dev, const float* b1_dev, const void* w2_dev, const float* b2_dev,
+                           const float* gamma_dev, const float* beta_dev, void* h_out_dev, int32_t M, int32_t ff,
+                           void* stream);
 int b200mdm_test_target(b200mdm_engine* e, const float* target_dev, const uint8_t* valid_host, int32_t batch,
                         float* out_dev, void* stream);
 int b200mdm_test_cross_rows(b200mdm_engine* e, int32_t timestep, float* out_dev, void* stream);
diff --git a/motion-diffusion-model_b200/_lib.py b/motion-diffusion-model_b200/_lib.py
--- a/motion-diffusion-model_b200/_lib.py
+++ b/motion-diffusion-model_b200/_lib.py
@@ -24,7 +24,7 @@
     "b200mdm_denoise", "b200mdm_sample_step", "b200mdm_sample_loop", "b200mdm_q_sample", "b200mdm_launch_count",
     "b200mdm_sample_loop_range", "b200mdm_set_noise_stream", "b200mdm_philox_normal",
     "b200mdm_recover_from_ric", "b200mdm_test_gemm_f16", "b200mdm_test_attention", "b200mdm_test_cross_attention", "b200mdm_test_qkv_attention",
-    "b200mdm_test_gemm_resid_ln", "b200mdm_test_gemm_epi", "b200mdm_test_embed", "b200mdm_test_out_step",
+    "b200mdm_test_gemm_resid_ln", "b200mdm_test_ffn_block", "b200mdm_test_gemm_epi", "b200mdm_test_embed", "b200mdm_test_out_step",
     "b200mdm_set_target", "b200mdm_test_target", "b200mdm_plms_loop_range", "b200mdm_plms_step",
     "b200mdm_set_schedule_next", "b200mdm_ddim_reverse_loop_range", "b200mdm_test_cross_rows",
     "b200mdm_test_row_bias_ln", "b200mdm_test_forward_taps",
@@ -113,6 +113,8 @@
         lib.b200mdm_test_cross_attention.argtypes = [vp, vp, vp, vp, i32, i32, i32, i32, vp]
     lib.b200mdm_test_qkv_attention.argtypes = [vp, i32, vp, vp, vp, vp, i32, i32, vp]
     lib.b200mdm_test_gemm_resid_ln.argtypes = [vp, vp, vp, vp, vp, vp, i32, i32, vp]
+    if hasattr(lib, "b200mdm_test_ffn_block"):
+        lib.b200mdm_test_ffn_block.argtypes = [vp, vp, vp, vp, vp, vp, vp, vp, i32, i32, vp]
     for name, args in (("b200mdm_test_gemm_epi", [vp, vp, vp, vp, i32, i32, i32, i32, vp]),
                        ("b200mdm_test_embed", [vp, vp, vp, vp, vp, i32, i32, i32, i32, i32, i32, vp]),
                        ("b200mdm_test_out_step", [vp, vp, vp, vp, vp, vp, vp, i32, i32, vp, vp, vp, vp,
diff --git a/motion-diffusion-model_b200/csrc/engine.cu b/motion-diffusion-model_b200/csrc/engine.cu
--- a/motion-diffusion-model_b200/csrc/engine.cu
+++ b/motion-diffusion-model_b200/csrc/engine.cu
@@ -17,6 +17,7 @@
 #include "epilogues.cuh"
 #include "gemm.cuh"
 #include "gemm_ln.cuh"
+#include "ffn_block.cuh"
 #include "gemm_pingpong.cuh"
 #include "chunk_frame.cuh"
 #include "joint_guidance.cuh"
@@ -325,6 +326,7 @@
   TRY((set_pingpong_attr<EpiBiasF16Wide<true>>()));
   TRY((set_pingpong_attr<EpiBiasF16Global>()));
   CUDA_TRY(cudaFuncSetAttribute(gemm_resid_ln_cluster, cudaFuncAttributeMaxDynamicSharedMemorySize, GemmLnSmem::TOTAL));
+  CUDA_TRY(cudaFuncSetAttribute(ffn_block_cluster, cudaFuncAttributeMaxDynamicSharedMemorySize, FfnBlockSmem::TOTAL));
   TRY((set_gemm_attr<128, EpiEmbed>()));
   TRY((set_gemm_attr<96, EpiOut<OutStep>>()));
   TRY((set_gemm_attr<96, EpiOut<OutStepSlots>>()));
@@ -427,6 +429,19 @@
   const int clusters = tiles < max_clusters ? tiles : max_clusters;
   GemmLnParams lp{bias, gamma, beta, 1e-5f};
   CUDA_TRY(launch_k(gemm_resid_ln_cluster, dim3(2 * clusters), dim3(GLN_THREADS), GemmLnSmem::TOTAL, s, a, w256, hres, M, K, lp));
+  return B200MDM_OK;
+}
+
+static bool ffn_block_fits(int ff) { return ff % (2 * FFB_CHUNK) == 0 && ff <= FFB_MAX_FF; }
+static int launch_ffn_block(const CUtensorMap& a, const CUtensorMap& w1, const CUtensorMap& w2_256, const CUtensorMap& hres,
+                            int M, int ff, const float* b1, const float* b2, const float* gamma, const float* beta, __half* h_out,
+                            cudaStream_t s, int num_sms) {
+  if (!ffn_block_fits(ff)) return fail(B200MDM_ENOTIMPL, "FFN block: ff %d is not a multiple of %d up to %d", ff, 2 * FFB_CHUNK, FFB_MAX_FF);
+  const int tiles = (M + GEMM_BLOCK_M - 1) / GEMM_BLOCK_M;
+  const int max_clusters = num_sms / 2;
+  const int clusters = tiles < max_clusters ? tiles : max_clusters;
+  FfnBlockParams p{b1, b2, gamma, beta, 1e-5f, ff, h_out};
+  CUDA_TRY(launch_k(ffn_block_cluster, dim3(2 * clusters), dim3(FFB_THREADS), FfnBlockSmem::TOTAL, s, a, w1, w2_256, hres, M, p));
   return B200MDM_OK;
 }
 
@@ -1869,17 +1884,26 @@
       nk += 3;
     }
     if (taps) TRY(take_taps(e, *taps, B200MDM_TAP_L_LN2, B200MDM_TAP_L_LN2, l, s));
-    if (wide) {
-      EpiBiasF16Wide<true>::Params p{w.b1, ff};
-      TRY((launch_gemm_pp<EpiBiasF16Wide<true>>(e->m_h16, w.m_w1, e->m_ffn_st, e->M, ff, kw * d, p, s, e->num_sms)));
-    } else if (!B200_SKIP(4)) {
-      TRY((launch_gemm_bias<true>(e->m_h16, w.m_w1, e->m_ffn_st, e->M, ff, d, w.b1, s, e->num_sms)));
+    const float* g_ffn = e->dec ? w.g3 : w.g2;
+    const float* be_ffn = e->dec ? w.be3 : w.be2;
+    if (!wide && ffn_block_fits(ff)) {
+      if (!B200_SKIP(8))
+        TRY(launch_ffn_block(e->m_h16, w.m_w1, w.m_w2_256, e->m_hres, e->M, ff, w.b1, w.b2, g_ffn, be_ffn,
+                             taps ? e->ffn16 : nullptr, s, e->num_sms));
+      if (taps) TRY(take_taps(e, *taps, B200MDM_TAP_L_FFN, B200MDM_TAP_L_FFN, l, s));
+      nk += 4;
+    } else {
+      if (wide) {
+        EpiBiasF16Wide<true>::Params p{w.b1, ff};
+        TRY((launch_gemm_pp<EpiBiasF16Wide<true>>(e->m_h16, w.m_w1, e->m_ffn_st, e->M, ff, kw * d, p, s, e->num_sms)));
+      } else if (!B200_SKIP(4)) {
+        TRY((launch_gemm_bias<true>(e->m_h16, w.m_w1, e->m_ffn_st, e->M, ff, d, w.b1, s, e->num_sms)));
+      }
+      if (taps) TRY(take_taps(e, *taps, B200MDM_TAP_L_FFN, B200MDM_TAP_L_FFN, l, s));
+      if (!B200_SKIP(8)) TRY(launch_gemm_resid_ln(e->m_ffn, w.m_w2_256, e->m_hres, e->M, kw * ff, w.b2, g_ffn, be_ffn, s, e->num_sms));
+      nk += 5;
     }
-    if (taps) TRY(take_taps(e, *taps, B200MDM_TAP_L_FFN, B200MDM_TAP_L_FFN, l, s));
-    if (!B200_SKIP(8)) TRY(launch_gemm_resid_ln(e->m_ffn, w.m_w2_256, e->m_hres, e->M, kw * ff, w.b2, e->dec ? w.g3 : w.g2,
-                             e->dec ? w.be3 : w.be2, s, e->num_sms));
     if (taps) TRY(take_taps(e, *taps, B200MDM_TAP_L_LN3, B200MDM_TAP_L_LN3, l, s));
-    nk += 5;
   }
   const int G = e->groups, GB = G ? G * B : B;
   TRY(launch_blend_split(e->hres, e->g16, e->scale, GB, S, T, e->s_off, d, G ? 1 : e->halves, e->hs_set ? e->hs_desc : nullptr, s));
@@ -3222,6 +3246,23 @@
   return launch_gemm_resid_ln(ma, mb, mh, M, K, bias_dev, gamma_dev, beta_dev, static_cast<cudaStream_t>(stream), sms);
 }
 
+extern "C" int b200mdm_test_ffn_block(void* hres16_dev, const void* w1_dev, const float* b1_dev, const void* w2_dev,
+                                      const float* b2_dev, const float* gamma_dev, const float* beta_dev, void* h_out_dev,
+                                      int32_t M, int32_t ff, void* stream) {
+  if (!hres16_dev || !w1_dev || !b1_dev || !w2_dev || !b2_dev || !gamma_dev || !beta_dev || M <= 0)
+    return fail(B200MDM_EINVAL, "bad argument");
+  if (!ffn_block_fits(ff)) return fail(B200MDM_EINVAL, "ff %d: a multiple of %d up to %d", ff, 2 * FFB_CHUNK, FFB_MAX_FF);
+  int sms = 132;
+  TRY(test_prologue(&sms));
+  CUtensorMap ma, mw1, mw2, mh;
+  TRY(make_map(&ma, hres16_dev, M, GLN_D, 2 * GLN_D, GEMM_BLOCK_M));
+  TRY(make_map(&mw1, w1_dev, ff, GLN_D, GLN_D, FFB_CHUNK));
+  TRY(make_map(&mw2, w2_dev, GLN_D, ff, ff, 256));
+  TRY(make_hres_map(&mh, hres16_dev, M));
+  return launch_ffn_block(ma, mw1, mw2, mh, M, ff, b1_dev, b2_dev, gamma_dev, beta_dev, static_cast<__half*>(h_out_dev),
+                          static_cast<cudaStream_t>(stream), sms);
+}
+
 extern "C" int b200mdm_test_cross_rows(b200mdm_engine* e, int32_t timestep, float* out_dev, void* stream) {
   if (!e || !out_dev) return fail(B200MDM_EINVAL, "bad argument");
   if (!e->dec_clip) return fail(B200MDM_EINVAL, "cross-attention rows belong to trans_dec engines with a CLIP memory");
diff --git a/motion-diffusion-model_b200/csrc/ffn_block.cuh b/motion-diffusion-model_b200/csrc/ffn_block.cuh
--- /dev/null
+++ b/motion-diffusion-model_b200/csrc/ffn_block.cuh
@@ -0,0 +1,240 @@
+#pragma once
+#include "gemm_ln.cuh"
+
+namespace b200 {
+
+constexpr int FFB_THREADS = 384;
+constexpr int FFB_REGS_PRODUCER = 40, FFB_REGS_CONSUMER = 232;
+constexpr int FFB_STAGES = 4;
+constexpr int FFB_STAGE_BYTES = 32768;
+constexpr int FFB_CHUNK = 128;
+constexpr int FFB_UP_TX = GEMM_BLOCK_M * GEMM_BLOCK_K * 2 + FFB_CHUNK * GEMM_BLOCK_K * 2;
+constexpr int FFB_BOX_BYTES = GEMM_BLOCK_M * 128;
+constexpr int FFB_H_BYTES = 2 * FFB_BOX_BYTES;
+constexpr int FFB_H_WG_BYTES = FFB_BOX_BYTES / 2;
+constexpr int FFB_MAX_FF = 2048;
+constexpr int FFB_AUX_BYTES = 3 * GLN_BN * 4  + FFB_MAX_FF * 4  + 2 * 128 * 8  +
+                              1024 ;
+struct FfnBlockSmem {
+  static constexpr int TOTAL = 1024 + FFB_STAGES * FFB_STAGE_BYTES + 2 * FFB_H_BYTES + FFB_AUX_BYTES;
+  static_assert(TOTAL <= 227 * 1024, "shared memory budget");
+};
+static_assert(2 * GLN_RES_HALF <= FFB_STAGE_BYTES && FFB_UP_TX <= FFB_STAGE_BYTES, "stage layouts");
+static_assert(GLN_GROUPS <= FFB_STAGES, "a tile's residual groups occupy distinct ring stages");
+
+struct FfnBlockParams {
+  const float* b1;
+  const float* b2;
+  const float* gamma;
+  const float* beta;
+  float eps;
+  int ff;
+  __half* h_out;
+};
+
+__global__ void __cluster_dims__(2, 1, 1) __launch_bounds__(FFB_THREADS, 1)
+ffn_block_cluster(const __grid_constant__ CUtensorMap map_a, const __grid_constant__ CUtensorMap map_w1,
+                  const __grid_constant__ CUtensorMap map_w2, const __grid_constant__ CUtensorMap map_h, int M,
+                  const FfnBlockParams p) {
+  extern __shared__ uint8_t smem_raw[];
+  uint8_t* tiles = smem_raw + smem_pad1024(smem_raw);
+  uint8_t* hslab = tiles + FFB_STAGES * FFB_STAGE_BYTES;
+  float* prm = reinterpret_cast<float*>(hslab + 2 * FFB_H_BYTES);
+  float* b1s = prm + 3 * GLN_BN;
+  float2* st_remote = reinterpret_cast<float2*>(b1s + FFB_MAX_FF);
+  uint64_t* bars = reinterpret_cast<uint64_t*>(st_remote + 256);
+  uint64_t* full_bar = bars;
+  uint64_t* empty_bar = bars + FFB_STAGES;
+  uint64_t* xbar = bars + 2 * FFB_STAGES;
+  uint64_t* hfull = xbar + 16;
+  uint64_t* hfree = hfull + 2;
+
+  const int warp = threadIdx.x >> 5;
+  const int lane = threadIdx.x & 31;
+  const uint32_t rank = cluster_ctarank();
+  const uint32_t peer = rank ^ 1;
+  const int cluster_id = blockIdx.x >> 1;
+  const int num_clusters = gridDim.x >> 1;
+  const int num_tiles = (M + GEMM_BLOCK_M - 1) / GEMM_BLOCK_M;
+  const int steps = p.ff / (2 * FFB_CHUNK);
+  const int col_cta = static_cast<int>(rank) * GLN_BN;
+
+  pdl_launch_dependents();
+  for (int i = threadIdx.x; i < GLN_BN; i += blockDim.x) {
+    prm[i] = p.b2[col_cta + i];
+    prm[GLN_BN + i] = p.gamma[col_cta + i];
+    prm[2 * GLN_BN + i] = p.beta[col_cta + i];
+  }
+  for (int i = threadIdx.x; i < p.ff; i += blockDim.x) b1s[i] = p.b1[i];
+  if (threadIdx.x == 0) {
+    tma_prefetch_desc(&map_a);
+    tma_prefetch_desc(&map_w1);
+    tma_prefetch_desc(&map_w2);
+    tma_prefetch_desc(&map_h);
+    for (int s = 0; s < FFB_STAGES; ++s) {
+      mbar_init(&full_bar[s], 1);
+      mbar_init(&empty_bar[s], 8);
+    }
+    for (int s = 0; s < 16; ++s) mbar_init(&xbar[s], 1);
+    for (int s = 0; s < 2; ++s) {
+      mbar_init(&hfull[s], 1);
+      mbar_init(&hfree[s], 4);
+    }
+    fence_barrier_init();
+  }
+  __syncthreads();
+  cluster_sync_all();
+  pdl_wait();
+
+  if (warp < 4) {
+    asm volatile("setmaxnreg.dec.sync.aligned.u32 %0;" ::"n"(FFB_REGS_PRODUCER));
+    if (warp == 0 && elect_one()) {
+      Ring<FFB_STAGES> ring;
+      for (int tile = cluster_id; tile < num_tiles; tile += num_clusters) {
+        const int row0 = tile * GEMM_BLOCK_M;
+        for (int s = 0; s <= steps; ++s) {
+          if (s < steps) {
+            const int w_row = FFB_CHUNK * (2 * s + static_cast<int>(rank));
+            for (int kb = 0; kb < GLN_D / GEMM_BLOCK_K; ++kb) {
+              mbar_wait(&empty_bar[ring.stage], ring.phase ^ 1);
+              uint8_t* st = tiles + ring.stage * FFB_STAGE_BYTES;
+              uint64_t* fb = &full_bar[ring.stage];
+              mbar_expect_tx(fb, FFB_UP_TX);
+              tma_load_2d(st, &map_a, fb, kb * GEMM_BLOCK_K, row0);
+              tma_load_2d(st + GEMM_BLOCK_M * 128, &map_w1, fb, kb * GEMM_BLOCK_K, w_row);
+              ring.advance();
+            }
+          }
+          if (s > 0) {
+            for (int j = 0; j < 2 * FFB_CHUNK / GEMM_BLOCK_K; ++j) {
+              mbar_wait(&empty_bar[ring.stage], ring.phase ^ 1);
+              uint64_t* fb = &full_bar[ring.stage];
+              mbar_expect_tx(fb, FFB_STAGE_BYTES);
+              tma_load_2d(tiles + ring.stage * FFB_STAGE_BYTES, &map_w2, fb, 2 * FFB_CHUNK * (s - 1) + GEMM_BLOCK_K * j, col_cta);
+              ring.advance();
+            }
+          }
+        }
+        gln_produce_residual(ring, tiles, FFB_STAGE_BYTES, full_bar, empty_bar, &map_h, tile, M, col_cta);
+      }
+    }
+    __syncwarp();
+    cluster_sync_all();
+  } else {
+    asm volatile("setmaxnreg.inc.sync.aligned.u32 %0;" ::"n"(FFB_REGS_CONSUMER));
+    const int wg = (warp >> 2) - 1;
+    const int wq = warp & 3;
+    const int cw = warp - 4;
+    const int g = lane >> 2, t = lane & 3;
+    const bool leader = wq == 0 && lane == 0;
+    const int toff = (64 * wg + 16 * wq + g) * 128 + 4 * t;
+    const typename EpiBiasF16<true>::Params up_ep{p.b1};
+    Ring<FFB_STAGES> ring;
+    float acc[128];
+    float hacc[64];
+    uint32_t full_ph = 0, free_ph = 0;
+    int it = 0;
+    auto up_mma = [&](uint32_t s, int kb) {
+      const uint64_t da = wgmma_desc_k_sw128(s + wg * 64 * 128);
+      const uint64_t db = wgmma_desc_k_sw128(s + GEMM_BLOCK_M * 128);
+      wgmma_fence_acc(hacc);
+      wgmma_fence();
+#pragma unroll
+      for (int k = 0; k < GEMM_BLOCK_K / 16; ++k) Wgmma<128>::mma(hacc, da + 2 * k, db + 2 * k, (kb | k) != 0);
+      wgmma_commit();
+      wgmma_fence_acc(hacc);
+    };
+    auto down_mma = [&](uint32_t s, int kb) {
+      const int c = kb / (FFB_CHUNK / GEMM_BLOCK_K);
+      const uint8_t* hb = hslab + (c & 1) * FFB_H_BYTES + (kb % (FFB_CHUNK / GEMM_BLOCK_K)) * FFB_BOX_BYTES;
+      const uint64_t da = wgmma_desc_k_sw128(smem_u32(hb) + wg * 64 * 128);
+      const uint64_t db = wgmma_desc_k_sw128(s);
+      wgmma_fence_acc(acc);
+      wgmma_fence();
+#pragma unroll
+      for (int k = 0; k < GEMM_BLOCK_K / 16; ++k) Wgmma<256>::mma(acc, da + 2 * k, db + 2 * k, (kb | k) != 0);
+      wgmma_commit();
+      wgmma_fence_acc(acc);
+    };
+    constexpr int DOWN_KB = 2 * FFB_CHUNK / GEMM_BLOCK_K;
+    for (int tile = cluster_id; tile < num_tiles; tile += num_clusters, ++it) {
+      const int as = it & 1;
+      if (lane == 0) mbar_expect_tx(&xbar[as * 8 + cw], 16 * 8);
+      const int row_w = tile * GEMM_BLOCK_M + 64 * wg + 16 * wq + g;
+      for (int s = 0; s <= steps; ++s) {
+        int prev = -1;
+        auto next_stage = [&]() {
+          wgmma_wait<1>();
+          if (prev >= 0 && lane == 0) mbar_arrive(&empty_bar[prev]);
+          prev = ring.stage;
+          ring.advance();
+        };
+        if (s < steps) {
+          for (int kb = 0; kb < GLN_D / GEMM_BLOCK_K; ++kb) {
+            mbar_wait(&full_bar[ring.stage], ring.phase);
+            up_mma(smem_u32(tiles + ring.stage * FFB_STAGE_BYTES), kb);
+            next_stage();
+          }
+        }
+        if (s > 0) {
+          mbar_wait_cluster(&hfull[wg], full_ph);
+          full_ph ^= 1;
+#pragma unroll
+          for (int j = 0; j < DOWN_KB; ++j) {
+            mbar_wait(&full_bar[ring.stage], ring.phase);
+            down_mma(smem_u32(tiles + ring.stage * FFB_STAGE_BYTES), DOWN_KB * (s - 1) + j);
+            next_stage();
+          }
+        }
+        wgmma_wait<0>();
+        wgmma_fence_acc(hacc);
+        wgmma_fence_acc(acc);
+        if (lane == 0) {
+          mbar_arrive(&empty_bar[prev]);
+          if (s > 0) mbar_arrive_cluster(mapa_shared(smem_u32(&hfree[wg]), peer));
+        }
+        if (s == steps) {
+          gln_epilogue(acc, ring, tiles, FFB_STAGE_BYTES, full_bar, empty_bar, prm, st_remote, xbar, &map_h, tile, M, p.eps,
+                       it, col_cta, rank, wg, wq, lane);
+          break;
+        }
+        mbar_wait_cluster(&hfree[wg], free_ph ^ 1);
+        free_ph ^= 1;
+        uint8_t* hs = hslab + rank * FFB_H_BYTES;
+        const int hc = FFB_CHUNK * (2 * s + static_cast<int>(rank));
+#pragma unroll
+        for (int jj = 0; jj < FFB_CHUNK / 8; ++jj) {
+          const int c = 8 * jj + 2 * t;
+          const float2 bb = *reinterpret_cast<const float2*>(b1s + hc + c);
+          uint8_t* d = hs + (jj >> 3) * FFB_BOX_BYTES + toff + (((jj & 7) ^ g) << 4);
+          EpiBiasF16<true>::pp_pair(up_ep, bb, hacc[4 * jj], hacc[4 * jj + 1], d);
+          EpiBiasF16<true>::pp_pair(up_ep, bb, hacc[4 * jj + 2], hacc[4 * jj + 3], d + 1024);
+          if (p.h_out) {
+            if (row_w < M)
+              *reinterpret_cast<uint32_t*>(p.h_out + static_cast<size_t>(row_w) * p.ff + hc + c) = *reinterpret_cast<const uint32_t*>(d);
+            if (row_w + 8 < M)
+              *reinterpret_cast<uint32_t*>(p.h_out + static_cast<size_t>(row_w + 8) * p.ff + hc + c) =
+                  *reinterpret_cast<const uint32_t*>(d + 1024);
+          }
+        }
+        fence_proxy_async_smem();
+        named_bar_sync(1 + wg, 128);
+        if (leader) {
+          mbar_expect_tx(&hfull[wg], 2 * FFB_H_WG_BYTES);
+          const uint32_t bar = mapa_shared(smem_u32(&hfull[wg]), peer);
+#pragma unroll
+          for (int box = 0; box < 2; ++box) {
+            const uint8_t* src = hs + box * FFB_BOX_BYTES + wg * FFB_H_WG_BYTES;
+            bulk_copy_to_peer(mapa_shared(smem_u32(src), peer), src, FFB_H_WG_BYTES, bar);
+          }
+        }
+      }
+      ring = ring.ahead(GLN_GROUPS);
+    }
+    if (leader) bulk_wait_group<0>();
+    __syncwarp();
+    cluster_sync_all();
+  }
+}
+
+}
diff --git a/motion-diffusion-model_b200/csrc/gemm_ln.cuh b/motion-diffusion-model_b200/csrc/gemm_ln.cuh
--- a/motion-diffusion-model_b200/csrc/gemm_ln.cuh
+++ b/motion-diffusion-model_b200/csrc/gemm_ln.cuh
@@ -42,6 +42,136 @@
   float eps;
 };
 
+template <int STAGES>
+__device__ __forceinline__ void gln_produce_residual(Ring<STAGES>& ring, uint8_t* tiles, int stage_bytes, uint64_t* full_bar,
+                                                     uint64_t* empty_bar, const CUtensorMap* map_h, int tile, int M,
+                                                     int col_cta) {
+  const int r0 = tile * GEMM_BLOCK_M;
+  const bool two = r0 + GLN_RES_BOX_ROWS < M;
+  for (int grp = 0; grp < GLN_GROUPS; ++grp) {
+    mbar_wait(&empty_bar[ring.stage], ring.phase ^ 1);
+    uint64_t* fb = &full_bar[ring.stage];
+    uint8_t* sr = tiles + ring.stage * stage_bytes;
+    const int c = col_cta + 64 * grp;
+    mbar_expect_tx(fb, (two ? 4 : 2) * GLN_RES_BOX_BYTES);
+    tma_load_2d(sr, map_h, fb, c, r0);
+    tma_load_2d(sr + GLN_RES_HALF, map_h, fb, GLN_D + c, r0);
+    if (two) {
+      tma_load_2d(sr + GLN_RES_BOX_BYTES, map_h, fb, c, r0 + GLN_RES_BOX_ROWS);
+      tma_load_2d(sr + GLN_RES_HALF + GLN_RES_BOX_BYTES, map_h, fb, GLN_D + c, r0 + GLN_RES_BOX_ROWS);
+    }
+    ring.advance();
+  }
+}
+
+template <int STAGES>
+__device__ __forceinline__ void gln_epilogue(float (&acc)[128], const Ring<STAGES>& ring, uint8_t* tiles, int stage_bytes,
+                                             uint64_t* full_bar, uint64_t* empty_bar, const float* prm, float2* st_remote,
+                                             uint64_t* xbar, const CUtensorMap* map_h, int tile, int M, float eps, int it,
+                                             int col_cta, uint32_t rank, int wg, int wq, int lane) {
+  const int cw = 4 * wg + wq;
+  const int g = lane >> 2, t = lane & 3;
+  const int lrow = 64 * wg + 16 * wq + g;
+  const bool store_thread = wq == 0 && lane == 0;
+  const int toff = lrow * 128 + 4 * t;
+  const float* bias_s = prm;
+  const float* gamma_s = prm + GLN_BN;
+  const float* beta_s = prm + 2 * GLN_BN;
+  const int as = it & 1;
+  const uint32_t aphase = (it >> 1) & 1;
+  float sa = 0.f, qa = 0.f, sb = 0.f, qb = 0.f;
+#pragma unroll
+  for (int j = 0; j < GLN_BN / 8; ++j) {
+    const int grp = j >> 3, jj = j & 7;
+    const Ring<STAGES> rg = ring.ahead(grp);
+    if (jj == 0) mbar_wait(&full_bar[rg.stage], rg.phase);
+    GLN_STAMP(jj == 0 && (grp == 0 || grp == GLN_GROUPS - 1) && store_thread, it, 1 + wg, grp == 0 ? 3 : 4);
+    const uint8_t* slab = tiles + rg.stage * stage_bytes + toff + ((jj ^ g) << 4);
+    const int c = 8 * j + 2 * t;
+    const float2 bb = *reinterpret_cast<const float2*>(bias_s + c);
+    float2 ra, rb;
+    {
+      const float2 h = __half22float2(*reinterpret_cast<const __half2*>(slab));
+      const float2 l = __half22float2(*reinterpret_cast<const __half2*>(slab + GLN_RES_HALF));
+      ra = make_float2(h.x + l.x, h.y + l.y);
+    }
+    {
+      const float2 h = __half22float2(*reinterpret_cast<const __half2*>(slab + 1024));
+      const float2 l = __half22float2(*reinterpret_cast<const __half2*>(slab + GLN_RES_HALF + 1024));
+      rb = make_float2(h.x + l.x, h.y + l.y);
+    }
+    acc[4 * j] = ra.x + (acc[4 * j] + bb.x);
+    acc[4 * j + 1] = ra.y + (acc[4 * j + 1] + bb.y);
+    acc[4 * j + 2] = rb.x + (acc[4 * j + 2] + bb.x);
+    acc[4 * j + 3] = rb.y + (acc[4 * j + 3] + bb.y);
+    sa += acc[4 * j] + acc[4 * j + 1];
+    qa = fmaf(acc[4 * j], acc[4 * j], fmaf(acc[4 * j + 1], acc[4 * j + 1], qa));
+    sb += acc[4 * j + 2] + acc[4 * j + 3];
+    qb = fmaf(acc[4 * j + 2], acc[4 * j + 2], fmaf(acc[4 * j + 3], acc[4 * j + 3], qb));
+  }
+#pragma unroll
+  for (int o = 1; o < 4; o <<= 1) {
+    sa += __shfl_xor_sync(0xffffffffu, sa, o);
+    qa += __shfl_xor_sync(0xffffffffu, qa, o);
+    sb += __shfl_xor_sync(0xffffffffu, sb, o);
+    qb += __shfl_xor_sync(0xffffffffu, qb, o);
+  }
+  float2* rem = st_remote + as * 128;
+  if (t == 0) {
+    const uint32_t peer = rank ^ 1;
+    const uint32_t pbar = mapa_shared(smem_u32(&xbar[as * 8 + cw]), peer);
+    st_async_f32x2(mapa_shared(smem_u32(&rem[lrow]), peer), sa, qa, pbar);
+    st_async_f32x2(mapa_shared(smem_u32(&rem[lrow + 8]), peer), sb, qb, pbar);
+  }
+  mbar_wait_cluster(&xbar[as * 8 + cw], aphase);
+  GLN_STAMP(store_thread, it, 1 + wg, 5);
+  const float2 pa = rem[lrow], pb = rem[lrow + 8];
+  const float mean_a = (sa + pa.x) * (1.f / GLN_D), mean_b = (sb + pb.x) * (1.f / GLN_D);
+  const float rstd_a = rsqrtf(fmaxf((qa + pa.y) * (1.f / GLN_D) - mean_a * mean_a, 0.f) + eps);
+  const float rstd_b = rsqrtf(fmaxf((qb + pb.y) * (1.f / GLN_D) - mean_b * mean_b, 0.f) + eps);
+  const int row_wg = tile * GEMM_BLOCK_M + 64 * wg;
+#pragma unroll
+  for (int j = 0; j < GLN_BN / 8; ++j) {
+    const int grp = j >> 3, jj = j & 7;
+    const int rs = ring.ahead(grp).stage;
+    uint8_t* slab = tiles + rs * stage_bytes + toff + ((jj ^ g) << 4);
+    const int c = 8 * j + 2 * t;
+    const float2 gg = *reinterpret_cast<const float2*>(gamma_s + c);
+    const float2 ee = *reinterpret_cast<const float2*>(beta_s + c);
+    {
+      const float y0 = (acc[4 * j] - mean_a) * rstd_a * gg.x + ee.x, y1 = (acc[4 * j + 1] - mean_a) * rstd_a * gg.y + ee.y;
+      const __half2 h = __floats2half2_rn(y0, y1);
+      const float2 f = __half22float2(h);
+      *reinterpret_cast<__half2*>(slab) = h;
+      *reinterpret_cast<__half2*>(slab + GLN_RES_HALF) = __floats2half2_rn(y0 - f.x, y1 - f.y);
+    }
+    {
+      const float y0 = (acc[4 * j + 2] - mean_b) * rstd_b * gg.x + ee.x, y1 = (acc[4 * j + 3] - mean_b) * rstd_b * gg.y + ee.y;
+      const __half2 h = __floats2half2_rn(y0, y1);
+      const float2 f = __half22float2(h);
+      *reinterpret_cast<__half2*>(slab + 1024) = h;
+      *reinterpret_cast<__half2*>(slab + GLN_RES_HALF + 1024) = __floats2half2_rn(y0 - f.x, y1 - f.y);
+    }
+    if (jj == 7) {
+      GLN_STAMP(grp == GLN_GROUPS - 1 && store_thread, it, 1 + wg, 6);
+      fence_proxy_async_smem();
+      named_bar_sync(1 + wg, 128);
+      if (store_thread) {
+        uint8_t* sg = tiles + rs * stage_bytes + wg * GLN_RES_BOX_BYTES;
+        if (row_wg < M) {
+          const int cg = col_cta + 64 * grp;
+          tma_store_2d(map_h, sg, cg, row_wg);
+          tma_store_2d(map_h, sg + GLN_RES_HALF, GLN_D + cg, row_wg);
+          bulk_commit_group();
+        }
+        bulk_wait_group_read<0>();
+        GLN_STAMP(grp == GLN_GROUPS - 1, it, 1 + wg, 7);
+        mbar_arrive_cnt(&empty_bar[rs], 4);
+      }
+    }
+  }
+}
+
 __global__ void __cluster_dims__(2, 1, 1) __launch_bounds__(GLN_THREADS, 1)
 gemm_resid_ln_cluster(const __grid_constant__ CUtensorMap map_a, const __grid_constant__ CUtensorMap map_b,
                       const __grid_constant__ CUtensorMap map_h, int M, int K, const GemmLnParams lp) {
@@ -92,22 +222,7 @@
         GLN_STAMP(true, (tile - cluster_id) / num_clusters, 0, 0);
         produce_kblocks(ring, tiles, GLN_STAGE_BYTES, full_bar, empty_bar, &map_a, tile * GEMM_BLOCK_M, &map_b, 16384,
                         col_cta, num_kb, [&] { GLN_STAMP(true, (tile - cluster_id) / num_clusters, 0, 1); });
-        const int r0 = tile * GEMM_BLOCK_M;
-        const bool two = r0 + GLN_RES_BOX_ROWS < M;
-        for (int grp = 0; grp < GLN_GROUPS; ++grp) {
-          mbar_wait(&empty_bar[ring.stage], ring.phase ^ 1);
-          uint64_t* fb = &full_bar[ring.stage];
-          uint8_t* sr = tiles + ring.stage * GLN_STAGE_BYTES;
-          const int c = col_cta + 64 * grp;
-          mbar_expect_tx(fb, (two ? 4 : 2) * GLN_RES_BOX_BYTES);
-          tma_load_2d(sr, &map_h, fb, c, r0);
-          tma_load_2d(sr + GLN_RES_HALF, &map_h, fb, GLN_D + c, r0);
-          if (two) {
-            tma_load_2d(sr + GLN_RES_BOX_BYTES, &map_h, fb, c, r0 + GLN_RES_BOX_ROWS);
-            tma_load_2d(sr + GLN_RES_HALF + GLN_RES_BOX_BYTES, &map_h, fb, GLN_D + c, r0 + GLN_RES_BOX_ROWS);
-          }
-          ring.advance();
-        }
+        gln_produce_residual(ring, tiles, GLN_STAGE_BYTES, full_bar, empty_bar, &map_h, tile, M, col_cta);
         GLN_STAMP(true, (tile - cluster_id) / num_clusters, 0, 2);
       }
     }
@@ -116,13 +231,7 @@
     const int wg = (warp >> 2) - 1;
     const int wq = warp & 3;
     const int cw = warp - 4;
-    const int g = lane >> 2, t = lane & 3;
-    const int lrow = 64 * wg + 16 * wq + g;
     const bool store_thread = wq == 0 && lane == 0;
-    const int toff = lrow * 128 + 4 * t;
-    const float* bias_s = prm;
-    const float* gamma_s = prm + GLN_BN;
-    const float* beta_s = prm + 2 * GLN_BN;
     Ring<GLN_STAGES> ring;
     float acc[128];
     int it = 0;
@@ -139,7 +248,6 @@
     };
     for (int tile = cluster_id; tile < num_tiles; tile += num_clusters, ++it) {
       const int as = it & 1;
-      const uint32_t aphase = (it >> 1) & 1;
       if (lane == 0) mbar_expect_tx(&xbar[as * 8 + cw], 16 * 8);
       GLN_STAMP(store_thread, it, 1 + wg, 0);
       const int last_stage = consume_kblocks(ring, tiles, GLN_STAGE_BYTES, full_bar, empty_bar, num_kb, lane, mma);
@@ -147,98 +255,8 @@
       wgmma_fence_acc(acc);
       GLN_STAMP(store_thread, it, 1 + wg, 2);
       if (lane == 0) mbar_arrive(&empty_bar[last_stage]);
-
-      float sa = 0.f, qa = 0.f, sb = 0.f, qb = 0.f;
-#pragma unroll
-      for (int j = 0; j < GLN_BN / 8; ++j) {
-        const int grp = j >> 3, jj = j & 7;
-        const Ring<GLN_STAGES> rg = ring.ahead(grp);
-        if (jj == 0) mbar_wait(&full_bar[rg.stage], rg.phase);
-        GLN_STAMP(jj == 0 && (grp == 0 || grp == GLN_GROUPS - 1) && store_thread, it, 1 + wg, grp == 0 ? 3 : 4);
-        const uint8_t* slab = tiles + rg.stage * GLN_STAGE_BYTES + toff + ((jj ^ g) << 4);
-        const int c = 8 * j + 2 * t;
-        const float2 bb = *reinterpret_cast<const float2*>(bias_s + c);
-        float2 ra, rb;
-        {
-          const float2 h = __half22float2(*reinterpret_cast<const __half2*>(slab));
-          const float2 l = __half22float2(*reinterpret_cast<const __half2*>(slab + GLN_RES_HALF));
-          ra = make_float2(h.x + l.x, h.y + l.y);
-        }
-        {
-          const float2 h = __half22float2(*reinterpret_cast<const __half2*>(slab + 1024));
-          const float2 l = __half22float2(*reinterpret_cast<const __half2*>(slab + GLN_RES_HALF + 1024));
-          rb = make_float2(h.x + l.x, h.y + l.y);
-        }
-        acc[4 * j] = ra.x + (acc[4 * j] + bb.x);
-        acc[4 * j + 1] = ra.y + (acc[4 * j + 1] + bb.y);
-        acc[4 * j + 2] = rb.x + (acc[4 * j + 2] + bb.x);
-        acc[4 * j + 3] = rb.y + (acc[4 * j + 3] + bb.y);
-        sa += acc[4 * j] + acc[4 * j + 1];
-        qa = fmaf(acc[4 * j], acc[4 * j], fmaf(acc[4 * j + 1], acc[4 * j + 1], qa));
-        sb += acc[4 * j + 2] + acc[4 * j + 3];
-        qb = fmaf(acc[4 * j + 2], acc[4 * j + 2], fmaf(acc[4 * j + 3], acc[4 * j + 3], qb));
-      }
-#pragma unroll
-      for (int o = 1; o < 4; o <<= 1) {
-        sa += __shfl_xor_sync(0xffffffffu, sa, o);
-        qa += __shfl_xor_sync(0xffffffffu, qa, o);
-        sb += __shfl_xor_sync(0xffffffffu, sb, o);
-        qb += __shfl_xor_sync(0xffffffffu, qb, o);
-      }
-      float2* rem = st_remote + as * 128;
-      if (t == 0) {
-        const uint32_t peer = rank ^ 1;
-        const uint32_t pbar = mapa_shared(smem_u32(&xbar[as * 8 + cw]), peer);
-        st_async_f32x2(mapa_shared(smem_u32(&rem[lrow]), peer), sa, qa, pbar);
-        st_async_f32x2(mapa_shared(smem_u32(&rem[lrow + 8]), peer), sb, qb, pbar);
-      }
-      mbar_wait_cluster(&xbar[as * 8 + cw], aphase);
-      GLN_STAMP(store_thread, it, 1 + wg, 5);
-      const float2 pa = rem[lrow], pb = rem[lrow + 8];
-      const float mean_a = (sa + pa.x) * (1.f / GLN_D), mean_b = (sb + pb.x) * (1.f / GLN_D);
-      const float rstd_a = rsqrtf(fmaxf((qa + pa.y) * (1.f / GLN_D) - mean_a * mean_a, 0.f) + lp.eps);
-      const float rstd_b = rsqrtf(fmaxf((qb + pb.y) * (1.f / GLN_D) - mean_b * mean_b, 0.f) + lp.eps);
-      const int row_wg = tile * GEMM_BLOCK_M + 64 * wg;
-#pragma unroll
-      for (int j = 0; j < GLN_BN / 8; ++j) {
-        const int grp = j >> 3, jj = j & 7;
-        const int rs = ring.ahead(grp).stage;
-        uint8_t* slab = tiles + rs * GLN_STAGE_BYTES + toff + ((jj ^ g) << 4);
-        const int c = 8 * j + 2 * t;
-        const float2 gg = *reinterpret_cast<const float2*>(gamma_s + c);
-        const float2 ee = *reinterpret_cast<const float2*>(beta_s + c);
-        {
-          const float y0 = (acc[4 * j] - mean_a) * rstd_a * gg.x + ee.x, y1 = (acc[4 * j + 1] - mean_a) * rstd_a * gg.y + ee.y;
-          const __half2 h = __floats2half2_rn(y0, y1);
-          const float2 f = __half22float2(h);
-          *reinterpret_cast<__half2*>(slab) = h;
-          *reinterpret_cast<__half2*>(slab + GLN_RES_HALF) = __floats2half2_rn(y0 - f.x, y1 - f.y);
-        }
-        {
-          const float y0 = (acc[4 * j + 2] - mean_b) * rstd_b * gg.x + ee.x, y1 = (acc[4 * j + 3] - mean_b) * rstd_b * gg.y + ee.y;
-          const __half2 h = __floats2half2_rn(y0, y1);
-          const float2 f = __half22float2(h);
-          *reinterpret_cast<__half2*>(slab + 1024) = h;
-          *reinterpret_cast<__half2*>(slab + GLN_RES_HALF + 1024) = __floats2half2_rn(y0 - f.x, y1 - f.y);
-        }
-        if (jj == 7) {
-          GLN_STAMP(grp == GLN_GROUPS - 1 && store_thread, it, 1 + wg, 6);
-          fence_proxy_async_smem();
-          named_bar_sync(1 + wg, 128);
-          if (store_thread) {
-            uint8_t* sg = tiles + rs * GLN_STAGE_BYTES + wg * GLN_RES_BOX_BYTES;
-            if (row_wg < M) {
-              const int cg = col_cta + 64 * grp;
-              tma_store_2d(&map_h, sg, cg, row_wg);
-              tma_store_2d(&map_h, sg + GLN_RES_HALF, GLN_D + cg, row_wg);
-              bulk_commit_group();
-            }
-            bulk_wait_group_read<0>();
-            GLN_STAMP(grp == GLN_GROUPS - 1, it, 1 + wg, 7);
-            mbar_arrive_cnt(&empty_bar[rs], 4);
-          }
-        }
-      }
+      gln_epilogue(acc, ring, tiles, GLN_STAGE_BYTES, full_bar, empty_bar, prm, st_remote, xbar, &map_h, tile, M, lp.eps, it,
+                   col_cta, rank, wg, wq, lane);
       ring = ring.ahead(GLN_GROUPS);
     }
     if (store_thread) bulk_wait_group<0>();
diff --git a/motion-diffusion-model_b200/csrc/ptx.cuh b/motion-diffusion-model_b200/csrc/ptx.cuh
--- a/motion-diffusion-model_b200/csrc/ptx.cuh
+++ b/motion-diffusion-model_b200/csrc/ptx.cuh
@@ -50,11 +50,12 @@
 #ifndef B200_WATCHDOG_CYCLES
 #define B200_WATCHDOG_CYCLES (4000000000ll)
 #endif
+__device__ __noinline__ void watchdog_trap() { __trap(); }
 __device__ __forceinline__ void mbar_wait(uint64_t* bar, uint32_t parity) {
   if (mbar_try_wait(bar, parity)) return;
   long long t0 = clock64();
   while (!mbar_try_wait(bar, parity)) {
-    if (clock64() - t0 > B200_WATCHDOG_CYCLES) __trap();
+    if (clock64() - t0 > B200_WATCHDOG_CYCLES) watchdog_trap();
   }
 }
 
@@ -132,7 +133,7 @@
   if (mbar_try_wait_cluster(bar, parity)) return;
   long long t0 = clock64();
   while (!mbar_try_wait_cluster(bar, parity)) {
-    if (clock64() - t0 > B200_WATCHDOG_CYCLES) __trap();
+    if (clock64() - t0 > B200_WATCHDOG_CYCLES) watchdog_trap();
   }
 }
 __device__ __forceinline__ void cluster_sync_all() {
@@ -148,6 +149,15 @@
 __device__ __forceinline__ void st_async_f32x2(uint32_t remote_addr, float a, float b, uint32_t remote_bar) {
   asm volatile("st.async.shared::cluster.mbarrier::complete_tx::bytes.v2.f32 [%0], {%1, %2}, [%3];"
                ::"r"(remote_addr), "f"(a), "f"(b), "r"(remote_bar)
+               : "memory");
+}
+
+__device__ __forceinline__ void mbar_arrive_cluster(uint32_t remote_bar) {
+  asm volatile("mbarrier.arrive.release.cluster.shared::cluster.b64 _, [%0];" ::"r"(remote_bar) : "memory");
+}
+__device__ __forceinline__ void bulk_copy_to_peer(uint32_t remote_dst, const void* src, uint32_t bytes, uint32_t remote_bar) {
+  asm volatile("cp.async.bulk.shared::cluster.shared::cta.mbarrier::complete_tx::bytes [%0], [%1], %2, [%3];"
+               ::"r"(remote_dst), "r"(smem_u32(src)), "r"(bytes), "r"(remote_bar)
                : "memory");
 }
 
```
